# second-state/qwen3_asr_rs

Hardware: AMD Instinct MI355X
Metric: audio-seconds/sec (RTFx) Qwen3-ASR-0.6B greedy, 30s clips (higher is better)
Workload: dtype bf16; 1 GPU; Qwen3-ASR-0.6b bf16, batch=1 x 30s synthetic 16kHz clip per GPU, 100 new tokens (fixed, EOS ignored); clips_per_gpu=1, parallelism=dp1 (independent utterances per GPU, no data-path collective)

## Files before the change

### include/q3asr.h

```cpp
#ifndef Q3ASR_H
#define Q3ASR_H

#include <stdint.h>

#ifdef __cplusplus
extern "C" {
#endif

typedef struct q3a_engine q3a_engine;

typedef struct q3a_opts {
  int32_t precise;
  int32_t max_new_tokens;
  int32_t use_graph;
  int32_t debug_taps;
  int32_t valu_attention;
  int32_t token_logprobs;
  int32_t reserved[10];
} q3a_opts;

void q3a_opts_default(q3a_opts* o);

typedef struct q3a_dims {
  int32_t enc_d_model, enc_layers, enc_heads, enc_ffn, num_mel_bins, n_window, n_window_infer,
// ... 129 lines not shown


int32_t q3a_aligner_info(const q3a_engine* e, int32_t* classify_num, int32_t* timestamp_token_id, float* segment_ms);
int32_t q3a_build_align_prompt(int32_t num_audio_tokens, const int32_t* text_ids, int32_t n_text, int32_t* ids, int32_t* len);
int32_t q3a_align(q3a_engine* e, const int32_t* ids, const int32_t* lens, int32_t B, int32_t* out_classes, int32_t stride,
                  int32_t* out_counts, float* logits_out);
int32_t q3a_align_batch_ptrs(q3a_engine* e, const float* const* pcm16k, const int64_t* n_samples, int32_t B, const int32_t* text_ids,
                             const int32_t* text_lens, int32_t* out_classes, int32_t stride, int32_t* out_counts);
int32_t q3a_split_words_for_alignment(const char* utf8, const char* language, char* out, int32_t cap, int32_t* n_words,
                                      int32_t* len);
int32_t q3a_align_text_ids(const q3a_tokenizer* t, const char* const* words, int32_t n_words, int32_t timestamp_token_id,
                           int32_t* ids, int32_t cap, int32_t* n);
int32_t q3a_fix_timestamps(const float* ms, int32_t n, float* out);


int32_t q3a_score(q3a_engine* e, const int32_t* prompt_ids, const int32_t* prompt_lens, const int32_t* target_ids,
                  const int32_t* target_lens, int32_t B, float* out_lp, int32_t* out_top_ids, float* out_top_lp, int32_t stride,
                  float* logits_out);
int32_t q3a_score_batch_ptrs(q3a_engine* e, const float* const* pcm16k, const int64_t* n_samples, int32_t B,
                             const int32_t* lang_prefix_ids, int32_t n_prefix, const int32_t* target_ids, const int32_t* target_lens,
                             float* out_lp, int32_t* out_top_ids, float* out_top_lp, int32_t stride);


int32_t q3a_prefill_draft(q3a_engine* e, const int32_t* prompt_ids, const int32_t* prompt_lens, const int32_t* draft_ids,
                          const int32_t* draft_lens, int32_t B, int32_t* accepted_out, int32_t* next_ids_out, float* logits_out);
int32_t q3a_transcribe_draft_batch_ptrs(q3a_engine* e, const float* const* pcm16k, const int64_t* n_samples, int32_t B,
                                        const int32_t* lang_prefix_ids, int32_t n_prefix, const int32_t* draft_ids, const int32_t* draft_lens,
                                        int32_t max_new, int32_t max_rounds, int32_t min_tail, int32_t* out_ids, int32_t stride,
                                        int32_t* out_lens, int32_t* accepted_out);
int32_t q3a_draft_next_round(const int32_t* draft, int32_t n, int32_t k, int32_t tok, int32_t* out, int32_t cap, int32_t* n_out);
int32_t q3a_selftest_draft_accept(int32_t device, int32_t S, const int32_t* draft_ids, const int32_t* draft_off, const int32_t* prompt_lens,
                                  const int32_t* top_ids, const float* top_lp, int32_t out_stride, const uint16_t* embed, int32_t V, int32_t H,
                                  const float* norm_w, int32_t group_size, const float* cos_t, const float* sin_t, int32_t max_pos,
                                  int32_t* accepted, int32_t* out_ids, float* out_lp, int32_t* state, float* x_next, float* rope_cur,
                                  uint16_t* nn_x, float* nn_ss);


int32_t q3a_beam_search_batch_ptrs(q3a_engine* e, const float* const* pcm16k, const int64_t* n_samples, int32_t U,
                                   const int32_t* lang_prefix_ids, int32_t n_prefix, int32_t width, int32_t max_new, int32_t* out_ids,
                                   int32_t stride, int32_t* out_lens, float* out_scores, uint8_t* out_finished, float* out_lp);
int32_t q3a_beam_begin(q3a_engine* e, int32_t width);
int32_t q3a_beam_step(q3a_engine* e, uint8_t* all_finished, float* logits_out);
int32_t q3a_beam_fetch(q3a_engine* e, int32_t* out_ids, int32_t stride, int32_t* out_lens, float* out_scores, uint8_t* out_finished,
                       float* out_lp);
int32_t q3a_selftest_beam_topk(int32_t device, const float* logits, int32_t S, int32_t V, int32_t W, int32_t* out_ids, float* out_lp);
int32_t q3a_selftest_beam_advance(int32_t device, int32_t U, int32_t W, const int32_t* topk_ids, const float* topk_lp, const float* score_in,
                                  const uint8_t* finished_in, int32_t* parent_out, int32_t* token_out, float* score_out, uint8_t* finished_out);
int32_t q3a_selftest_kv_reorder(int32_t device, void* cache, int32_t elem_bytes, int32_t layers, int32_t S, int32_t n_kv, int32_t max_ctx,
                                const int32_t* lo, const int32_t* hi, const int32_t* parent);


int32_t q3a_set_logit_bias(q3a_engine* e, const int32_t* ids, const float* bias, int32_t n, float default_bias);
int32_t q3a_parse_logit_bias(const char* text, const char* suppress_list, int32_t* ids, float* bias, int32_t cap, int32_t* n);

int32_t q3a_set_sampling(q3a_engine* e, float temperature, float min_p, uint64_t seed);
uint32_t q3a_sample_word(uint64_t seed, uint32_t s, uint32_t t, uint32_t j);
int32_t q3a_selftest_sample(int32_t device, const float* logits, int32_t S, int32_t V, float temperature, float min_p,
                            uint64_t seed, int32_t step, int32_t* out_ids, float* out_lp, float* out_z);

int32_t q3a_set_repetition(q3a_engine* e, float repetition_penalty, int32_t no_repeat_ngram_size);
int32_t q3a_selftest_repeat(int32_t device, const float* logits, int32_t S, int32_t V, const int32_t* hist, int32_t stride,
                            const int32_t* lens, float p, int32_t n, float* out_logits, int32_t* out_ids, float* out_lp);

int32_t q3a_debug_set(const char* key, int32_t value);

int32_t q3a_selftest_gemm(int32_t device, int32_t M, int32_t N, int32_t K, int32_t split, float* max_abs_err,
                          float* ref_abs_max);
int32_t q3a_selftest_gemm16(int32_t device, int32_t M, int32_t N, int32_t K, int32_t reps, float* max_abs_err,
                            float* ref_abs_max, float* avg_us_bf16, float* avg_us_f32);

int32_t q3a_selftest_gemm_launch(int32_t device, int32_t launcher, int32_t flags, const void* x, const uint16_t* w, int32_t M, int32_t N, int32_t K,
                                 int32_t lda, int32_t ldo, int32_t imgs, int32_t H, int32_t Wd, int32_t C, const float* bias, const float* addend,
                                 int32_t addend_period, const float* resid, const int32_t* rowmap, int32_t act, void* out, int32_t out_rows);
int32_t q3a_selftest_qkrope_launch(int32_t device, int32_t fused, int32_t kv_f32, const uint16_t* x, int32_t lda, const uint16_t* w, int32_t M, int32_t K,
                                   const float* bias, float* qkv, const int32_t* row_seq, const int32_t* row_pos, const float* q_norm,
                                   const float* k_norm, float eps, const float* cos_t, const float* sin_t, int32_t max_pos, int32_t n_q, int32_t n_kv,
                                   int32_t n_seq, int32_t max_ctx, uint16_t* q16, void* kcache, void* vcache);
int32_t q3a_selftest_gemv_launch(int32_t device, int32_t pruned, const uint16_t* w, int32_t N, int32_t K, const float* x, const float* rms_w, float eps,
                                 const float* bias, int32_t mode, const float* resid, const float* attn_pm, const float* attn_pl, const float* attn_po,
                                 int32_t attn_nsplit, int32_t attn_heads, float* out, int32_t* out_state);
int32_t q3a_selftest_decode_attn_launch(int32_t device, int32_t kv_f32, const float* qkv, int32_t pos, const float* q_norm, const float* k_norm, float eps,
                                        const float* rope_cur, void* kcache, void* vcache, int32_t n_q, int32_t n_kv, int32_t max_ctx, int32_t nsplit,
                                        float scale_div, float* pm, float* pl, float* po);
int32_t q3a_gemm256_split_rows(int32_t M, int32_t N);

#ifdef __cplusplus
}
#endif
#endif
```

### qwen3_asr_rs_amd/_lib.py

```python
from __future__ import annotations

import ctypes as C
import os

HERE = os.path.dirname(os.path.abspath(__file__))
LIB_PATH = os.environ.get("Q3A_LIB") or os.path.join(HERE, "lib", "libq3asr_hip.so")

SYMBOLS = [
    "q3a_opts_default", "q3a_device_count", "q3a_engine_create", "q3a_arena_bytes", "q3a_arena_pack", "q3a_engine_create_from_arena",
    "q3a_engine_destroy", "q3a_last_error", "q3a_get_dims", "q3a_weights_rounded", "q3a_num_frames", "q3a_num_audio_tokens",
    "q3a_build_prompt", "q3a_mel", "q3a_encode", "q3a_prefill", "q3a_decode_step", "q3a_set_next_tokens",
    "q3a_upload_pcm", "q3a_run_resident", "q3a_fetch_ids", "q3a_fetch_logprobs", "q3a_transcribe_batch", "q3a_transcribe_batch_ptrs", "q3a_io_timings_last", "q3a_stage_timings",
    "q3a_profile_decode_step", "q3a_profile_weight_stream", "q3a_measure_peaks", "q3a_debug_read", "q3a_debug_set", "q3a_selftest_gemm", "q3a_selftest_gemm16",
    "q3a_load_audio", "q3a_resample", "q3a_resample_rubato", "q3a_free", "q3a_tokenizer_create", "q3a_tokenizer_destroy",
    "q3a_tokenizer_decode", "q3a_tokenizer_encode", "q3a_normalize_nfc", "q3a_parse_asr_output", "q3a_capitalize_first",
    "q3a_group_create", "q3a_group_destroy", "q3a_group_size", "q3a_group_used_rccl", "q3a_group_last_error",
    "q3a_group_engine", "q3a_group_partition", "q3a_group_transcribe", "q3a_group_transcribe_ptrs", "q3a_group_startup_seconds",
    "q3a_aligner_info", "q3a_build_align_prompt", "q3a_align", "q3a_align_batch_ptrs", "q3a_split_words_for_alignment",
    "q3a_align_text_ids", "q3a_fix_timestamps", "q3a_score", "q3a_score_batch_ptrs",
    "q3a_beam_search_batch_ptrs", "q3a_beam_begin", "q3a_beam_step", "q3a_beam_fetch", "q3a_selftest_beam_topk", "q3a_selftest_beam_advance",
    "q3a_selftest_kv_reorder", "q3a_set_logit_bias", "q3a_parse_logit_bias",
    "q3a_set_sampling", "q3a_sample_word", "q3a_selftest_sample",
    "q3a_set_repetition", "q3a_selftest_repeat",
    "q3a_selftest_gemm_launch", "q3a_selftest_qkrope_launch", "q3a_gemm256_split_rows",
    "q3a_selftest_gemv_launch", "q3a_selftest_decode_attn_launch",
    "q3a_prefill_draft", "q3a_transcribe_draft_batch_ptrs", "q3a_draft_next_round", "q3a_selftest_draft_accept",
]


class Peaks(C.Structure):
    _fields_ = [("hbm_read_gbps", C.c_double), ("hbm_copy_gbps", C.c_double), ("hbm_triad_gbps", C.c_double), ("hbm_read_bytes", C.c_double),
                ("mfma_bf16_tflops", C.c_double), ("gemm_m", C.c_int32), ("gemm_n", C.c_int32), ("gemm_k", C.c_int32), ("n_cu", C.c_int32),
                ("reps", C.c_int32), ("reserved", C.c_int32), ("mfma_bf16_tflops_random", C.c_double)]


class Opts(C.Structure):
    _fields_ = [("precise", C.c_int32), ("max_new_tokens", C.c_int32), ("use_graph", C.c_int32),
                ("debug_taps", C.c_int32), ("valu_attention", C.c_int32), ("token_logprobs", C.c_int32), ("reserved", C.c_int32 * 10)]


class DimsC(C.Structure):
    _fields_ = [(n, C.c_int32) for n in (
        "enc_d_model", "enc_layers", "enc_heads", "enc_ffn", "num_mel_bins", "n_window", "n_window_infer",
        "conv_channels", "enc_output_dim", "max_source_positions", "vocab_size", "hidden_size",
        "intermediate_size", "dec_layers", "num_q_heads", "num_kv_heads", "head_dim", "tie_word_embeddings",
        "mrope_interleaved")] + [("mrope_section", C.c_int32 * 4), ("rms_norm_eps", C.c_float), ("rope_theta", C.c_double)]


class Timings(C.Structure):
    _fields_ = [("mel_ms", C.c_float), ("encoder_ms", C.c_float), ("prefill_ms", C.c_float), ("decode_ms", C.c_float),
                ("total_ms", C.c_float), ("decode_steps", C.c_int32), ("batch", C.c_int32),
                ("total_audio_tokens", C.c_int32), ("total_prompt_tokens", C.c_int32)]


class IoTimings(C.Structure):
    _fields_ = [("stage_ms", C.c_float), ("h2d_ms", C.c_float), ("wall_ms", C.c_float), ("pieces", C.c_int32), ("threads", C.c_int32),
                ("mode", C.c_int32)]


KC_NAMES = ["gemv_qkv_gateup", "decode_attn", "argmax", "gemm", "norm", "other", "gemv_o_proj", "gemv_down", "gemv_lm_head"]


class KernelProfile(C.Structure):
    _fields_ = [("total_us", C.c_float * 9), ("launches", C.c_int32 * 9), ("weight_bytes", C.c_double * 9)]


_lib = None


def load() -> C.CDLL:
    global _lib
    if _lib is not None:
        return _lib
    if not os.path.exists(LIB_PATH):
        raise RuntimeError(f"{LIB_PATH} not found: build it with `python -m qwen3_asr_rs_amd.build` "
                           "(there is no CPU fallback for the HIP engine)")
    lib = C.CDLL(LIB_PATH)
    P, i32, i64, u64, f32p = C.c_void_p, C.c_int32, C.c_int64, C.c_uint64, C.POINTER(C.c_float)
    i32p, i64p, u8p = C.POINTER(C.c_int32), C.POINTER(C.c_int64), C.POINTER(C.c_uint8)
    sig = {
        "q3a_opts_default": (None, [C.POINTER(Opts)]),
        "q3a_device_count": (i32, []),
        "q3a_engine_create": (i32, [C.c_char_p, i32, C.POINTER(Opts), C.POINTER(P)]),
        "q3a_arena_bytes": (i32, [C.c_char_p, C.POINTER(u64)]),
        "q3a_arena_pack": (i32, [C.c_char_p, P, u64]),
        "q3a_engine_create_from_arena": (i32, [C.c_char_p, i32, P, u64, C.POINTER(Opts), C.POINTER(P)]),
        "q3a_engine_destroy": (None, [P]),
        "q3a_last_error": (C.c_char_p, [P]),
        "q3a_get_dims": (i32, [P, C.POINTER(DimsC)]),
        "q3a_weights_rounded": (i32, [P]),
        "q3a_num_frames": (i64, [i64]),
        "q3a_num_audio_tokens": (i32, [P, i64]),
        "q3a_build_prompt": (i32, [i32, i32p, i32, i32p, i32p]),
        "q3a_mel": (i32, [P, f32p, i64p, i32, f32p, i32p]),
        "q3a_encode": (i32, [P, f32p, i32p]),
        "q3a_prefill": (i32, [P, i32p, i32p, i32, f32p, i32p]),
        "q3a_decode_step": (i32, [P, i32p, u8p, f32p]),
        "q3a_set_next_tokens": (i32, [P, i32p, i32]),
        "q3a_upload_pcm": (i32, [P, f32p, i64p, i32]),
        "q3a_run_resident": (i32, [P, i32p, i32, i32, i32]),
        "q3a_fetch_ids": (i32, [P, i32p, i32, i32p]),
        "q3a_fetch_logprobs": (i32, [P, f32p, i32, i32p]),
        "q3a_transcribe_batch": (i32, [P, f32p, i64p, i32, i32p, i32, i32, i32, i32p, i32, i32p]),
        "q3a_transcribe_batch_ptrs": (i32, [P, C.POINTER(P), i64p, i32, i32p, i32, i32, i32, i32p, i32, i32p]),
        "q3a_io_timings_last": (i32, [P, C.POINTER(IoTimings)]),
        "q3a_stage_timings": (i32, [P, C.POINTER(Timings)]),
        "q3a_profile_decode_step": (i32, [P, C.POINTER(KernelProfile)]),
        "q3a_profile_weight_stream": (i32, [P, i32, f32p, C.POINTER(C.c_double), i32p]),
        "q3a_measure_peaks": (i32, [i32, i32, C.POINTER(Peaks)]),
        "q3a_debug_read": (i32, [P, C.c_char_p, P, u64, C.POINTER(u64)]),
        "q3a_debug_set": (i32, [C.c_char_p, i32]),
        "q3a_selftest_gemm": (i32, [i32, i32, i32, i32, i32, f32p, f32p]),
        "q3a_selftest_gemm16": (i32, [i32, i32, i32, i32, i32, f32p, f32p, f32p, f32p]),
        "q3a_load_audio": (i32, [C.c_char_p, i32, C.POINTER(f32p), i64p]),
        "q3a_resample": (i32, [f32p, i64, i32, i32, C.POINTER(f32p), i64p]),
        "q3a_resample_rubato": (i32, [f32p, i64, i32, i32, C.POINTER(f32p), i64p]),
        "q3a_free": (None, [P]),
        "q3a_tokenizer_create": (i32, [C.c_char_p, C.POINTER(P)]),
        "q3a_tokenizer_destroy": (None, [P]),
        "q3a_tokenizer_decode": (i32, [P, i32p, i32, i32, C.c_char_p, i32, i32p]),
        "q3a_tokenizer_encode": (i32, [P, C.c_char_p, i32p, i32, i32p]),
        "q3a_parse_asr_output": (i32, [C.c_char_p, i32, C.c_char_p, i32, C.c_char_p, i32]),
        "q3a_capitalize_first": (i32, [C.c_char_p, C.c_char_p, i32]),
        "q3a_normalize_nfc": (i32, [C.c_char_p, C.c_char_p, i32, i32p]),
        "q3a_group_create": (i32, [C.c_char_p, i32, i32p, C.POINTER(Opts), C.POINTER(P)]),
        "q3a_group_destroy": (None, [P]),
        "q3a_group_size": (i32, [P]),
        "q3a_group_used_rccl": (i32, [P]),
        "q3a_group_startup_seconds": (i32, [P, C.POINTER(C.c_double)]),
        "q3a_group_last_error": (C.c_char_p, [P]),
        "q3a_group_engine": (P, [P, i32]),
        "q3a_group_partition": (None, [i32, i32, i32, i32p, i32p]),
        "q3a_group_transcribe": (i32, [P, f32p, i64p, i32, i32p, i32, i32, i32, i32p, i32, i32p]),
        "q3a_group_transcribe_ptrs": (i32, [P, C.POINTER(P), i64p, i32, i32p, i32, i32, i32, i32p, i32, i32p]),
        "q3a_aligner_info": (i32, [P, i32p, i32p, f32p]),
        "q3a_build_align_prompt": (i32, [i32, i32p, i32, i32p, i32p]),
        "q3a_align": (i32, [P, i32p, i32p, i32, i32p, i32, i32p, f32p]),
        "q3a_align_batch_ptrs": (i32, [P, C.POINTER(P), i64p, i32, i32p, i32p, i32p, i32, i32p]),
        "q3a_split_words_for_alignment": (i32, [C.c_char_p, C.c_char_p, C.c_char_p, i32, i32p, i32p]),
        "q3a_align_text_ids": (i32, [P, C.POINTER(C.c_char_p), i32, i32, i32p, i32, i32p]),
        "q3a_fix_timestamps": (i32, [f32p, i32, f32p]),
        "q3a_score": (i32, [P, i32p, i32p, i32p, i32p, i32, f32p, i32p, f32p, i32, f32p]),
        "q3a_score_batch_ptrs": (i32, [P, C.POINTER(P), i64p, i32, i32p, i32, i32p, i32p, f32p, i32p, f32p, i32]),
        "q3a_beam_search_batch_ptrs": (i32, [P, C.POINTER(P), i64p, i32, i32p, i32, i32, i32, i32p, i32, i32p, f32p, u8p, f32p]),
        "q3a_beam_begin": (i32, [P, i32]),
        "q3a_beam_step": (i32, [P, u8p, f32p]),
        "q3a_beam_fetch": (i32, [P, i32p, i32, i32p, f32p, u8p, f32p]),
        "q3a_selftest_beam_topk": (i32, [i32, f32p, i32, i32, i32, i32p, f32p]),
        "q3a_selftest_beam_advance": (i32, [i32, i32, i32, i32p, f32p, f32p, u8p, i32p, i32p, f32p, u8p]),
        "q3a_selftest_kv_reorder": (i32, [i32, P, i32, i32, i32, i32, i32, i32p, i32p, i32p]),
        "q3a_set_logit_bias": (i32, [P, i32p, f32p, i32, C.c_float]),
        "q3a_parse_logit_bias": (i32, [C.c_char_p, C.c_char_p, i32p, f32p, i32, i32p]),
        "q3a_set_sampling": (i32, [P, C.c_float, C.c_float, u64]),
        "q3a_sample_word": (C.c_uint32, [u64, C.c_uint32, C.c_uint32, C.c_uint32]),
        "q3a_selftest_sample": (i32, [i32, f32p, i32, i32, C.c_float, C.c_float, u64, i32, i32p, f32p, f32p]),
        "q3a_set_repetition": (i32, [P, C.c_float, i32]),
        "q3a_selftest_repeat": (i32, [i32, f32p, i32, i32, i32p, i32, i32p, C.c_float, i32, f32p, i32p, f32p]),
        "q3a_selftest_gemm_launch": (i32, [i32, i32, i32, P, P, i32, i32, i32, i32, i32, i32, i32, i32, i32, P, P, i32, P, P, i32, P, i32]),
        "q3a_selftest_qkrope_launch": (i32, [i32, i32, i32, P, i32, P, i32, i32, P, P, P, P, P, P, C.c_float, P, P, i32, i32, i32, i32, i32, P, P, P]),
        "q3a_selftest_gemv_launch": (i32, [i32, i32, P, i32, i32, P, P, C.c_float, P, i32, P, P, P, P, i32, i32, P, P]),
        "q3a_selftest_decode_attn_launch": (i32, [i32, i32, P, i32, P, P, C.c_float, P, P, P, i32, i32, i32, i32, C.c_float, P, P, P]),
        "q3a_gemm256_split_rows": (i32, [i32, i32]),
        "q3a_prefill_draft": (i32, [P, i32p, i32p, i32p, i32p, i32, i32p, i32p, f32p]),
        "q3a_transcribe_draft_batch_ptrs": (i32, [P, C.POINTER(P), i64p, i32, i32p, i32, i32p, i32p, i32, i32, i32, i32p, i32, i32p, i32p]),
        "q3a_draft_next_round": (i32, [i32p, i32, i32, i32, i32p, i32, i32p]),
        "q3a_selftest_draft_accept": (i32, [i32, i32, i32p, i32p, i32p, i32p, f32p, i32, P, i32, i32, f32p, i32, f32p, f32p, i32,
                                            i32p, i32p, f32p, i32p, f32p, f32p, P, f32p]),
    }
    for name, (res, args) in sig.items():
        fn = getattr(lib, name)
        fn.restype = res
        fn.argtypes = args
    _lib = lib
    return lib
```

### qwen3_asr_rs_amd/csrc/engine.cpp

```cpp
#include <hip/hip_runtime.h>

#include <sched.h>

#include <chrono>
#include <cmath>
#include <cstdio>
#include <cstring>
#include <map>
#include <memory>
#include <mutex>
#include <thread>

#include "engine_internal.h"

using namespace q3a;

namespace {

thread_local std::string g_last_error;

constexpr int kGemvMaxSeq = 2;

template <typename T>
void upload(DevBuf& b, const std::vector<T>& v, hipStream_t s) {
  b.ensure(std::max<size_t>(v.size() * sizeof(T), 16));
  if (!v.empty()) HIPCHK(hipMemcpyAsync(b.p, v.data(), v.size() * sizeof(T), hipMemcpyHostToDevice, s));
}

struct ProfEvent {
  int kclass;
  double bytes;
  hipEvent_t a, b;
};

template <class Build>
std::pair<std::vector<int32_t>, std::vector<int32_t>> concat_prompts(int B, Build&& build) {
  std::vector<int32_t> ids, lens(B);
  for (int s = 0; s < B; ++s) {
    lens[s] = build(s, nullptr);
    const size_t o = ids.size();
    ids.resize(o + lens[s]);
    build(s, ids.data() + o);
  }
  return {std::move(ids), std::move(lens)};
}

void require_utterance_ptrs(const char* what, const float* const* ptrs, int B) {
  for (int u = 0; u < B; ++u)
    if (!ptrs[u]) fail(std::string(what) + ": null utterance pointer");
}

}

namespace q3a {
struct KnobEntry { const char* key; const char* env; std::atomic<int> Knobs::*field; };
static const KnobEntry kKnobTable[] = {
    {"gemm256_min_tiles", "Q3A_GEMM256_MIN_TILES", &Knobs::gemm256_min_tiles},
    {"gemm256_persist", "Q3A_GEMM256_PERSIST", &Knobs::gemm256_persist},
    {"gemm256_group_m", "Q3A_GEMM256_GROUP_M", &Knobs::gemm256_group_m},
    {"dattn_batched_min_wgs", "Q3A_DATTN_BATCHED_MIN_WGS", &Knobs::dattn_batched_min_wgs},
    {"decode_group_size", "Q3A_DECODE_GROUP", &Knobs::decode_group_size},
    {"decode_parallel_groups", "Q3A_DECODE_PARALLEL", &Knobs::decode_parallel_groups},
    {"fuse_qkrope", "Q3A_FUSE_QKROPE", &Knobs::fuse_qkrope},
    {"skinny_q", "Q3A_SKINNY_Q", &Knobs::skinny_q},
    {"eos_run_ahead", "Q3A_EOS_RUN_AHEAD", &Knobs::eos_run_ahead},
    {"skinny_glu_hp3", "Q3A_SKINNY_GLU_HP3", &Knobs::skinny_glu_hp3},
    {"lm_head_prune", "Q3A_LM_HEAD_PRUNE", &Knobs::lm_head_prune},
    {"layer_taps", "Q3A_DEBUG_LAYER_TAPS", &Knobs::layer_taps},
    {"poison_attn_partials", nullptr, &Knobs::poison_attn_partials},
};
Knobs& knobs() {
  static Knobs k;
  static std::once_flag once;
  std::call_once(once, [] {
    for (const KnobEntry& t : kKnobTable)
      if (const char* e = t.env ? getenv(t.env) : nullptr) (k.*t.field).store(atoi(e));
  });
  return k;
}
}

namespace {

struct Taps {
  std::map<std::string, DevBuf> bufs;  std::map<std::string, size_t> bytes;
  DevBuf& reserve(const char* name, size_t n) { DevBuf& t = bufs[name]; t.ensure(n); bytes[name] = n; return t; }
  static bool light(const char* name) { return strcmp(name, "dec_last_hidden") == 0 || strcmp(name, "head_in") == 0; }
  void copy(int level, hipStream_t s, const char* name, const void* ptr, size_t n) {
    if (!level || n == 0 || (level == 2 && !light(name))) return;
    HIPCHK(hipMemcpyAsync(reserve(name, n).p, ptr, n, hipMemcpyDeviceToDevice, s));
  }
};

struct StepView {
  const Dims& d; const ArenaLayout& L; const q3a_opts& opts;
  uint8_t* const& arena; const uint32_t& arena_flags; const hipStream_t& stream;
  const std::vector<hipStream_t>& chain_streams;
  const std::vector<hipEvent_t>& join_ev; const hipEvent_t& fork_ev; const int& n_cu; int* const& host_prog_dev;
  std::vector<ProfEvent>* const& prof; Taps& taps;
  const int8_t* const& lm_q; const float* const& lm_qs; const int& lm_q_cols;
  const int &B, &max_ctx, &max_new, &gsize, &live_nsplit_, &attn_nsplit, &min_P_, &part_stride, &beam_w_;
  const size_t& kv_layer_elems; const bool& head_logits_;
  const int &k_parallel_groups, &k_skinny_q, &k_dattn_batched_min_wgs, &k_skinny_glu_hp3, &k_lm_head_prune;
  const bool& logit_bias_on_;
  const bool& sampling_on_;
  const bool& repetition_on_;

  bool precise() const { return opts.precise != 0; }
  bool token_lp() const { return opts.token_logprobs != 0; }
  bool kv_f32() const { return opts.precise != 0; }
  size_t kv_elem() const { return kv_f32() ? 4 : 2; }
  int fast_math() const { return precise() ? 0 : 1; }
  template <typename T> const T* w(uint64_t off) const { return reinterpret_cast<const T*>(arena + off); }
  const float* wf(uint64_t off) const { return w<float>(off); }
  const uint16_t* wh(uint64_t off) const { return w<uint16_t>(off); }
};

struct DecodeStep : StepView {
  DevBuf kcache, vcache, x_dec, d_pos, next_tok, out_ids, step_count, done, s_ln, s_qkv, s_ctx, s_act, logits, part_val, part_idx;
  DevBuf part_sum, out_lp;
  DevBuf blk_lo, blk_hi;
  DevBuf prune_stats;
  DevBuf attn_pm, attn_pl, attn_po, nn_x, nn_ss;
  DevBuf rope_cur, rope_cos, rope_sin;
  DevBuf n_done, forced_tok;
  DevBuf beam_cand_val, beam_cand_idx, beam_part_max, beam_part_sum, beam_topk_ids, beam_topk_lp, beam_score, beam_finished, beam_parent, beam_token;
  DevBuf beam_feed, beam_hist_parent, beam_hist_token, beam_hist_lp, beam_state, beam_lo;
  DevBuf logit_bias;
  DevBuf samp_params, samp_max, samp_sum;
  DevBuf rep_params;
  DevBuf draft_accepted;
  template <class Self, class F> static void each_buf(Self& s, F&& f) {
    for (auto* b : {&s.kcache, &s.vcache, &s.x_dec, &s.d_pos, &s.next_tok, &s.out_ids, &s.step_count, &s.done, &s.s_ln, &s.s_qkv, &s.s_ctx, &s.s_act, &s.logits,
                    &s.part_val, &s.part_idx, &s.part_sum, &s.out_lp, &s.blk_lo, &s.blk_hi, &s.prune_stats, &s.attn_pm, &s.attn_pl, &s.attn_po, &s.nn_x, &s.nn_ss,
                    &s.rope_cur, &s.rope_cos, &s.rope_sin, &s.n_done, &s.forced_tok,
                    &s.beam_cand_val, &s.beam_cand_idx, &s.beam_part_max, &s.beam_part_sum, &s.beam_topk_ids, &s.beam_topk_lp, &s.beam_score, &s.beam_finished,
                    &s.beam_parent, &s.beam_token, &s.beam_feed, &s.beam_hist_parent, &s.beam_hist_token, &s.beam_hist_lp, &s.beam_state, &s.beam_lo,
                    &s.logit_bias, &s.samp_params, &s.samp_max, &s.samp_sum, &s.rep_params, &s.draft_accepted})
      f(*b);
  }

  void tap(const char* name, const void* ptr, size_t bytes) { taps.copy(opts.debug_taps, stream, name, ptr, bytes); }
  template <class F> void timed(int kclass, double bytes, F&& fn) {
    if (!prof) return fn();
    ProfEvent pe{kclass, bytes, nullptr, nullptr};
    HIPCHK(hipEventCreate(&pe.a));
    HIPCHK(hipEventCreate(&pe.b));
    HIPCHK(hipEventRecord(pe.a, stream));
    fn();
    HIPCHK(hipEventRecord(pe.b, stream));
    prof->push_back(pe);
  }

  void* kc_layer(int l) { return (uint8_t*)kcache.p + (size_t)l * kv_layer_elems * kv_elem(); }
  void* vc_layer(int l) { return (uint8_t*)vcache.p + (size_t)l * kv_layer_elems * kv_elem(); }

  LmHeadPruneArgs prune_args(const GemvArgs& g) {
    LmHeadPruneArgs pa{};
    pa.g = g; pa.Wq = lm_q; pa.qcols = lm_q_cols; pa.qs = lm_qs;
    pa.blk_lo = blk_lo.as<float>(); pa.blk_hi = blk_hi.as<float>(); pa.stats = prune_stats.as<int>();
    pa.logit_bias = g.bias != nullptr;
    return pa;
  }

  const float* head_bias() const { return logit_bias_on_ ? logit_bias.as<float>() : nullptr; }

  void run_head(int advance) {
    const int S = B, H = d.hidden, V = d.vocab;
    const float* const hb = head_bias();
    const bool sample = sampling_on_, repeat = repetition_on_, store = head_logits_ || sample || repeat;
    tap("head_in", x_dec.p, (size_t)S * H * 4);
    const double wbytes = 2.0 * V * H;
    int n_part = 0;
    const ArgmaxPartials part{part_val.as<float>(), part_idx.as<int>(), token_lp() ? part_sum.as<float>() : nullptr, part_stride};
    if (S <= kGemvMaxSeq) {
      GemvArgs g{};
      g.fast_math = fast_math();
      g.x = x_dec.as<float>(); g.ldx = H; g.rms_w = wf(L.final_norm); g.eps = d.rms_eps;
      g.W = wh(L.lm_head); g.N = V; g.K = H; g.mode = 3; g.out = logits.as<float>(); g.ldo = V;
      g.part = part; g.bias = hb;
      LmHeadPruneArgs pa{};
      const bool prunable = S == 1 && !precise() && lm_q_cols > 0 && (pa = prune_args(g), !lm_head_prune_check(pa));
      if (prunable && opts.debug_taps == 1) {
        DevBuf& t = taps.reserve("lm_head_bound", (size_t)V * 8);
        LmHeadPruneArgs pd = pa;
        pd.dbg = t.as<float>(); pd.stats = nullptr;
        KCHK(launch_lm_head_approx(pd, stream));
      }
      if (prunable && k_lm_head_prune && !store) {
        g.out = nullptr; pa.g.out = nullptr;
        n_part = lm_head_rescore_groups(g, n_cu);
        timed(Q3A_KC_GEMV_LM_HEAD, (double)V * lm_q_cols, [&] { KCHK(launch_lm_head_approx(pa, stream)); });
        timed(Q3A_KC_ARGMAX, 0, [&] { KCHK(launch_lm_head_rescore(pa, n_part, stream)); });
      } else {
        n_part = gemv_blocks(g);
        timed(Q3A_KC_GEMV_LM_HEAD, wbytes, [&] { KCHK(launch_gemv(g, S, stream)); });
      }
    } else if (!precise()) {
      timed(Q3A_KC_NORM, 0, [&] { KCHK(launch_rmsnorm(x_dec.as<float>(), wf(L.final_norm), s_ln.as<float>(), S, H, d.rms_eps, stream, s_ln.as<uint16_t>())); });
      GemmEpilogue ep; ep.out = logits.as<float>(); ep.ldo = V; ep.bias = hb;
      if (S <= 32 && V % 4 == 0 && H % 64 == 0 && part_stride >= (V + 63) / 64) {
        ep.part = part;
        if (!store) ep.out = nullptr;
        n_part = (V + 63) / 64;
        timed(Q3A_KC_GEMM, wbytes, [&] { KCHK(launch_gemm16(s_ln.as<uint16_t>(), H, wh(L.lm_head), S, V, H, ep, false, stream)); });
      } else {
        timed(Q3A_KC_GEMM, wbytes, [&] { KCHK(launch_gemm16(s_ln.as<uint16_t>(), H, wh(L.lm_head), S, V, H, ep, false, stream)); });
        n_part = 128;
        if (!repeat) timed(Q3A_KC_ARGMAX, 0, [&] { KCHK(launch_argmax_partials(logits.as<float>(), V, S, part, n_part, stream)); });
      }
    } else {
      timed(Q3A_KC_NORM, 0, [&] { KCHK(launch_rmsnorm(x_dec.as<float>(), wf(L.final_norm), s_ln.as<float>(), S, H, d.rms_eps, stream)); });
      timed(Q3A_KC_GEMM, wbytes, [&] { batched_proj(s_ln.as<float>(), H, wh(L.lm_head), V, H, hb, 0, logits.as<float>(), V, nullptr); });
      n_part = 128;
      if (!repeat) timed(Q3A_KC_ARGMAX, 0, [&] { KCHK(launch_argmax_partials(logits.as<float>(), V, S, part, n_part, stream)); });
    }
    if (repeat) n_part = enqueue_repetition(part, !sample);
// ... 42 lines not shown
  void enqueue_sample_logprob() {
    SampleLogprobArgs sl{};
    sl.logits = logits.as<float>(); sl.S = B; sl.V = d.vocab; sl.chunk_max = samp_max.as<float>(); sl.chunk_sum = samp_sum.as<float>();
    sl.next_tok = next_tok.as<int>(); sl.step_count = step_count.as<int>(); sl.out_lp = out_lp.as<float>(); sl.out_stride = max_new;
    timed(Q3A_KC_ARGMAX, 0, [&] { KCHK(launch_sample_logprob(sl, stream)); });
  }

  bool prenorm_path() const { return B > kGemvMaxSeq && !precise(); }
  bool skinny_q() const {
    auto whole = [](int K) { const int st = K / 32, per = (st + 7) / 8, unr = per <= 2 ? 2 : per <= 4 ? 4 : per <= 8 ? 8 : 12; return K % 256 == 0 && per % unr == 0; };
    return k_skinny_q != 0 && !precise() && d.hidden % 64 == 0 && whole(d.q_dim()) && whole(d.inter);
  }
  int nn_parts() const { return d.hidden / (skinny_q() ? 8 : 16); }
  int n_groups(int b) const { return b <= kGemvMaxSeq ? 1 : (b + gsize - 1) / gsize; }
  size_t nn_x_stride() const { return (size_t)32 * d.hidden; }
  size_t nn_ss_stride() const { return (size_t)nn_parts() * 32; }
  uint16_t* nn_x_g(int g) const { return nn_x.as<uint16_t>() + (size_t)g * nn_x_stride(); }
  float* nn_ss_g(int g) const { return nn_ss.as<float>() + (size_t)g * nn_ss_stride(); }
  float* s_ctx_g(int g) const { return s_ctx.as<float>() + (size_t)g * 32 * d.q_dim(); }
  float* s_act_g(int g) const { return s_act.as<float>() + (size_t)g * 32 * d.inter; }
  NextNormOut first_layer_norm_out() const {
    NextNormOut nn{};
    if (prenorm_path()) {
      nn.next_w = wf(L.dec[0].in_ln); nn.next_xw16f = nn_x.as<uint16_t>(); nn.next_ss = nn_ss.as<float>(); nn.nparts = nn_parts();
      nn.group_stride_x = (long)nn_x_stride(); nn.group_stride_ss = (long)nn_ss_stride(); nn.group_size = gsize;
    }
    return nn;
  }

  void batched_proj(const float* x, int ldx, const uint16_t* W, int N, int K, const float* bias, int mode, float* out,
                    int ldo, const float* resid) {
    const int S = B;
    if (S <= 32) {
      SkinnyArgs sk{};
      sk.fast_math = fast_math();
      sk.x = x; sk.ldx = ldx; sk.S = S; sk.W = W; sk.N = N; sk.K = K; sk.bias = bias; sk.mode = mode; sk.out = out; sk.ldo = ldo; sk.resid = resid;
      KCHK(launch_skinny(sk, precise(), stream));
    } else {
      GemmEpilogue ep; ep.out = out; ep.ldo = ldo; ep.bias = bias; ep.resid = (mode == 1) ? resid : nullptr;
      KCHK(launch_gemm(x, ldx, W, S, N, K, ep, mode == 2, precise(), stream));
    }
  }

  struct Proj {
    const uint16_t* W;
    int N, K;
    const float* bias;
    int mode;
    int kclass;
    double bytes;
  };
  struct LayerProjs { Proj qkv, o, gu, down; };
  LayerProjs layer_projs(int li) const {
    const DecLayerOff& l = L.dec[li];
    const int H = d.hidden, I = d.inter, QD = d.q_dim(), QKV = d.qkv_dim();
    auto proj = [&](uint64_t w_off, int N, int K, uint32_t bias_flag, uint64_t b_off, int mode, int kclass) {
      return Proj{wh(w_off), N, K, (arena_flags & bias_flag) ? wf(b_off) : nullptr, mode, kclass, 2.0 * N * K};
    };
    return {proj(l.qkv_w, QKV, H, kFlagDecQkvBias, l.qkv_b, 0, Q3A_KC_GEMV), proj(l.o_w, H, QD, kFlagDecOBias, l.o_b, 1, Q3A_KC_GEMV_O),
            proj(l.gu_w, 2 * I, H, kFlagDecMlpBias, l.gu_b, 2, Q3A_KC_GEMV), proj(l.down_w, H, I, kFlagDecMlpBias, l.down_b, 1, Q3A_KC_GEMV_DOWN)};
  }
  template <class Args> Args proj_args(const Proj& p) const {
    Args a{};
    a.fast_math = fast_math(); a.eps = d.rms_eps;
    a.W = p.W; a.N = p.N; a.K = p.K; a.ldx = p.K; a.bias = p.bias; a.mode = p.mode; a.ldo = p.mode == 2 ? p.N / 2 : p.N;
    return a;
  }
  GemvArgs gemv_args(const Proj& p) const { return proj_args<GemvArgs>(p); }
  SkinnyArgs skinny_args(const Proj& p, int S) const { SkinnyArgs k = proj_args<SkinnyArgs>(p); k.S = S; return k; }

  void decode_layer(int li, int grp, int s0, int S, hipStream_t ks) {
    const int H = d.hidden, QKV = d.qkv_dim();
    const bool gemv = B <= kGemvMaxSeq;
    const DecLayerOff& l = L.dec[li];
    const LayerProjs pj = layer_projs(li);
    float* const x = x_dec.as<float>() + (size_t)s0 * H;
    float* const qkv = s_qkv.as<float>() + (size_t)s0 * QKV;
    const size_t kv_seq = (size_t)d.n_kv * max_ctx * 128 * kv_elem();
    DecodeAttnArgs da{};
    da.qkv = qkv; da.pos = d_pos.as<int>() + s0; da.eps = d.rms_eps;
    da.rope_cur = rope_cur.as<float>() + (size_t)s0 * 128;
    da.pm = attn_pm.as<float>() + (size_t)s0 * d.n_q * attn_nsplit; da.pl = attn_pl.as<float>() + (size_t)s0 * d.n_q * attn_nsplit;
    da.po = attn_po.as<float>() + (size_t)s0 * d.n_q * attn_nsplit * 128; da.nsplit = live_nsplit_;
    da.n_q = d.n_q; da.n_kv = d.n_kv; da.max_ctx = max_ctx; da.scale_div = sqrtf((float)d.head_dim);
    da.q_norm = wf(l.q_norm); da.k_norm = wf(l.k_norm);
    da.kcache = (uint8_t*)kc_layer(li) + (size_t)s0 * kv_seq; da.vcache = (uint8_t*)vc_layer(li) + (size_t)s0 * kv_seq;
    if (gemv) {
      auto run = [&](const Proj& p, const GemvArgs& a) { timed(p.kclass, p.bytes, [&] { KCHK(launch_gemv(a, S, ks)); }); };
      GemvArgs g = gemv_args(pj.qkv);
      g.x = x; g.rms_w = wf(l.in_ln); g.out = qkv;
      run(pj.qkv, g);
      timed(Q3A_KC_DECODE_ATTN, 0, [&] { KCHK(launch_decode_attn(da, S, kv_f32(), ks)); });
      GemvArgs o = gemv_args(pj.o);
      if (std::min(S, 4) * d.n_q * live_nsplit_ <= GEMV_ATTN_MAX_TABLE) {
        o.attn_pm = da.pm; o.attn_pl = da.pl; o.attn_po = da.po;
        o.attn_nsplit = live_nsplit_; o.attn_heads = d.n_q; o.attn_fast_exp = fast_math();
      } else {
        timed(Q3A_KC_DECODE_ATTN, 0, [&] { KCHK(launch_attn_combine(da.pm, da.pl, da.po, live_nsplit_, S, d.n_q, s_ctx_g(grp), ks)); });
        o.x = s_ctx_g(grp);
      }
      o.out = x; o.resid = x;
      run(pj.o, o);
      GemvArgs u = gemv_args(pj.gu);
      u.x = x; u.rms_w = wf(l.post_ln); u.out = s_act_g(grp);
      run(pj.gu, u);
      GemvArgs dn = gemv_args(pj.down);
      dn.x = s_act_g(grp); dn.out = x; dn.resid = x;
      run(pj.down, dn);
      return;
    }
    const bool b16 = !precise(), pre = prenorm_path();
    uint16_t* const s_ctx16 = b16 ? reinterpret_cast<uint16_t*>(s_ctx_g(grp)) : nullptr;
    uint16_t* const s_act16 = b16 ? reinterpret_cast<uint16_t*>(s_act_g(grp)) : nullptr;
    auto run = [&](const Proj& p, const SkinnyArgs& a) { timed(Q3A_KC_GEMM, p.bytes, [&] { KCHK(launch_skinny(a, precise(), ks)); }); };
    auto from_residual = [&](SkinnyArgs& a, const float* norm_w) {
      a.x = x;
      if (pre) { a.xw16f = nn_x_g(grp); a.ss_parts = nn_ss_g(grp); a.ss_nparts = nn_parts(); }
      else a.rms_w = norm_w;
    };
    auto to_residual = [&](SkinnyArgs& a, const float* next_w) {
      a.out = x; a.resid = x;
      a.qsplit = b16 && skinny_q();
      if (pre && next_w) { a.next_w = next_w; a.next_xw16f = nn_x_g(grp); a.next_ss = nn_ss_g(grp); }
    };
    SkinnyArgs q = skinny_args(pj.qkv, S);
    from_residual(q, wf(l.in_ln));
    q.out = qkv;
    run(pj.qkv, q);
    if (S * d.n_kv >= k_dattn_batched_min_wgs) {
      if (b16) { da.out16 = s_ctx16; da.out_frag = 1; } else da.out = s_ctx_g(grp);
      da.trim_prologue = min_P_ < 2 * 128;
      timed(Q3A_KC_DECODE_ATTN, 0, [&] { KCHK(launch_decode_attn_batched(da, S, kv_f32(), ks)); });
    } else {
      timed(Q3A_KC_DECODE_ATTN, 0, [&] { KCHK(launch_decode_attn(da, S, kv_f32(), ks)); });
      timed(Q3A_KC_DECODE_ATTN, 0, [&] { KCHK(launch_attn_combine(da.pm, da.pl, da.po, live_nsplit_, S, d.n_q, s_ctx_g(grp), ks, s_ctx16, b16)); });
    }
    SkinnyArgs o = skinny_args(pj.o, S);
    o.x = s_ctx_g(grp); o.x16 = s_ctx16; o.x16_frag = b16;
    to_residual(o, wf(l.post_ln));
    run(pj.o, o);
    SkinnyArgs u = skinny_args(pj.gu, S);
    from_residual(u, wf(l.post_ln));
    u.out = s_act_g(grp); u.out16 = s_act16; u.out16_frag = b16;
    u.n_cu = n_cu;
    u.glu_hp3 = k_skinny_glu_hp3;
    run(pj.gu, u);
    SkinnyArgs dn = skinny_args(pj.down, S);
    dn.x = s_act_g(grp); dn.x16 = s_act16; dn.x16_frag = b16;
    to_residual(dn, li + 1 < d.dec_layers ? wf(L.dec[li + 1].in_ln) : nullptr);
    run(pj.down, dn);
  }

  bool forks() const { return n_groups(B) > 1 && !prof && k_parallel_groups != 0; }
  void enqueue_decode_step() {
    const int ng = n_groups(B);
    const bool chains = forks();
    if (chains) HIPCHK(hipEventRecord(fork_ev, stream));
    for (int g = 0; g < ng; ++g) {
      const int s0 = ng == 1 ? 0 : g * gsize;
      const int S = ng == 1 ? B : std::min(gsize, B - s0);
      hipStream_t ks = (chains && g > 0) ? chain_streams[g - 1] : stream;
      if (chains && g > 0) HIPCHK(hipStreamWaitEvent(ks, fork_ev, 0));
      for (int li = 0; li < d.dec_layers; ++li) decode_layer(li, g, s0, S, ks);
      if (chains && g > 0) {
        HIPCHK(hipEventRecord(join_ev[g - 1], ks));
        HIPCHK(hipStreamWaitEvent(stream, join_ev[g - 1], 0));
      }
    }
    run_head(1);
  }

  bool uses_key_splits() const {
    if (B <= kGemvMaxSeq) return true;
    const int ng = n_groups(B);
    const int smallest = ng == 1 ? B : std::min(gsize, B - (ng - 1) * gsize);
    return smallest * d.n_kv < k_dattn_batched_min_wgs;
  }

  void enqueue_step() {
    enqueue_decode_step();
    if (beam_w_ > 0) enqueue_beam_round();
  }
  void enqueue_beam_round() {
    const int W = beam_w_, S = B, U = B / W;
    BeamTopkArgs t{};
    t.logits = logits.as<float>(); t.S = S; t.V = d.vocab; t.W = W;
    t.cand_val = beam_cand_val.as<float>(); t.cand_idx = beam_cand_idx.as<int>();
    t.part_max = beam_part_max.as<float>(); t.part_sum = beam_part_sum.as<float>();
    t.out_ids = beam_topk_ids.as<int>(); t.out_lp = beam_topk_lp.as<float>();
    timed(Q3A_KC_ARGMAX, 0, [&] { KCHK(launch_beam_topk(t, stream)); });
    BeamAdvanceArgs a{};
    a.U = U; a.W = W; a.topk_ids = t.out_ids; a.topk_lp = t.out_lp;
    a.score = beam_score.as<float>(); a.finished = beam_finished.as<uint8_t>();
    a.parent = beam_parent.as<int>(); a.token = beam_token.as<int>(); a.feed = beam_feed.as<int>();
    a.hist_parent = beam_hist_parent.as<int>(); a.hist_token = beam_hist_token.as<int>(); a.hist_lp = beam_hist_lp.as<float>();
    a.hist_cap = max_new; a.state = beam_state.as<int>();
    a.pos = d_pos.as<int>(); a.lo = beam_lo.as<int>(); a.hi_bias = -1;
    a.host_progress = host_prog_dev + 2; a.eos0 = kEos0; a.eos1 = kEos1;
    timed(Q3A_KC_ARGMAX, 0, [&] { KCHK(launch_beam_advance(a, stream)); });
    KvReorderArgs r{};
    r.kcache = kcache.p; r.vcache = vcache.p; r.elem_bytes = (int)kv_elem(); r.layers = d.dec_layers; r.S = S; r.n_kv = d.n_kv; r.max_ctx = max_ctx;
    r.parent = a.parent; r.lo = a.lo; r.hi = a.pos; r.hi_bias = -1; r.all_done = a.state + BEAM_ST_ALL_DONE;
    timed(Q3A_KC_OTHER, 0, [&] { KCHK(launch_kv_reorder(r, stream)); });
    timed(Q3A_KC_OTHER, 0, [&] { enqueue_set_tokens(a.feed); });
  }
};

enum class Stage { None, Batch, Mel, Encoded, Decoding };

class CallState {
  Stage stage_ = Stage::None;
  int beam_w_ = 0;
  bool fixed_mode_ = false;
  bool head_logits_ = true;
 public:
  bool at(Stage s) const { return stage_ >= s; }
  const int& beam_w() const { return beam_w_; }
  bool fixed_mode() const { return fixed_mode_; }
  const bool& head_logits() const { return head_logits_; }
  void advance(Stage s) { if (stage_ < s) stage_ = s; }
  void rewind(Stage s) {
    if (stage_ > s) stage_ = s;
    if (stage_ < Stage::Decoding) end_search();
  }
  void drop_decode_state() { rewind(Stage::Encoded); }
  void require(Stage s, const char* text) const { if (stage_ < s) fail(text); }
  void require(Stage s, const std::string& text) const { require(s, text.c_str()); }
  void begin_search(int W) { beam_w_ = W; }
  void end_search() { beam_w_ = 0; }
  void begin_call(bool fixed, bool keep_logits) { fixed_mode_ = fixed; head_logits_ = keep_logits; }
  void begin_step_call() { head_logits_ = true; }
};

}

struct q3a_engine : CallState {
  Dims d;
  ArenaLayout L;
  q3a_opts opts{};
  int device = 0;
  hipStream_t stream = nullptr;
  uint8_t* arena = nullptr;
  bool own_arena = false;
  uint32_t arena_flags = 0;
  std::string err;

  DevBuf dft, filt_t, pos_emb;
  int rope_positions = 0;

  int B = 0;
  std::vector<int64_t> n_samples, pcm_off, mel_off;
  std::vector<int> n_frames, n_chunks, T, tok_off;
  int total_chunks = 0, total_T = 0, max_frames = 0;
  std::vector<int> P, seq_off;
  int total_P = 0, max_ctx = 0, max_new = 0;
  std::vector<AttnSeg> enc_segs_h;
  int enc_max_seg = 0;

  DevBuf pcm, d_pcm_off, d_n_samples, d_mel_off, d_n_frames, mel, gmax, d_chunk_utt, d_chunk_frame0;
  DevBuf conv1, conv2, conv3, conv3_rowmap, convout_rowmap;
  DevBuf enc_x, enc_ln, enc_qkv, enc_ctx, enc_ffn, enc_segs, audio_embeds;
  DevBuf ids, audio_rowmap, row_seq, row_pos, dec_segs, last_rows;
  DevBuf dec_x, dec_ln, dec_qkv, dec_ctx, dec_act;
  DevBuf lm_q_buf, lm_qs_buf;
  const int8_t* lm_q = nullptr; const float* lm_qs = nullptr;
  int lm_q_cols = 0;
  DevBuf enc_ctx16, dec_ctx16;
  DevBuf dec_q16;
  int n_cu = 256;
  int* host_prog = nullptr;
  int* host_prog_dev = nullptr;
  DevBuf zero_page;
  int part_stride = 0, attn_nsplit = 0;
  size_t kv_layer_elems = 0;

  int gsize = 32;
  int k_parallel_groups = 1, k_skinny_q = 1, k_dattn_batched_min_wgs = 128, k_skinny_glu_hp3 = 1, k_lm_head_prune = 1;
  std::vector<hipStream_t> chain_streams;
  std::vector<hipEvent_t> join_ev;
  hipEvent_t fork_ev = nullptr;

  static constexpr size_t kGraphCacheMax = 16;
  std::vector<std::pair<std::string, hipGraphExec_t>> graph_cache;
  int pos_hi_ = 0, live_nsplit_ = 0;
  int min_P_ = 0;

  hipStream_t up_stream = nullptr;
  void* pin_p = nullptr;
  size_t pin_cap = 0;
  std::vector<hipEvent_t> up_ev;
  hipEvent_t up_t0 = nullptr, up_t1 = nullptr;
  q3a_io_timings io{};
  bool geom_valid = false;

  q3a_timings timings{};
  hipEvent_t ev[5] = {nullptr, nullptr, nullptr, nullptr, nullptr};
  std::vector<ProfEvent>* prof = nullptr;
  Taps taps;

  bool logit_bias_on_ = false;
  int logit_bias_finite_ = 0;
  bool sampling_on_ = false;
  uint32_t samp_words_[4] = {0, 0, 0, 0};
  bool logit_bias_eos_open_ = true;
  bool repetition_on_ = false;
  float rep_penalty_ = 1.f;
  int rep_ngram_ = 0;

  DecodeStep step{StepView{d, L, opts, arena, arena_flags, stream, chain_streams, join_ev, fork_ev, n_cu, host_prog_dev, prof, taps, lm_q, lm_qs, lm_q_cols,
                           B, max_ctx, max_new, gsize, live_nsplit_, attn_nsplit, min_P_, part_stride, beam_w(), kv_layer_elems, head_logits(),
                           k_parallel_groups, k_skinny_q, k_dattn_batched_min_wgs, k_skinny_glu_hp3, k_lm_head_prune, logit_bias_on_, sampling_on_, repetition_on_}};

  bool precise() const { return step.precise(); }
  bool token_lp() const { return step.token_lp(); }
  bool kv_f32() const { return step.kv_f32(); }
  size_t kv_elem() const { return step.kv_elem(); }
  size_t act_elem() const { return precise() ? 4 : 2; }
  bool valu_attn() const { return precise() || opts.valu_attention; }
  const float* wf(uint64_t off) const { return step.wf(off); }
  const uint16_t* wh(uint64_t off) const { return step.wh(off); }

  void tap(const char* name, const void* ptr, size_t bytes) { step.tap(name, ptr, bytes); }
  void tap_act(const char* name, const void* ptr, size_t elems) {
    if (!opts.debug_taps || elems == 0 || opts.debug_taps == 2) return;
    if (precise()) return tap(name, ptr, elems * 4);
    KCHK(launch_from_bf16((const uint16_t*)ptr, taps.reserve(name, elems * 4).as<float>(), elems, stream));
  }

  void act_gemm(const DevBuf& x, int lda, const uint16_t* W, int M, int N, int K, const GemmEpilogue& ep, bool glu) {
    if (precise()) KCHK(launch_gemm(x.as<float>(), lda, W, M, N, K, ep, glu, true, stream));
    else KCHK(launch_gemm16(x.as<uint16_t>(), lda, W, M, N, K, ep, glu, stream));
  }
  void act_conv(const DevBuf& x, int imgs, int H, int Wd, int C, const uint16_t* W, int Cout, const GemmEpilogue& ep) {
    if (precise()) KCHK(launch_conv3x3s2_gemm(x.as<float>(), imgs, H, Wd, C, W, Cout, ep, true, stream));
    else KCHK(launch_conv3x3s2_gemm16(x.as<uint16_t>(), zero_page.as<uint16_t>(), imgs, H, Wd, C, W, Cout, ep, stream));
  }
  void act_out(GemmEpilogue& ep, const DevBuf& buf) const {
    if (precise()) ep.out = buf.as<float>(); else ep.out16 = buf.as<uint16_t>();
  }
  uint16_t* act16(const DevBuf& buf) const { return precise() ? nullptr : buf.as<uint16_t>(); }

  float stage_ms(int i, int j) { float ms = 0.f; HIPCHK(hipEventElapsedTime(&ms, ev[i], ev[j])); return ms; }

  void init_common(const std::string& model_dir, int dev, const q3a_opts* o) {
    if (o) opts = *o; else q3a_opts_default(&opts);
    if (opts.max_new_tokens <= 0) opts.max_new_tokens = 4096;
    d = parse_config_file(model_dir + "/config.json");
    validate_dims(d);
    L = plan_arena(d);
    device = dev;
    int n_dev = 0;
    hipError_t e = hipGetDeviceCount(&n_dev);
    if (e != hipSuccess || n_dev == 0)
      fail("no HIP device available: libq3asr_hip has no CPU fallback (hipGetDeviceCount: " + std::string(hipGetErrorString(e)) + ")");
    if (dev < 0 || dev >= n_dev) fail("device index out of range");
    HIPCHK(hipSetDevice(dev));
    KCHK(skinny_init());
    (void)hipDeviceGetAttribute(&n_cu, hipDeviceAttributeMultiprocessorCount, dev);
    HIPCHK(hipStreamCreateWithFlags(&stream, hipStreamNonBlocking));
    for (auto& x : ev) HIPCHK(hipEventCreate(&x));
    HIPCHK(hipHostMalloc((void**)&host_prog, 64, hipHostMallocMapped));
    memset(host_prog, 0, 64);
    HIPCHK(hipHostGetDevicePointer((void**)&host_prog_dev, host_prog, 0));
    step.n_done.ensure(64);
    step.prune_stats.ensure(8);
    HIPCHK(hipMemsetAsync(step.prune_stats.p, 0, 8, stream));
    if (!d.aligner()) {
      step.logit_bias.ensure((size_t)d.vocab * 4);
      HIPCHK(hipMemsetAsync(step.logit_bias.p, 0, (size_t)d.vocab * 4, stream));
      logit_bias_finite_ = d.vocab;
      step.samp_params.ensure(16);
      step.rep_params.ensure(16);
    }
  }

  void init_tables() {
    auto dftm = make_dft_matrix(400, 416);
    auto filt = make_mel_filterbank_T(d.n_mels, 400, 16000, 202);
    auto pe = make_sinusoid_rows(d.tokens_per_chunk(), d.enc_d);
    upload(dft, dftm, stream);
    upload(filt_t, filt, stream);
    upload(pos_emb, pe, stream);
    zero_page.ensure(256);
    HIPCHK(hipMemsetAsync(zero_page.p, 0, 256, stream));
    ensure_rope(8192);
    HIPCHK(hipStreamSynchronize(stream));
  }

  void ensure_rope(int n_pos) {
    if (n_pos <= rope_positions) return;
    int n = std::max(n_pos, 8192);
    std::vector<float> c, s;
    make_rope_tables(n, d.head_dim, d.rope_theta, c, s);
    HIPCHK(hipStreamSynchronize(stream));
// ... 304 lines not shown
        tap(name, enc_x.p, Tt * D * 4);
      }
    }
    tap("enc_last", enc_x.p, Tt * D * 4);
    KCHK(launch_layernorm(enc_x.as<float>(), wf(L.ln_post_w), wf(L.ln_post_b), enc_ln.as<float>(), total_T, D, 1e-5f, stream, act16(enc_ln)));
    {
      GemmEpilogue ep; act_out(ep, enc_ffn); ep.ldo = D; ep.bias = wf(L.proj1_b); ep.act = 1;
      act_gemm(enc_ln, D, wh(L.proj1_w), total_T, D, D, ep, false);
    }
    {
      GemmEpilogue ep; ep.out = audio_embeds.as<float>(); ep.ldo = d.enc_out; ep.bias = wf(L.proj2_b);
      act_gemm(enc_ffn, D, wh(L.proj2_w), total_T, d.enc_out, D, ep, false);
    }
    tap("audio_embeds", audio_embeds.p, Tt * d.enc_out * 4);
    HIPCHK(hipGetLastError());
    advance(Stage::Encoded);
  }

  void setup_prompts(const int32_t* ids_h, const int32_t* lens, int b, int max_new_req, bool before_encoder = false) {
    if (!before_encoder) require_encoded("q3a_prefill", b);
    P.assign(lens, lens + b);
    end_search();
    seq_off.resize(b);
    std::vector<int> rowseq, rowpos, amap((size_t)total_T, -1), last(b);
    int off = 0, maxP = 0;
    for (int s = 0; s < b; ++s) {
      seq_off[s] = off;
      int na = 0;
      for (int i = 0; i < P[s]; ++i) {
        rowseq.push_back(s);
        rowpos.push_back(i);
        int id = ids_h[off + i];
        if (id < 0 || id >= d.vocab) fail("q3a_prefill: token id out of range");
        if (id == kAudioPad) {
          if (na >= T[s]) fail("q3a_prefill: more <|audio_pad|> tokens than encoder tokens");
          amap[(size_t)tok_off[s] + na] = off + i;
          ++na;
        }
      }
      if (na != T[s]) fail("q3a_prefill: number of <|audio_pad|> tokens does not match the encoder output length");
      if (P[s] <= 0) fail("q3a_prefill: empty prompt");
      last[s] = off + P[s] - 1;
      off += P[s];
      maxP = std::max(maxP, P[s]);
    }
    total_P = off;
    max_new = std::min(std::max(max_new_req, 1), opts.max_new_tokens);
    max_ctx = ((maxP + max_new + 1 + 127) / 128) * 128;
    pos_hi_ = maxP;
    min_P_ = *std::min_element(P.begin(), P.end());
    {
      static const int pad = [] { const char* e = getenv("Q3A_CTX_PAD"); return e ? atoi(e) : 0; }();
      if (pad > 0) max_ctx += (pad + 127) / 128 * 128;
    }
    ensure_rope(max_ctx + 1);
    std::vector<int> ids_v(ids_h, ids_h + total_P);
    std::vector<AttnSeg> segs(b);
    for (int s = 0; s < b; ++s)
      segs[s] = AttnSeg{seq_off[s], P[s], (int64_t)s * d.n_kv * max_ctx * 128};
    upload(ids, ids_v, stream);
    upload(row_seq, rowseq, stream);
    upload(row_pos, rowpos, stream);
    upload(audio_rowmap, amap, stream);
    upload(last_rows, last, stream);
    upload(dec_segs, segs, stream);
    upload(step.d_pos, P, stream);
    const size_t Pt = (size_t)total_P, H = d.hidden;
    dec_x.ensure(Pt * H * 4); dec_ln.ensure(Pt * H * act_elem()); dec_qkv.ensure(Pt * d.qkv_dim() * 4);
    dec_ctx.ensure(Pt * d.q_dim() * (valu_attn() ? 4 : act_elem())); dec_act.ensure(Pt * d.inter * act_elem());
    if (!valu_attn()) dec_q16.ensure(Pt * d.q_dim() * 2);
    if (valu_attn() && !precise()) dec_ctx16.ensure(Pt * d.q_dim() * 2);
    kv_layer_elems = (size_t)b * d.n_kv * max_ctx * 128;
    step.kcache.ensure(kv_layer_elems * d.dec_layers * kv_elem());
    step.vcache.ensure(kv_layer_elems * d.dec_layers * kv_elem());
    step.rope_cur.ensure((size_t)b * 128 * 4);
    {
      Knobs& kn = knobs();
      const int gs = kn.decode_group_size.load();
      gsize = (gs >= 1 && gs <= 32) ? gs : 32;
      k_parallel_groups = kn.decode_parallel_groups.load(); k_skinny_q = kn.skinny_q.load();
      k_dattn_batched_min_wgs = kn.dattn_batched_min_wgs.load();
      k_skinny_glu_hp3 = kn.skinny_glu_hp3.load();
      k_lm_head_prune = kn.lm_head_prune.load();
    }
    const size_t ng = (size_t)step.n_groups(b);
    step.nn_x.ensure(ng * 32 * H * 2); step.nn_ss.ensure((size_t)ng * (H / 8) * 32 * 4);
    step.x_dec.ensure((size_t)b * H * 4); step.next_tok.ensure((size_t)b * 4); step.forced_tok.ensure((size_t)b * 4); step.draft_accepted.ensure((size_t)b * 8);
    step.out_ids.ensure((size_t)b * max_new * 4); step.step_count.ensure((size_t)b * 4); step.done.ensure((size_t)b);
    step.s_ln.ensure((size_t)b * H * 4); step.s_qkv.ensure((size_t)b * d.qkv_dim() * 4); step.s_ctx.ensure(ng * 32 * d.q_dim() * 4);
    step.s_act.ensure(ng * 32 * d.inter * 4); step.logits.ensure((size_t)b * d.vocab * 4);
    part_stride = std::max(128, (d.vocab + 3) / 4);
    step.part_val.ensure((size_t)b * part_stride * 4); step.part_idx.ensure((size_t)b * part_stride * 4);
    if (token_lp()) { step.part_sum.ensure((size_t)b * part_stride * 4); step.out_lp.ensure((size_t)b * max_new * 4); }
    if (sampling_on_) { step.samp_max.ensure((size_t)b * sample_chunks(d.vocab) * 4); step.samp_sum.ensure((size_t)b * sample_chunks(d.vocab) * 4); }
    {
      const size_t nblk4 = ((size_t)(d.vocab + 15) / 16 + 3) & ~size_t(3);
      step.blk_lo.ensure(nblk4 * 4); step.blk_hi.ensure(nblk4 * 4);
    }
    attn_nsplit = (max_ctx + dattn_keys_per_split(kv_f32()) - 1) / dattn_keys_per_split(kv_f32());
    {
      const size_t n_stat = (size_t)b * d.n_q * attn_nsplit;
      step.attn_pm.ensure((n_stat + 8) * 4); step.attn_pl.ensure((n_stat + 8) * 4);
      step.attn_po.ensure(n_stat * 128 * 4);
      if (knobs().poison_attn_partials.load() != 0) {
        HIPCHK(hipMemsetAsync(step.attn_pm.p, 0xFF, step.attn_pm.cap, stream));
        HIPCHK(hipMemsetAsync(step.attn_pl.p, 0xFF, step.attn_pl.cap, stream));
        HIPCHK(hipMemsetAsync(step.attn_po.p, 0xFF, step.attn_po.cap, stream));
      }
    }
    HIPCHK(hipMemsetAsync(step.step_count.p, 0, (size_t)b * 4, stream));
    HIPCHK(hipMemsetAsync(step.done.p, 0, (size_t)b, stream));
    HIPCHK(hipMemsetAsync(step.n_done.p, 0, 64, stream));
    HIPCHK(hipMemsetAsync(step.out_ids.p, 0, (size_t)b * max_new * 4, stream));
    if (token_lp()) HIPCHK(hipMemsetAsync(step.out_lp.p, 0, (size_t)b * max_new * 4, stream));
    HIPCHK(hipStreamSynchronize(stream));
    for (auto cs : chain_streams) HIPCHK(hipStreamSynchronize(cs));
    __atomic_store_n(&host_prog[0], 0, __ATOMIC_RELAXED);
    __atomic_store_n(&host_prog[1], 0, __ATOMIC_RELAXED);
    drain_retired_graphs();
    {
      bool any = false;
      DecodeStep::each_buf(step, [&](DevBuf& sb) { any = any || sb.grew; sb.grew = false; });
      if (any) drop_graphs();
    }
  }

  void run_prefill() {
    run_prefill_layers();
    const int H = d.hidden;
    KCHK(launch_gather_rows(dec_x.as<float>(), last_rows.as<int>(), B, H, step.x_dec.as<float>(), stream));
    tap("dec_last_hidden", step.x_dec.p, (size_t)B * H * 4);
    step.run_head(0);
    tap("logits", step.logits.p, (size_t)B * d.vocab * 4);
    HIPCHK(hipGetLastError());
    advance(Stage::Decoding);
  }

  void run_prefill_layers() {
    drop_decode_state();
    const int H = d.hidden, I = d.inter, QD = d.q_dim(), QKV = d.qkv_dim();
    const bool sp = precise();
    KCHK(launch_embed(ids.as<int>(), total_P, wh(L.embed), H, kAudioPad, dec_x.as<float>(), stream));
    KCHK(launch_scatter_rows(audio_embeds.as<float>(), audio_rowmap.as<int>(), total_T, d.hidden, dec_x.as<float>(), stream));
    tap("dec_embed", dec_x.p, (size_t)total_P * H * 4);
    AttnArgs at{};
    at.q = dec_qkv.as<float>(); at.q_rs = QKV; at.kv_hs = (int64_t)max_ctx * 128; at.kv_rs = 128;
    at.o = dec_ctx.as<float>(); at.o_rs = QD; at.segs = dec_segs.as<AttnSeg>(); at.n_segs = B;
    at.max_len = *std::max_element(P.begin(), P.end()); at.n_kv_heads = d.n_kv;
    at.scale_div = sqrtf((float)d.head_dim);
    at.o16 = valu_attn() ? nullptr : dec_ctx.as<uint16_t>();
    if (!valu_attn()) { at.q16 = dec_q16.as<uint16_t>(); at.q_rs = QD; }
    const DevBuf& ctx_in = (valu_attn() && !sp) ? dec_ctx16 : dec_ctx;
    auto proj_gemm = [&](const DevBuf& x, const DecodeStep::Proj& p, GemmEpilogue ep) {
      ep.bias = p.bias;
      act_gemm(x, p.K, p.W, total_P, p.N, p.K, ep, p.mode == 2);
    };
    const bool fuse_rope = knobs().fuse_qkrope.load() != 0 && !valu_attn() && !precise() && d.head_dim == 128 && gemm256_eligible(total_P, QKV, H) && H % 64 == 0;
    const bool layer_taps = opts.debug_taps && knobs().layer_taps.load() != 0;
    for (int li = 0; li < d.dec_layers; ++li) {
      const DecLayerOff& l = L.dec[li];
      const DecodeStep::LayerProjs pj = step.layer_projs(li);
      auto ltap = [&](const char* what, const void* ptr, size_t bytes) {
        if (!layer_taps) return;
        char name[32];
        snprintf(name, sizeof(name), "L%02d_%s", li, what);
        tap(name, ptr, bytes);
      };
      KCHK(launch_rmsnorm(dec_x.as<float>(), wf(l.in_ln), dec_ln.as<float>(), total_P, H, d.rms_eps, stream, act16(dec_ln)));
      ltap("ln1", dec_ln.p, (size_t)total_P * H * act_elem());
      RopeKvArgs rk{};
      rk.qkv = dec_qkv.as<float>(); rk.row_seq = row_seq.as<int>(); rk.row_pos = row_pos.as<int>();
      rk.q_norm = wf(l.q_norm); rk.k_norm = wf(l.k_norm); rk.eps = d.rms_eps;
      rk.cos_t = step.rope_cos.as<float>(); rk.sin_t = step.rope_sin.as<float>();
      rk.kcache = step.kc_layer(li); rk.vcache = step.vc_layer(li); rk.n_q = d.n_q; rk.n_kv = d.n_kv; rk.max_ctx = max_ctx;
      rk.q16 = valu_attn() ? nullptr : dec_q16.as<uint16_t>();
      if (fuse_rope) {
        KCHK(launch_gemm256_qkrope(dec_ln.as<uint16_t>(), pj.qkv.K, pj.qkv.W, total_P, pj.qkv.K, pj.qkv.bias, rk, stream));
      } else {
        GemmEpilogue ep; ep.out = dec_qkv.as<float>(); ep.ldo = QKV;
        proj_gemm(dec_ln, pj.qkv, ep);
        KCHK(launch_qknorm_rope_kv(rk, total_P, kv_f32(), stream));
      }
// ... 171 lines not shown
      gp.lens[s] = p + fed;
      po += p; to += n;
    }
    return gp;
  }
  void run_score(const GivenPlan& sp, int stride, float* out_lp, int32_t* out_top_ids, float* out_top_lp, float* logits_out) {
    const int M = (int)sp.rows.size(), V = d.vocab;
    run_prefill_then_head(sp.rows, &score_head_ms, [&] { KCHK(launch_score_head(score_head_args(M, sp.targets, logits_out != nullptr), stream)); });
    if (M == 0) return;
    std::vector<float> res((size_t)M * 4);
    HIPCHK(hipMemcpy(res.data(), score_out.p, res.size() * 4, hipMemcpyDeviceToHost));
    if (logits_out) HIPCHK(hipMemcpy(logits_out, align_logits.p, (size_t)M * V * 4, hipMemcpyDeviceToHost));
    scatter_rows(res.data() + M, sp.n.data(), stride, out_lp);
    scatter_rows(reinterpret_cast<const int32_t*>(res.data()) + 2 * (size_t)M, sp.n.data(), stride, out_top_ids);
    scatter_rows(res.data() + 3 * (size_t)M, sp.n.data(), stride, out_top_lp);
  }
  DevBuf score_tgt, score_psum, score_out;
  float score_head_ms = 0.f;

  void draft_check(const char* what) const {
    require_asr(what);
    if (sampling_on_) fail(std::string(what) + ": sampling is on (q3a_set_sampling with temperature > 0): a sampled id is not the argmax of its row -- turn it off first");
    if (repetition_on_) fail(std::string(what) + ": repetition control is on (q3a_set_repetition): its choice depends on the history, not on the row alone -- turn it off first");
    if (beam_w() > 0) fail(std::string(what) + ": a beam search owns the decode state (a new q3a_prefill returns to the greedy step)");
  }
  void run_prefill_draft(const GivenPlan& dp, std::vector<int>& acc, float* logits_out) {
    const int M = (int)dp.rows.size(), V = d.vocab;
    std::vector<int> words((size_t)2 * B + 1, 0);
    for (int s = 0, off = 0; s < B; off += dp.lens[s++]) {
      words[s + 1] = words[s] + dp.n[s];
      words[(size_t)B + 1 + s] = dp.lens[s] - dp.n[s];
      words.insert(words.end(), dp.ids.begin() + off + dp.lens[s] - dp.n[s], dp.ids.begin() + off + dp.lens[s]);
    }
    const int* const plen = words.data() + B + 1;
    run_prefill_then_head(dp.rows, nullptr, [&] {
      upload(draft_in, words, stream);
      ScoreHeadArgs a = score_head_args(M, dp.targets, logits_out != nullptr);
      a.bias = step.head_bias();
      KCHK(launch_score_head(a, stream));
      DraftAcceptArgs da{};
      da.draft_off = draft_in.as<int>(); da.prompt_len = da.draft_off + B + 1; da.draft = da.prompt_len + B;
      da.top_id = a.top_id; da.top_lp = a.top_lp;
      step.enqueue_draft_accept(da);
    });
    acc.resize((size_t)2 * B);
    HIPCHK(hipMemcpy(acc.data(), step.draft_accepted.p, acc.size() * 4, hipMemcpyDeviceToHost));
    if (logits_out) HIPCHK(hipMemcpy(logits_out, align_logits.p, (size_t)M * V * 4, hipMemcpyDeviceToHost));
    pos_hi_ = 0; min_P_ = 0x7fffffff;
    for (int s = 0; s < B; ++s) {
      if (acc[s] < 0 || acc[s] > dp.n[s]) fail("draft accept: the device returned a first mismatch outside the draft");
      pos_hi_ = std::max(pos_hi_, plen[s] + acc[s]);
      min_P_ = std::min(min_P_, plen[s] + acc[s]);
    }
    draft_stats_[0] += 1;
    draft_stats_.push_back(total_P);
    advance(Stage::Decoding);
  }
  DevBuf draft_in;
  std::vector<int32_t> draft_stats_{0};

  void enqueue_step() {
    if (step.forks()) ensure_chain_streams(step.n_groups(B) - 1);
    step.enqueue_step();
  }
  void ensure_chain_streams(int n) {
    while ((int)chain_streams.size() < n) {
      hipStream_t s2;
      hipEvent_t e2;
      HIPCHK(hipStreamCreateWithFlags(&s2, hipStreamNonBlocking));
      HIPCHK(hipEventCreateWithFlags(&e2, hipEventDisableTiming));
      chain_streams.push_back(s2);
      join_ev.push_back(e2);
    }
    if (!fork_ev) HIPCHK(hipEventCreateWithFlags(&fork_ev, hipEventDisableTiming));
  }

  std::string make_graph_sig() const {
    uint64_t h = 1469598103934665603ull;
    DecodeStep::each_buf(step, [&](const DevBuf& sb) {
      uint64_t v = (uint64_t)(uintptr_t)sb.p;
      for (int i = 0; i < 8; ++i) { h ^= (v >> (8 * i)) & 0xff; h *= 1099511628211ull; }
    });
    char buf[256];
    snprintf(buf, sizeof(buf), "%d.%d.%d.%d.%d.%d.%d.%d.%d.%d.b%d.lb%d.sm%d.rp%d/%d/%d/%d/%p/%016llx", B, gsize, k_parallel_groups, k_skinny_q,
             k_dattn_batched_min_wgs, k_skinny_glu_hp3, k_lm_head_prune, (int)(min_P_ < 256), (int)head_logits(), (int)token_lp(), beam_w(), (int)logit_bias_on_, (int)sampling_on_, (int)repetition_on_, live_nsplit_,
             max_ctx, max_new, (const void*)arena, (unsigned long long)h);
    return buf;
  }

  template <class F> hipGraphExec_t capture_graph(F&& fn) {
    hipGraph_t g = nullptr;
    hipGraphExec_t exec = nullptr;
    HIPCHK(hipStreamBeginCapture(stream, hipStreamCaptureModeThreadLocal));
    try {
      fn();
    } catch (...) {
      hipGraph_t tmp = nullptr;
      (void)hipStreamEndCapture(stream, &tmp);
      if (tmp) (void)hipGraphDestroy(tmp);
      throw;
    }
    HIPCHK(hipStreamEndCapture(stream, &g));
    const hipError_t ie = hipGraphInstantiate(&exec, g, nullptr, nullptr, 0);
    (void)hipGraphDestroy(g);
    HIPCHK(ie);
    return exec;
  }
  hipGraphExec_t graph_for_step() {
    const std::string sig = make_graph_sig();
    for (size_t i = 0; i < graph_cache.size(); ++i)
      if (graph_cache[i].first == sig) {
        if (i + 1 != graph_cache.size()) std::rotate(graph_cache.begin() + i, graph_cache.begin() + i + 1, graph_cache.end());
        return graph_cache.back().second;
      }
    const hipGraphExec_t exec = capture_graph([&] { enqueue_step(); });
    ++graph_captures_;
    if (graph_cache.size() >= kGraphCacheMax) {
      retired_graphs.push_back(graph_cache.front().second);
      graph_cache.erase(graph_cache.begin());
    }
    graph_cache.emplace_back(sig, exec);
    return exec;
  }
  std::vector<hipGraphExec_t> retired_graphs;
  int32_t graph_captures_ = 0;
  void drain_retired_graphs() {
    for (auto ge : retired_graphs) (void)hipGraphExecDestroy(ge);
    retired_graphs.clear();
  }
  void drop_graphs() {
    drain_retired_graphs();
    for (auto& ge : graph_cache) (void)hipGraphExecDestroy(ge.second);
    graph_cache.clear();
  }

  void decode_steps(int n) {
    require(Stage::Decoding, "decode: no prefill state");
    if (n <= 0) return;
    const bool eager = !opts.use_graph || prof;
    const int kps = dattn_keys_per_split(kv_f32());
    for (int i = 0; i < n; ++i) {
      live_nsplit_ = step.uses_key_splits() ? std::min(attn_nsplit, pos_hi_ / kps + 1) : attn_nsplit;
      if (eager) enqueue_step();
      else HIPCHK(hipGraphLaunch(graph_for_step(), stream));
      ++pos_hi_;
    }
    if (eager) HIPCHK(hipGetLastError());
  }

  int max_new_request(int max_new_req, int fixed_new) const { return fixed_new > 0 ? fixed_new : max_new_req > 0 ? max_new_req : opts.max_new_tokens; }
  std::pair<std::vector<int32_t>, std::vector<int32_t>> asr_prompts(const int32_t* lang_ids, int n_prefix) const {
    return concat_prompts(B, [&](int s, int32_t* dst) {
      int32_t len = 0;
      q3a_build_prompt(T[s], lang_ids, n_prefix, dst, &len);
      return len;
    });
  }

  template <class Prompts>
  void whole_path_front(const char* what, const float* const* pcm16k, const int64_t* ns_in, int n, int width, int max_new_req, Prompts&& prompts) {
    if (!pcm16k || !ns_in || n < 1) fail(std::string(what) + ": bad argument");
    require_utterance_ptrs(what, pcm16k, n);
    HIPCHK(hipSetDevice(device));
    const int b = n * width;
    std::vector<const float*> ptrs((size_t)b);
    std::vector<int64_t> ns((size_t)b);
    for (int s = 0; s < b; ++s) { ptrs[s] = pcm16k[s / width]; ns[s] = ns_in[s / width]; }
    set_batch(ns.data(), b);
    auto&& [ids_v, lens_v] = prompts();
    setup_prompts(ids_v.data(), lens_v.data(), b, max_new_req, true);
    timings = q3a_timings{};
    upload_ptrs_and_mel(ptrs.data(), ns.data(), b);
    run_encoder();
  }

  void run_resident(int fixed_new, bool front_done = false) {
    if (!front_done) {
      HIPCHK(hipEventRecord(ev[0], stream));
      run_mel();
      HIPCHK(hipEventRecord(ev[1], stream));
      run_encoder();
    }
    HIPCHK(hipEventRecord(ev[2], stream));
    run_prefill();
    HIPCHK(hipEventRecord(ev[3], stream));
    int steps = 0;
    static const bool host_timing = [] { const char* e = getenv("Q3A_DEBUG_HOST_TIMING"); return e && atoi(e) != 0; }();
    const auto h0 = std::chrono::steady_clock::now();
    if (fixed_new > 0) {
      steps = fixed_new - 1;
      decode_steps(steps);
      if (host_timing) fprintf(stderr, "[q3a host timing] %d graph launches enqueued in %.1f us\n", steps,
                               std::chrono::duration<double, std::micro>(std::chrono::steady_clock::now() - h0).count());
    } else {
      steps = run_ahead(host_prog, max_new - 1, "greedy");
    }
    HIPCHK(hipEventRecord(ev[4], stream));
    HIPCHK(hipStreamSynchronize(stream));
    HIPCHK(hipGetLastError());
    decode_timings(steps);
  }

  void fetch_ids(int32_t* out, int stride, int32_t* out_lens) {
    if (!at(Stage::Decoding) || beam_w() > 0) fail("q3a_fetch_ids: nothing generated");
    fetch_generated<int32_t>(nullptr, out, stride, out_lens);
  }
  void fetch_logprobs(float* out, int stride, int32_t* out_lens) {
    if (!token_lp()) fail("q3a_fetch_logprobs: the engine was created without opts.token_logprobs = 1");
    require(Stage::Decoding, "q3a_fetch_logprobs: nothing generated");
    fetch_generated<float>(&step.out_lp, out, stride, out_lens);
  }
  template <class T> void fetch_generated(const DevBuf* vals, T* out, int stride, int32_t* out_lens) {
    std::vector<int> ids((size_t)B * max_new);
    std::vector<T> v(vals ? ids.size() : 0);
    HIPCHK(hipMemcpy(ids.data(), step.out_ids.p, ids.size() * 4, hipMemcpyDeviceToHost));
    if (vals) HIPCHK(hipMemcpy(v.data(), vals->p, v.size() * sizeof(T), hipMemcpyDeviceToHost));
    generated_lens(ids, out_lens);
    for (int s = 0; s < B; ++s)
      for (int i = 0; i < std::min(out_lens[s], stride); ++i) out[(size_t)s * stride + i] = vals ? v[(size_t)s * max_new + i] : (T)ids[(size_t)s * max_new + i];
  }
  void generated_lens(const std::vector<int>& all, int32_t* out_lens) {
    std::vector<int> sc(B);
    HIPCHK(hipMemcpy(sc.data(), step.step_count.p, (size_t)B * 4, hipMemcpyDeviceToHost));
    for (int s = 0; s < B; ++s) {
      int n = std::min(sc[s], max_new), len = 0;
// ... 924 lines not shown
```

### qwen3_asr_rs_amd/csrc/k_dattn.hip

```cpp
#include <stdlib.h>

#include <type_traits>

#include "dev.h"
#include "kernels.h"

namespace q3a {
namespace {

template <typename KVT> struct Frag16;
template <> struct Frag16<uint16_t> {
  static constexpr int DPL = 8;
  static __device__ __forceinline__ void unpack(const uint4& r, float (&f)[8]) {
    f[0] = bf16lo(r.x); f[1] = bf16hi(r.x); f[2] = bf16lo(r.y); f[3] = bf16hi(r.y);
    f[4] = bf16lo(r.z); f[5] = bf16hi(r.z); f[6] = bf16lo(r.w); f[7] = bf16hi(r.w);
  }
};
template <> struct Frag16<float> {
  static constexpr int DPL = 4;
  static __device__ __forceinline__ void unpack(const uint4& r, float (&f)[4]) {
    f[0] = __uint_as_float(r.x); f[1] = __uint_as_float(r.y); f[2] = __uint_as_float(r.z); f[3] = __uint_as_float(r.w);
  }
};

#ifndef Q3A_DATTN_NT
#define Q3A_DATTN_NT 1
#endif
#ifndef Q3A_DA_WAVES
#define Q3A_DA_WAVES 8
#endif
constexpr int DA_WAVES = Q3A_DA_WAVES;

template <int GROUP, typename KVT>
__device__ __forceinline__ void decode_attn_body(const DecodeAttnArgs& a, const int kvh, const int s, const int sp) {
  constexpr int DPL = Frag16<KVT>::DPL;
  constexpr int LPK = 128 / DPL;
  constexpr int KPI = 64 / LPK;
  constexpr int SPLIT_KEYS = sizeof(KVT) == 2 ? DATTN_KEYS_PER_SPLIT_BF16 : DATTN_KEYS_PER_SPLIT_F32;
  constexpr int NI = (SPLIT_KEYS / DA_WAVES) / KPI;
  constexpr int KEYS_PER_WAVE = KPI * NI;
  constexpr int KEYS_PER_SPLIT = KEYS_PER_WAVE * DA_WAVES;
  static_assert(KEYS_PER_SPLIT == (sizeof(KVT) == 2 ? DATTN_KEYS_PER_SPLIT_BF16 : DATTN_KEYS_PER_SPLIT_F32), "split size");
  __shared__ float q_s[GROUP][128];
  __shared__ __attribute__((aligned(16))) KVT k_s[128];
  __shared__ __attribute__((aligned(16))) KVT v_s[128];
  __shared__ float cm[DA_WAVES][GROUP], cl[DA_WAVES][GROUP];
  __shared__ float co[DA_WAVES][GROUP][128];
  const int pos = a.pos[s];
  Q3A_ARG(a.q_norm); Q3A_ARG(a.k_norm); Q3A_ARG(a.eps); Q3A_ARG(a.pm); Q3A_ARG(a.pl); Q3A_ARG(a.po); Q3A_ARG(a.scale_div); Q3A_ARG(pos);
  const int tid = threadIdx.x, lane = tid & 63, wave = tid >> 6;
  const int stamp_wg = (blockIdx.z * gridDim.y + blockIdx.y) * gridDim.x + blockIdx.x;
  Q3A_STAMP_ENTRY(t_entry);
  const int sub = lane % LPK, kq = lane / LPK;
  const int key_lo = sp * KEYS_PER_SPLIT;
  const size_t pbase = ((size_t)s * a.n_q + (size_t)kvh * GROUP) * a.nsplit + sp;
  const int qkv_dim = (a.n_q + 2 * a.n_kv) * 128;
  const float* row = a.qkv + (size_t)s * qkv_dim;
  KVT* kc = reinterpret_cast<KVT*>(a.kcache) + ((size_t)s * a.n_kv + kvh) * (size_t)a.max_ctx * 128;
  KVT* vc = reinterpret_cast<KVT*>(a.vcache) + ((size_t)s * a.n_kv + kvh) * (size_t)a.max_ctx * 128;

  float x1 = 0.f, x2 = 0.f, nw1 = 0.f, nw2 = 0.f, c = 0.f, sn = 0.f;
  auto load_rows = [&]() {
    if (wave < GROUP + 2) {
      const int r = wave < GROUP ? kvh * GROUP + wave : (wave == GROUP ? a.n_q + kvh : a.n_q + a.n_kv + kvh);
      x1 = row[r * 128 + lane];
      x2 = row[r * 128 + lane + 64];
    }
  };
  if (wave <= GROUP) {
    const float* nw = wave < GROUP ? a.q_norm : a.k_norm;
    nw1 = nw[lane];
    nw2 = nw[lane + 64];
    c = a.rope_cur[(size_t)s * 128 + lane];
    sn = a.rope_cur[(size_t)s * 128 + 64 + lane];
  }
  load_rows();
  const int key_base = key_lo + wave * KEYS_PER_WAVE + kq;
  uint4 kraw[NI], vraw[NI];
#pragma unroll
  for (int i = 0; i < NI; ++i) {
    const int key = min(key_base + i * KPI, a.max_ctx - 1);
#if Q3A_DATTN_NT
    kraw[i] = ld_stream16(kc + (size_t)key * 128 + sub * DPL);
    vraw[i] = ld_stream16(vc + (size_t)key * 128 + sub * DPL);
#else
    kraw[i] = *reinterpret_cast<const uint4*>(kc + (size_t)key * 128 + sub * DPL);
    vraw[i] = *reinterpret_cast<const uint4*>(vc + (size_t)key * 128 + sub * DPL);
#endif
  }
  __builtin_amdgcn_sched_barrier(0);
  Q3A_STAMP_AT(a.stamp, stamp_wg, 1);
  Q3A_STAMP_PUT(a.stamp, stamp_wg, 0, t_entry);
  if (key_lo > pos) {
    if (tid < GROUP) { a.pm[pbase + (size_t)tid * a.nsplit] = -INFINITY; a.pl[pbase + (size_t)tid * a.nsplit] = 0.f; }
    if (tid < GROUP * 128) a.po[(pbase + (size_t)(tid >> 7) * a.nsplit) * 128 + (tid & 127)] = 0.f;
    return;
  }
  const bool owner = (pos - key_lo) < KEYS_PER_SPLIT;

  if (wave <= GROUP) {
    const float ss = wave_sum_fast(x1 * x1 + x2 * x2);
    const float rstd = rstd_of(ss / 128.0f + a.eps, sizeof(KVT) == 2);
    const float n1 = (x1 * rstd) * nw1, n2 = (x2 * rstd) * nw2;
    rope_rotate(n1, n2, c, sn, x1, x2);
  }
  if (wave < GROUP) {
    q_s[wave][lane] = x1;
    q_s[wave][lane + 64] = x2;
  } else if (owner && wave == GROUP) {
    KvIo<KVT>::store(kc + (size_t)pos * 128 + lane, x1);
    KvIo<KVT>::store(kc + (size_t)pos * 128 + lane + 64, x2);
    KvIo<KVT>::store(&k_s[lane], x1);
    KvIo<KVT>::store(&k_s[lane + 64], x2);
  } else if (owner && wave == GROUP + 1) {
    KvIo<KVT>::store(vc + (size_t)pos * 128 + lane, x1);
    KvIo<KVT>::store(vc + (size_t)pos * 128 + lane + 64, x2);
    KvIo<KVT>::store(&v_s[lane], x1);
    KvIo<KVT>::store(&v_s[lane + 64], x2);
  }
  __syncthreads();
  Q3A_STAMP_AT(a.stamp, stamp_wg, 2);

  const float inv_scale = 1.0f / a.scale_div;
  auto expw = [](float x) { return sizeof(KVT) == 4 ? expf(x) : __expf(x); };
  f32x2_t qf[GROUP][DPL / 2];
#pragma unroll
  for (int g = 0; g < GROUP; ++g)
#pragma unroll
    for (int e = 0; e < DPL / 2; ++e) qf[g][e] = f32x2_t{q_s[g][sub * DPL + 2 * e], q_s[g][sub * DPL + 2 * e + 1]};
  const uint4 k_new = *reinterpret_cast<const uint4*>(&k_s[sub * DPL]), v_new = *reinterpret_cast<const uint4*>(&v_s[sub * DPL]);
  float sc[NI][GROUP];
#pragma unroll
  for (int i = 0; i < NI; ++i) {
    const int key = key_base + i * KPI;
    if (key == pos) { kraw[i] = k_new; vraw[i] = v_new; }
    if (key > pos) vraw[i] = make_uint4(0u, 0u, 0u, 0u);
    float kf[DPL];
    Frag16<KVT>::unpack(kraw[i], kf);
#pragma unroll
    for (int g = 0; g < GROUP; ++g) {
      f32x2_t p2 = qf[g][0] * f32x2_t{kf[0], kf[1]};
#pragma unroll
      for (int e = 1; e < DPL / 2; ++e) p2 += qf[g][e] * f32x2_t{kf[2 * e], kf[2 * e + 1]};
      float p = p2.x + p2.y;
      p = row16_sum(p);
      if (LPK == 32) p = xor16_sum(p);
      sc[i][g] = (key <= pos) ? p * inv_scale : -INFINITY;
    }
  }
  f32x2_t acc[GROUP][DPL / 2];
  float mw[GROUP], lw[GROUP];
#pragma unroll
  for (int g = 0; g < GROUP; ++g) {
    float mx = sc[0][g];
#pragma unroll
    for (int i = 1; i < NI; ++i) mx = fmaxf(mx, sc[i][g]);
    if (LPK == 16) mx = xor16_max(mx);
    mx = xor32_max(mx);
    mw[g] = mx;
    lw[g] = 0.f;
#pragma unroll
    for (int e = 0; e < DPL / 2; ++e) acc[g][e] = f32x2_t{0.f, 0.f};
  }
#pragma unroll
  for (int i = 0; i < NI; ++i) {
    const int key = key_base + i * KPI;
    float vf[DPL];
    Frag16<KVT>::unpack(vraw[i], vf);
#pragma unroll
    for (int g = 0; g < GROUP; ++g) {
      const float p = (key <= pos) ? expw(sc[i][g] - mw[g]) : 0.f;
      lw[g] += p;
#pragma unroll
      for (int e = 0; e < DPL / 2; ++e) acc[g][e] += f32x2_t{p, p} * f32x2_t{vf[2 * e], vf[2 * e + 1]};
    }
  }
  Q3A_STAMP_AT(a.stamp, stamp_wg, 3);
#pragma unroll
  for (int g = 0; g < GROUP; ++g) {
    if (LPK == 16) lw[g] = xor16_sum(lw[g]);
    lw[g] = xor32_sum(lw[g]);
    float af[DPL];
#pragma unroll
    for (int e = 0; e < DPL; ++e) {
      af[e] = (e & 1) ? acc[g][e >> 1].y : acc[g][e >> 1].x;
      if (LPK == 16) af[e] = xor16_sum(af[e]);
      af[e] = xor32_sum(af[e]);
    }
    if (lane == 0) { cm[wave][g] = mw[g]; cl[wave][g] = lw[g]; }
    if (kq == 0) {
#pragma unroll
      for (int e = 0; e < DPL; ++e) co[wave][g][sub * DPL + e] = af[e];
    }
  }
  __syncthreads();
  Q3A_STAMP_AT(a.stamp, stamp_wg, 4);
  if (wave < GROUP) {
    const int g = wave;
    float M = -INFINITY;
#pragma unroll
    for (int w = 0; w < DA_WAVES; ++w) M = fmaxf(M, cm[w][g]);
    float L = 0.f, o0 = 0.f, o1 = 0.f;
#pragma unroll
    for (int w = 0; w < DA_WAVES; ++w) {
      const float f = (cm[w][g] == -INFINITY) ? 0.f : expw(cm[w][g] - M);
      L += cl[w][g] * f;
      o0 += co[w][g][lane] * f;
      o1 += co[w][g][lane + 64] * f;
    }
    const size_t pi = pbase + (size_t)g * a.nsplit;
    if (lane == 0) { a.pm[pi] = M; a.pl[pi] = L; }
    a.po[pi * 128 + lane] = o0;
    a.po[pi * 128 + lane + 64] = o1;
  }
  Q3A_STAMP_AT(a.stamp, stamp_wg, 5);
}

struct DecodeAttnTail {
  const float* q_norm; const float* k_norm; float eps;
  float* pm; float* pl; float* po;
  float scale_div;
  Q3A_STAMP_FIELD
};
template <int GROUP, typename KVT>
__global__ __launch_bounds__(DA_WAVES * 64) void decode_attn_kernel(void* kcache, void* vcache, const int* pos, const float* qkv,
                                                                    const float* rope_cur, int nsplit, int n_q, int n_kv, int max_ctx,
                                                                    DecodeAttnTail t) {
  DecodeAttnArgs a{};
  a.kcache = kcache; a.vcache = vcache; a.pos = pos; a.qkv = qkv; a.rope_cur = rope_cur; a.nsplit = nsplit; a.n_q = n_q; a.n_kv = n_kv;
  a.max_ctx = max_ctx;
  a.q_norm = t.q_norm; a.k_norm = t.k_norm; a.eps = t.eps; a.pm = t.pm; a.pl = t.pl; a.po = t.po; a.scale_div = t.scale_div;
#ifdef Q3A_STAMP
  a.stamp = t.stamp;
#endif
  decode_attn_body<GROUP, KVT>(a, blockIdx.x, blockIdx.y, blockIdx.z);
}


template <bool B> struct BoolC { static constexpr bool value = B; };
#ifndef Q3A_DATTN_RING
#define Q3A_DATTN_RING 2
#endif
template <int GROUP, typename KVT, int TILE = 128, int RING_T = Q3A_DATTN_RING>
__global__ __launch_bounds__(DA_WAVES * 64) void decode_attn_batched_kernel(DecodeAttnArgs a) {
  constexpr int DPL = Frag16<KVT>::DPL;
  constexpr int LPK = 128 / DPL;
  constexpr int KPI = 64 / LPK;
  constexpr int NI = (TILE / DA_WAVES) / KPI;
  constexpr int KEYS_PER_WAVE = KPI * NI;
  constexpr bool DOT2 = sizeof(KVT) == 2;
  __shared__ float q_s[GROUP][128];
  __shared__ __attribute__((aligned(16))) KVT k_s[128];
  __shared__ __attribute__((aligned(16))) KVT v_s[128];
  __shared__ float cm[DA_WAVES][GROUP], cl[DA_WAVES][GROUP];
  __shared__ float co[DA_WAVES][GROUP][128];
  const int pos = a.pos[blockIdx.y];
  Q3A_ARG(a.qkv); Q3A_ARG(a.pos); Q3A_ARG(a.q_norm); Q3A_ARG(a.k_norm); Q3A_ARG(a.eps); Q3A_ARG(a.rope_cur); Q3A_ARG(a.kcache); Q3A_ARG(a.vcache);
  Q3A_ARG(a.n_q); Q3A_ARG(a.n_kv); Q3A_ARG(a.max_ctx); Q3A_ARG(a.scale_div); Q3A_ARG(a.out); Q3A_ARG(a.out16); Q3A_ARG(a.out_frag); Q3A_ARG(a.trim_prologue);
  const int kvh = blockIdx.x, s = blockIdx.y;
  const int tid = threadIdx.x, lane = tid & 63, wave = tid >> 6;
  const int stamp_wg = blockIdx.y * gridDim.x + blockIdx.x;
  Q3A_STAMP_AT(a.stamp, stamp_wg, 0);
  const int sub = lane % LPK, kq = lane / LPK;
  const int qkv_dim = (a.n_q + 2 * a.n_kv) * 128;
  const float* row = a.qkv + (size_t)s * qkv_dim;
  KVT* kc = reinterpret_cast<KVT*>(a.kcache) + ((size_t)s * a.n_kv + kvh) * (size_t)a.max_ctx * 128;
  KVT* vc = reinterpret_cast<KVT*>(a.vcache) + ((size_t)s * a.n_kv + kvh) * (size_t)a.max_ctx * 128;

  const int key_w = wave * KEYS_PER_WAVE + kq;
  constexpr int RING = DOT2 ? RING_T : 1;
  static_assert(RING >= 1 && RING <= 4 && NI >= 1, "ring depth / tile size");
  uint4 kr0[NI], vr0[NI], kr1[RING > 1 ? NI : 1], vr1[RING > 1 ? NI : 1], kr2[RING > 2 ? NI : 1], vr2[RING > 2 ? NI : 1], kr3[RING > 3 ? NI : 1], vr3[RING > 3 ? NI : 1];
  const int last_tile = a.max_ctx / TILE - 1;
  const size_t lane_off = (size_t)key_w * 128 + sub * DPL;
  auto load_tile = [&](int j, uint4 (&kr)[NI], uint4 (&vr)[NI], const bool trim = false, const int pos_row = 0) {
    const int t = j;
    if (!trim) {
      const size_t base = (size_t)min(t, last_tile) * (TILE * 128) + lane_off;
#pragma unroll
      for (int i = 0; i < NI; ++i) {
        kr[i] = ld_stream16(kc + base + (size_t)i * (KPI * 128));
        vr[i] = ld_stream16(vc + base + (size_t)i * (KPI * 128));
      }
    } else {
#pragma unroll
      for (int i = 0; i < NI; ++i) {
        const int key = min(t * TILE + key_w + i * KPI, pos_row);
        const size_t off = (size_t)key * 128 + sub * DPL;
        kr[i] = ld_stream16(kc + off);
        vr[i] = ld_stream16(vc + off);
      }
    }
  };
#ifndef Q3A_DATTN_TRIM
#define Q3A_DATTN_TRIM 2
#endif
  constexpr bool TRIM = Q3A_DATTN_TRIM != 0;
  const bool TRIM_PRO = Q3A_DATTN_TRIM >= 2 && a.trim_prologue != 0;
  load_tile(0, kr0, vr0);
  float x1 = 0.f, x2 = 0.f, nw1 = 0.f, nw2 = 0.f, c = 0.f, sn = 0.f;
  if (wave < GROUP + 2) {
    const int r = wave < GROUP ? kvh * GROUP + wave : (wave == GROUP ? a.n_q + kvh : a.n_q + a.n_kv + kvh);
    x1 = row[r * 128 + lane];
    x2 = row[r * 128 + lane + 64];
    if (wave <= GROUP) {
      const float* nw = wave < GROUP ? a.q_norm : a.k_norm;
      nw1 = nw[lane];
      nw2 = nw[lane + 64];
      c = a.rope_cur[(size_t)s * 128 + lane];
      sn = a.rope_cur[(size_t)s * 128 + 64 + lane];
    }
  }
  __builtin_amdgcn_sched_barrier(0);
  if constexpr (RING > 1) load_tile(1, kr1, vr1, TRIM_PRO, pos);
  if constexpr (RING > 2) load_tile(2, kr2, vr2, TRIM_PRO, pos);
  if constexpr (RING > 3) load_tile(3, kr3, vr3, TRIM_PRO, pos);
  __builtin_amdgcn_sched_barrier(0);
  Q3A_STAMP_AT(a.stamp, stamp_wg, 1);
// ... 148 lines not shown
  Q3A_STAMP_AT(a.stamp, stamp_wg, 3);
#pragma unroll
  for (int g = 0; g < GROUP; ++g) {
    float lw = lrun[g];
    if (LPK == 16) lw = xor16_sum(lw);
    lw = xor32_sum(lw);
    float af[DPL];
#pragma unroll
    for (int e = 0; e < DPL; ++e) {
      af[e] = (e & 1) ? acc[g][e >> 1].y : acc[g][e >> 1].x;
      if (LPK == 16) af[e] = xor16_sum(af[e]);
      af[e] = xor32_sum(af[e]);
    }
    if (lane == 0) { cm[wave][g] = mrun[g]; cl[wave][g] = lw; }
    if (kq == 0) {
#pragma unroll
      for (int e = 0; e < DPL; ++e) co[wave][g][sub * DPL + e] = af[e];
    }
  }
  __syncthreads();
  Q3A_STAMP_AT(a.stamp, stamp_wg, 4);
  float M = -INFINITY, L = 0.f, o0 = 0.f, o1 = 0.f;
  if (wave < GROUP) {
    const int g = wave;
#pragma unroll
    for (int w = 0; w < DA_WAVES; ++w) M = fmaxf(M, cm[w][g]);
#pragma unroll
    for (int w = 0; w < DA_WAVES; ++w) {
      const float f = (cm[w][g] == -INFINITY) ? 0.f : expw(cm[w][g] - M);
      L += cl[w][g] * f;
      o0 += co[w][g][lane] * f;
      o1 += co[w][g][lane + 64] * f;
    }
  }
  if (wave < GROUP) {
    const int g = wave;
    o0 /= L;
    o1 /= L;
    const int head = kvh * GROUP + g;
    if (a.out16) {
      const int k0 = head * 128 + lane;
      if (a.out_frag) {
        a.out16[skinny_frag_index(s, k0)] = (uint16_t)f32_to_bf16_bits(o0);
        a.out16[skinny_frag_index(s, k0 + 64)] = (uint16_t)f32_to_bf16_bits(o1);
      } else {
        a.out16[(size_t)s * a.n_q * 128 + k0] = (uint16_t)f32_to_bf16_bits(o0);
        a.out16[(size_t)s * a.n_q * 128 + k0 + 64] = (uint16_t)f32_to_bf16_bits(o1);
      }
    } else {
      a.out[(size_t)s * a.n_q * 128 + head * 128 + lane] = o0;
      a.out[(size_t)s * a.n_q * 128 + head * 128 + lane + 64] = o1;
    }
  }
  Q3A_STAMP_AT(a.stamp, stamp_wg, 5);
}

__global__ __launch_bounds__(128) void attn_combine_kernel(const float* __restrict__ pm, const float* __restrict__ pl,
                                                           const float* __restrict__ po, int nsplit, float* __restrict__ out,
                                                           uint16_t* __restrict__ out16, int n_q, int frag) {
  const size_t sh = blockIdx.x;
  const int d = threadIdx.x;
  float M = -INFINITY;
  for (int sp = 0; sp < nsplit; ++sp) M = fmaxf(M, pm[sh * nsplit + sp]);
  float L = 0.f, o = 0.f;
  for (int sp = 0; sp < nsplit; ++sp) {
    const float m = pm[sh * nsplit + sp];
    if (m == -INFINITY) continue;
    const float f = expf(m - M);
    L += pl[sh * nsplit + sp] * f;
    o += po[(sh * nsplit + sp) * 128 + d] * f;
  }
  if (out16) {
    const int s = (int)(sh / n_q), k = (int)(sh % n_q) * 128 + d;
    out16[frag ? skinny_frag_index(s, k) : sh * 128 + d] = (uint16_t)f32_to_bf16_bits(o / L);
  } else {
    out[sh * 128 + d] = o / L;
  }
}

}

const char* launch_decode_attn(const DecodeAttnArgs& a, int S, bool kv_f32, hipStream_t s) {
  if (S <= 0) return nullptr;
  if (a.nsplit <= 0 || (a.nsplit - 1) * dattn_keys_per_split(kv_f32) >= a.max_ctx) return "decode_attn: 1 .. ceil(max_ctx / keys per split) key splits";
  const int group = a.n_q / a.n_kv;
  dim3 grid(a.n_kv, S, a.nsplit), block(DA_WAVES * 64);
  DecodeAttnTail t{};
  t.q_norm = a.q_norm; t.k_norm = a.k_norm; t.eps = a.eps; t.pm = a.pm; t.pl = a.pl; t.po = a.po; t.scale_div = a.scale_div;
#ifdef Q3A_STAMP
  t.stamp = a.stamp;
#endif
#define Q3A_DA_ARGS a.kcache, a.vcache, a.pos, a.qkv, a.rope_cur, a.nsplit, a.n_q, a.n_kv, a.max_ctx, t
#define Q3A_DA(G)                                                                                   \
  do {                                                                                              \
    if (kv_f32) hipLaunchKernelGGL((decode_attn_kernel<G, float>), grid, block, 0, s, Q3A_DA_ARGS); \
    else hipLaunchKernelGGL((decode_attn_kernel<G, uint16_t>), grid, block, 0, s, Q3A_DA_ARGS);     \
  } while (0)
  if (group == 1) Q3A_DA(1);
  else if (group == 2) Q3A_DA(2);
  else if (group == 4) Q3A_DA(4);
  else return "decode_attn: GQA group must be 1, 2 or 4";
#undef Q3A_DA
#undef Q3A_DA_ARGS
  return nullptr;
}


const char* launch_decode_attn_batched(const DecodeAttnArgs& a, int S, bool kv_f32, hipStream_t s) {
  if (S <= 0) return nullptr;
  if (!a.out && !a.out16) return "decode_attn_batched: no output buffer";
  if (a.out16 && a.out_frag && S > 32) return "decode_attn_batched: fragment order holds at most 32 sequences";
  if (a.max_ctx % 128 != 0) return "decode_attn_batched: max_ctx must be a multiple of 128 (whole key tiles)";
  const int group = a.n_q / a.n_kv;
  dim3 grid(a.n_kv, S), block(DA_WAVES * 64);
#define Q3A_DAB(G)                                                                                          \
  do {                                                                                                      \
    if (kv_f32) hipLaunchKernelGGL((decode_attn_batched_kernel<G, float>), grid, block, 0, s, a);          \
    else hipLaunchKernelGGL((decode_attn_batched_kernel<G, uint16_t>), grid, block, 0, s, a);              \
  } while (0)
  if (group == 1) Q3A_DAB(1);
  else if (group == 2) Q3A_DAB(2);
  else if (group == 4) Q3A_DAB(4);
  else return "decode_attn_batched: GQA group must be 1, 2 or 4";
#undef Q3A_DAB
  return nullptr;
}

const char* launch_attn_combine(const float* pm, const float* pl, const float* po, int nsplit, int S, int n_q, float* out,
                                hipStream_t s, uint16_t* out16, bool frag) {
  if (S <= 0) return nullptr;
  if (frag && S > 32) return "attn_combine: fragment order holds at most 32 sequences";
  hipLaunchKernelGGL(attn_combine_kernel, dim3(S * n_q), dim3(128), 0, s, pm, pl, po, nsplit, out, out16, n_q, frag ? 1 : 0);
  return nullptr;
}

}
```

### qwen3_asr_rs_amd/csrc/k_gemv.hip

```cpp
#include <algorithm>
#include <type_traits>

#include "argmax.h"


namespace q3a {

int gemv_rows_per_wave(const GemvArgs& a) {
  const int logical = (a.mode == 2) ? a.N / 2 : a.N;
  if (logical >= 32768 && a.K <= 2048) return 4;
  if (logical >= 4096 || a.mode == 2) return 2;
  return 1;
}
int gemv_blocks(const GemvArgs& a) {
  const int pr = gemv_rows_per_wave(a);
  const int rows_per_wave = (a.mode == 2) ? pr / 2 : pr;
  const int logical = (a.mode == 2) ? a.N / 2 : a.N;
  return (logical + 4 * rows_per_wave - 1) / (4 * rows_per_wave);
}

namespace {

constexpr int ATTN_F_MAX = 1024;
struct AttnTables {
// ... 160 lines not shown
#pragma unroll
    for (int e = 0; e < 8; ++e) { ss += x[it][e] * x[it][e]; x[it][e] *= wv[e]; }
    if constexpr (YY) {
#pragma unroll
      for (int e = 0; e < 8; ++e) *yy += x[it][e] * x[it][e];
    }
  }
}
template <bool LP, int NB>
__device__ __forceinline__ ArgmaxAcc<LP> merge_wave_partials(float (*am_v)[NB], int (*am_i)[NB], float (*am_s)[NB], int b) {
  ArgmaxAcc<LP> r{am_v[0][b], am_i[0][b], LP ? am_s[0][b] : 0.f};
  for (int w = 1; w < 4; ++w) r.merge(am_v[w][b], am_i[w][b], LP ? am_s[w][b] : 0.f);
  return r;
}

template <int NB, int PR, bool LP>
__device__ __forceinline__ void gemv_epilogue(const GemvArgs& a, int g, const int (&prow)[PR], float (&acc)[PR][NB],
                                              float (*am_v)[NB], int (*am_i)[NB], float (*am_s)[NB]) {
  const int tid = threadIdx.x, lane = tid & 63, wave = tid >> 6;
  if (a.mode == 3) {
    ArgmaxAcc<LP> m[NB];
    float lv[LP ? PR : 1][NB];
#pragma unroll
    for (int i = 0; i < PR; ++i) {
      if constexpr (LP) {
#pragma unroll
        for (int b = 0; b < NB; ++b) lv[i][b] = -INFINITY;
      }
      if (prow[i] < 0) continue;
#pragma unroll
      for (int b = 0; b < NB; ++b) {
        float v = acc[i][b];
        if (a.bias) v += a.bias[prow[i]];
        if (lane == 0 && a.out) a.out[(size_t)b * a.ldo + prow[i]] = v;
        if (v > m[b].v) { m[b].v = v; m[b].i = prow[i]; }
        if constexpr (LP) lv[i][b] = v;
      }
    }
    if (lane == 0) {
#pragma unroll
      for (int b = 0; b < NB; ++b) {
        am_v[wave][b] = m[b].v; am_i[wave][b] = m[b].i;
        if constexpr (LP) {
          float ws = 0.f;
#pragma unroll
          for (int i = 0; i < PR; ++i) ws += lse_term(1.f, lv[i][b], m[b].v);
          am_s[wave][b] = ws;
        }
      }
    }
    __syncthreads();
    if (tid < NB) merge_wave_partials<LP, NB>(am_v, am_i, am_s, tid).store(a.part, tid, g >> 2);
    return;
  }
  if (lane != 0) return;
  if (a.mode != 2) {
#pragma unroll
    for (int i = 0; i < PR; ++i) {
      if (prow[i] < 0) continue;
      const int n = prow[i];
#pragma unroll
      for (int b = 0; b < NB; ++b) {
        float v = acc[i][b];
        if (a.bias) v += a.bias[n];
        if (a.mode == 1) v += a.resid[(size_t)b * a.ldo + n];
        a.out[(size_t)b * a.ldo + n] = v;
      }
    }
  } else {
#pragma unroll
    for (int i = 0; i + 1 < PR; i += 2) {
      if (prow[i] < 0) continue;
      const int j = g * (PR / 2) + (i >> 1);
#pragma unroll
      for (int b = 0; b < NB; ++b) {
        float gv = acc[i][b], uv = acc[i + 1][b];
        if (a.bias) { gv += a.bias[prow[i]]; uv += a.bias[prow[i + 1]]; }
        a.out[(size_t)b * a.ldo + j] = silu_sel(gv, a.fast_math != 0) * uv;
      }
    }
  }
}

template <int PR, int KI, bool RMS, bool ATTN, int MF, bool XL>
__device__ __forceinline__ void gemv1_body(const GemvArgs& a) {
  static_assert(!XL || !ATTN, "the merged attention vector already goes through LDS");
  constexpr bool XH = !RMS && !ATTN && KI > 4;
  constexpr bool XLDS = XL || XH;
  static_assert(!XH || KI % 2 == 0, "the hand-over stores unguarded: its rounds of 1024 columns must end at KI * 512");
  __shared__ __attribute__((aligned(16))) float x_lds[(ATTN || XLDS) ? KI * 512 : 4], xl_w[(XL && RMS) ? KI * 512 : 4];
  const int tid = threadIdx.x, lane = tid & 63, wave = tid >> 6;
  Q3A_STAMP_ENTRY(t_entry);
  const int K = a.K;
  const int g = blockIdx.x * 4 + wave;
  int prow[PR];
  gemv_rows<PR>(a, g, prow);
  bool kin[KI];
  int kk[KI];
#pragma unroll
  for (int it = 0; it < KI; ++it) {
    const int k = lane * 8 + it * 512;
    kin[it] = k < K;
    kk[it] = kin[it] ? k : 0;
  }
  float4 xr[KI][2], nr[RMS ? KI : 1][2];
  uint4 wq[KI][PR];
  constexpr int XLN = (KI + 1) / 2;
  float4 xl_rx[XLDS ? XLN : 1], xl_rw[(XL && RMS) ? XLN : 1];
  auto request_x = [&]() {
    if (ATTN) return;
    if constexpr (XLDS) {
#pragma unroll
      for (int j = 0; j < XLN; ++j) {
        const int k = (tid + j * 256) * 4, kc = k < K ? k : 0;
        xl_rx[j] = *reinterpret_cast<const float4*>(a.x + kc);
        if (RMS) xl_rw[j] = *reinterpret_cast<const float4*>(a.rms_w + kc);
      }
      return;
    }
#pragma unroll
    for (int it = 0; it < KI; ++it) {
      xr[it][0] = *reinterpret_cast<const float4*>(a.x + kk[it]);
      xr[it][1] = *reinterpret_cast<const float4*>(a.x + kk[it] + 4);
      if (RMS) {
        nr[it][0] = *reinterpret_cast<const float4*>(a.rms_w + kk[it]);
        nr[it][1] = *reinterpret_cast<const float4*>(a.rms_w + kk[it] + 4);
      }
    }
  };
  auto request_w = [&]() {
#pragma unroll
    for (int it = 0; it < KI; ++it)
#pragma unroll
      for (int i = 0; i < PR; ++i) {
        const int row = prow[i] >= 0 ? prow[i] : a.N - 1;
        wq[it][i] = ld_stream16(a.W + (size_t)row * K + kk[it]);
      }
  };
  constexpr int MCH = MF > 0 ? MF : 1;
  float mg_m[MCH], mg_l[MCH];
  float4 mg_o0[MCH], mg_o1[MCH];
  const int mg_k = lane * 8 + wave * 512;
  const bool mg_on = wave < KI && mg_k < K;
  if constexpr (ATTN && MF > 0) {
    const int kc = mg_k < K ? mg_k : 0;
    const int h = kc >> 7, d = kc & 127, ns = a.attn_nsplit, base = h * ns;
    typedef float __attribute__((ext_vector_type(4), aligned(4))) f4u_t;
#pragma unroll
    for (int j = 0; j < MCH; j += 4) {
      const f4u_t m4 = *reinterpret_cast<const f4u_t*>(a.attn_pm + base + j), l4 = *reinterpret_cast<const f4u_t*>(a.attn_pl + base + j);
#pragma unroll
      for (int e = 0; e < 4; ++e) {
        mg_m[j + e] = j + e < ns ? m4[e] : -INFINITY;
        mg_l[j + e] = j + e < ns ? l4[e] : 0.f;
      }
    }
#pragma unroll
    for (int j = 0; j < MCH; ++j) attn_partial_row8(a, base, j, d, mg_o0[j], mg_o1[j]);
    __builtin_amdgcn_sched_barrier(0);
  }
  if (RMS || XLDS) { request_x(); request_w(); } else { request_w(); request_x(); }
  if constexpr (ATTN && MF > 0) __builtin_amdgcn_sched_barrier(0);
  float bv[PR], rv[PR];
#pragma unroll
  for (int i = 0; i < PR; ++i) {
    const int n = prow[i] >= 0 ? prow[i] : 0;
    bv[i] = a.bias ? a.bias[n] : 0.f;
    rv[i] = a.mode == 1 ? a.resid[n] : 0.f;
  }
  __builtin_amdgcn_sched_barrier(0);
  Q3A_STAMP_AT(a.stamp, blockIdx.x, 1);
  Q3A_STAMP_PUT(a.stamp, blockIdx.x, 0, t_entry);
  Q3A_ARG(a.out); Q3A_ARG(a.fast_math);
  if (ATTN) Q3A_ARG(a.attn_fast_exp);
  if constexpr (ATTN && MF > 0) {
    if (mg_on) {
      const bool fast = a.attn_fast_exp != 0;
      float Mn = -INFINITY;
#pragma unroll
      for (int j = 0; j < MCH; ++j) Mn = fmaxf(Mn, mg_m[j]);
      float L = 0.f, v[8];
#pragma unroll
      for (int e = 0; e < 8; ++e) v[e] = 0.f;
#pragma unroll
      for (int j = 0; j < MCH; ++j) {
        const float f = fast ? __expf(mg_m[j] - Mn) : expf(mg_m[j] - Mn);
        L += mg_l[j] * f;
        v[0] += mg_o0[j].x * f; v[1] += mg_o0[j].y * f; v[2] += mg_o0[j].z * f; v[3] += mg_o0[j].w * f;
        v[4] += mg_o1[j].x * f; v[5] += mg_o1[j].y * f; v[6] += mg_o1[j].z * f; v[7] += mg_o1[j].w * f;
      }
      const float inv = 1.0f / L;
#pragma unroll
      for (int e = 0; e < 8; ++e) v[e] *= inv;
      *reinterpret_cast<float4*>(x_lds + mg_k) = make_float4(v[0], v[1], v[2], v[3]);
      *reinterpret_cast<float4*>(x_lds + mg_k + 4) = make_float4(v[4], v[5], v[6], v[7]);
    }
    __syncthreads();
  } else if constexpr (ATTN) {
    auto merge_pieces = [&](auto fast_c, auto ch_c) {
#pragma unroll
      for (int it = 0; it < KI; ++it) {
        if ((it & 3) == wave && kin[it]) {
          float v[8];
          attn_merge8_ch<decltype(fast_c)::value, decltype(ch_c)::value>(a, 0, kk[it], v);
          *reinterpret_cast<float4*>(x_lds + kk[it]) = make_float4(v[0], v[1], v[2], v[3]);
          *reinterpret_cast<float4*>(x_lds + kk[it] + 4) = make_float4(v[4], v[5], v[6], v[7]);
        }
      }
    };
    typedef std::integral_constant<int, 4> Ch4;
    typedef std::integral_constant<int, 8> Ch8;
    if (a.attn_fast_exp) {
      if (a.attn_nsplit <= 4) merge_pieces(std::true_type{}, Ch4{}); else merge_pieces(std::true_type{}, Ch8{});
    } else {
      if (a.attn_nsplit <= 4) merge_pieces(std::false_type{}, Ch4{}); else merge_pieces(std::false_type{}, Ch8{});
    }
    __syncthreads();
  }
  if constexpr (XLDS) {
#pragma unroll
    for (int j = 0; j < XLN; ++j) {
      const int k = (tid + j * 256) * 4;
      if (XH || k < KI * 512) {
        const float4 v = xl_rx[j];
        *reinterpret_cast<float4*>(x_lds + k) = make_float4(v.x, v.y, v.z, v.w);
        if (RMS) *reinterpret_cast<float4*>(xl_w + k) = xl_rw[j];
      }
    }
    __syncthreads();
  }
  if constexpr (ATTN || XLDS) {
#pragma unroll
    for (int it = 0; it < KI; ++it) {
      xr[it][0] = *reinterpret_cast<const float4*>(x_lds + kk[it]);
      xr[it][1] = *reinterpret_cast<const float4*>(x_lds + kk[it] + 4);
      if (XL && RMS) {
        nr[it][0] = *reinterpret_cast<const float4*>(xl_w + kk[it]);
        nr[it][1] = *reinterpret_cast<const float4*>(xl_w + kk[it] + 4);
      }
    }
  }
  Q3A_STAMP_AT(a.stamp, blockIdx.x, 2);
  float x[KI][8], acc[PR];
  float ss = 0.f;
#pragma unroll
  for (int it = 0; it < KI; ++it) {
    const float4 v0 = xr[it][0], v1 = xr[it][1];
    const float xv[8] = {v0.x, v0.y, v0.z, v0.w, v1.x, v1.y, v1.z, v1.w};
#pragma unroll
    for (int e = 0; e < 8; ++e) x[it][e] = (K == KI * 512 || kin[it]) ? xv[e] : 0.f;
    if (RMS) {
      const float4 w0 = nr[it][0], w1 = nr[it][1];
      const float wv[8] = {w0.x, w0.y, w0.z, w0.w, w1.x, w1.y, w1.z, w1.w};
#pragma unroll
      for (int e = 0; e < 8; ++e) { ss += x[it][e] * x[it][e]; x[it][e] *= wv[e]; }
    }
  }
#pragma unroll
  for (int i = 0; i < PR; ++i) acc[i] = 0.f;
#pragma unroll
  for (int it = 0; it < KI; ++it)
#pragma unroll
    for (int i = 0; i < PR; ++i) acc[i] = dot8(wq[it][i], x[it], acc[i]);
  if (wave == 0) asm volatile("" ::"v"(acc[0]));
  Q3A_STAMP_AT(a.stamp, blockIdx.x, 3);
  float rstd = 1.0f;
  if (RMS) rstd = rstd_of(wave_sum_fast(ss) / (float)K + a.eps, a.fast_math != 0);
#pragma unroll
  for (int i = 0; i < PR; ++i) acc[i] = wave_sum_fast(acc[i]) * rstd + bv[i];
  if (lane != 0) return;
  if (a.mode != 2) {
#pragma unroll
    for (int i = 0; i < PR; ++i)
      if (prow[i] >= 0) a.out[prow[i]] = acc[i] + rv[i];
  } else {
#pragma unroll
    for (int i = 0; i + 1 < PR; i += 2)
      if (prow[i] >= 0) a.out[g * (PR / 2) + (i >> 1)] = silu_sel(acc[i], a.fast_math != 0) * acc[i + 1];
  }
  Q3A_STAMP_AT(a.stamp, blockIdx.x, 4);
}

struct GemvTail {
  float* out; int fast_math;
  Q3A_STAMP_FIELD
};
struct GemvAttnTail {
  float* out; const float* bias; int attn_heads; int attn_fast_exp; int fast_math;
  Q3A_STAMP_FIELD
};
#ifdef Q3A_STAMP
#define Q3A_STAMP_COPY(dst, src) (dst).stamp = (src).stamp
#else
#define Q3A_STAMP_COPY(dst, src) do { } while (0)
#endif
template <int PR, int KI, bool RMS, bool ATTN, int MF = 0, bool XL = false>
__global__ __launch_bounds__(256) void gemv1_kernel(const uint16_t* W, const float* x, const float* rms_w, const float* bias,
                                                    const float* resid, int N, int K, int mode, float eps, GemvTail t) {
  static_assert(!ATTN, "the ATTN forms take the partials in their head");
  GemvArgs a{};
  a.W = W; a.x = x; a.rms_w = rms_w; a.bias = bias; a.resid = resid; a.N = N; a.K = K; a.mode = mode; a.eps = eps;
  a.out = t.out; a.fast_math = t.fast_math;
  Q3A_STAMP_COPY(a, t);
  gemv1_body<PR, KI, RMS, ATTN, MF, XL>(a);
}
template <int PR, int KI, bool RMS, bool ATTN, int MF = 0, bool XL = false>
__global__ __launch_bounds__(256) void gemv1_kernel(const float* attn_pm, const float* attn_pl, const float* attn_po, const uint16_t* W,
                                                    const float* resid, int N, int K, int attn_nsplit, int mode, GemvAttnTail t) {
  static_assert(ATTN && !RMS, "the plain forms take x and the norm weight in their head");
  GemvArgs a{};
  a.attn_pm = attn_pm; a.attn_pl = attn_pl; a.attn_po = attn_po; a.W = W; a.resid = resid; a.N = N; a.K = K; a.attn_nsplit = attn_nsplit;
  a.mode = mode;
  a.out = t.out; a.bias = t.bias; a.attn_heads = t.attn_heads; a.attn_fast_exp = t.attn_fast_exp; a.fast_math = t.fast_math;
  Q3A_STAMP_COPY(a, t);
  gemv1_body<PR, KI, RMS, ATTN, MF, XL>(a);
}

template <int PR, int KI, bool LP = false>
__device__ __forceinline__ void gemv1_head_block(const GemvArgs& a, int blk, float (&am_v)[4][1], int (&am_i)[4][1], float (*am_s)[1],
                                                 ArgmaxAcc<LP>& out) {
  const int tid = threadIdx.x, lane = tid & 63, wave = tid >> 6;
  const int g = blk * 4 + wave;
  int prow[PR];
  gemv_rows<PR>(a, g, prow);
  bool kin[KI];
  int kk[KI];
  lane_cols<KI>(lane, a.K, kin, kk);
  float4 xr[KI][2], nr[KI][2];
  uint4 wq[KI][PR];
  fetch_cols<KI>(a, kk, xr, nr);
  request_rows<KI, PR>(a, prow, kk, wq);
  float bv[PR];
#pragma unroll
  for (int i = 0; i < PR; ++i) bv[i] = a.bias ? a.bias[prow[i] >= 0 ? prow[i] : 0] : 0.f;
  __builtin_amdgcn_sched_barrier(0);
  float x[KI][8], acc[PR];
  float ss = 0.f;
  unpack_cols<KI>(a.K, kin, xr, nr, x, ss);
#pragma unroll
  for (int i = 0; i < PR; ++i) acc[i] = 0.f;
#pragma unroll
  for (int it = 0; it < KI; ++it)
#pragma unroll
    for (int i = 0; i < PR; ++i) acc[i] = dot8(wq[it][i], x[it], acc[i]);
  const float rstd = rstd_of(wave_sum_fast(ss) / (float)a.K + a.eps, a.fast_math != 0);
#pragma unroll
  for (int i = 0; i < PR; ++i) acc[i] = wave_sum_fast(acc[i]) * rstd + bv[i];
  ArgmaxAcc<LP> m;
#pragma unroll
  for (int i = 0; i < PR; ++i) {
    if (prow[i] < 0) continue;
    if (lane == 0 && a.out) a.out[prow[i]] = acc[i];
    if (acc[i] > m.v) { m.v = acc[i]; m.i = prow[i]; }
  }
  if (lane == 0) { am_v[wave][0] = m.v; am_i[wave][0] = m.i; }
  if constexpr (LP) {
    float ws = 0.f;
#pragma unroll
    for (int i = 0; i < PR; ++i) ws += prow[i] < 0 ? 0.f : lse_term(1.f, acc[i], m.v);
    if (lane == 0) am_s[wave][0] = ws;
  }
  __syncthreads();
  if (tid == 0) out = merge_wave_partials<LP, 1>(am_v, am_i, am_s, 0);
}

template <int PR, int KI, bool LP = false>
__global__ __launch_bounds__(256) void gemv1_head_kernel(const uint16_t* W, const float* x, const float* rms_w, const float* bias, float* out,
                                                         int N, int K, float eps, int fast_math, ArgmaxPartials part) {
  __shared__ float am_v[4][1];
  __shared__ int am_i[4][1];
  __shared__ float am_s[LP ? 4 : 1][1];
  GemvArgs a{};
  a.W = W; a.x = x; a.rms_w = rms_w; a.bias = bias; a.out = out; a.N = N; a.K = K; a.eps = eps; a.fast_math = fast_math; a.mode = 3;
  ArgmaxAcc<LP> r;
  gemv1_head_block<PR, KI, LP>(a, blockIdx.x, am_v, am_i, am_s, r);
  if (threadIdx.x == 0) r.store(part, 0, blockIdx.x);
}

struct LmHeadArgsDev {
  GemvArgs g;
  const int8_t* Wq; const float* qs; int qcols;
  float gamma;
  float* blk_lo; float* blk_hi; int n_blk;
  float* dbg;
};

__device__ __forceinline__ float dotq8(uint32_t lo, uint32_t hi, const float (&x)[8], float s) {
  f32x2_t a = f32x2_t{(float)(int8_t)lo, (float)(int8_t)(lo >> 8)} * f32x2_t{x[0], x[1]};
  a += f32x2_t{(float)(int8_t)(lo >> 16), (float)((int32_t)lo >> 24)} * f32x2_t{x[2], x[3]};
  a += f32x2_t{(float)(int8_t)hi, (float)(int8_t)(hi >> 8)} * f32x2_t{x[4], x[5]};
  a += f32x2_t{(float)(int8_t)(hi >> 16), (float)((int32_t)hi >> 24)} * f32x2_t{x[6], x[7]};
  return s + (a.x + a.y);
}

__global__ __launch_bounds__(256) void lm_head_quantize_kernel(const uint16_t* W, int N, int K, int cols, int8_t* Q, float* qs) {
  const int lane = threadIdx.x & 63, r = blockIdx.x * 4 + (threadIdx.x >> 6);
  if (r >= N) return;
  const uint16_t* w = W + (size_t)r * K;
  float m = 0.f;
  for (int k = lane; k < K; k += 64) m = fmaxf(m, fabsf(__uint_as_float((uint32_t)w[k] << 16)));
// ... 216 lines not shown
        x[0] = v0.x; x[1] = v0.y; x[2] = v0.z; x[3] = v0.w; x[4] = v1.x; x[5] = v1.y; x[6] = v1.z; x[7] = v1.w;
      }
      if (a.rms_w) {
        const float4 w0 = *reinterpret_cast<const float4*>(a.rms_w + k);
        const float4 w1 = *reinterpret_cast<const float4*>(a.rms_w + k + 4);
        const float wv[8] = {w0.x, w0.y, w0.z, w0.w, w1.x, w1.y, w1.z, w1.w};
#pragma unroll
        for (int e = 0; e < 8; ++e) { ss += x[e] * x[e]; x[e] *= wv[e]; }
      }
      *reinterpret_cast<float4*>(xs + (size_t)b * K + k) = make_float4(x[0], x[1], x[2], x[3]);
      *reinterpret_cast<float4*>(xs + (size_t)b * K + k + 4) = make_float4(x[4], x[5], x[6], x[7]);
    }
    if (a.rms_w) {
      ss = wave_sum_fast(ss);
      if (lane == 0) red[b][wave] = ss;
    }
  }
  __syncthreads();
  float acc[PR][NB];
#pragma unroll
  for (int i = 0; i < PR; ++i)
#pragma unroll
    for (int b = 0; b < NB; ++b) acc[i][b] = 0.f;
  auto fma_all = [&](const uint4 (&w)[PR], int k) {
#pragma unroll
    for (int b = 0; b < NB; ++b) {
      const float4 xa = *reinterpret_cast<const float4*>(xs + (size_t)b * K + k);
      const float4 xb = *reinterpret_cast<const float4*>(xs + (size_t)b * K + k + 4);
      const float x[8] = {xa.x, xa.y, xa.z, xa.w, xb.x, xb.y, xb.z, xb.w};
#pragma unroll
      for (int i = 0; i < PR; ++i) acc[i][b] = dot8(w[i], x, acc[i][b]);
    }
  };
#pragma unroll
  for (int it = 0; it < PF; ++it)
    if (kin[it]) fma_all(wq[it], kk[it]);
  for (int k = lane * 8 + PF * 512; k < K; k += 512) {
    uint4 w[PR];
#pragma unroll
    for (int i = 0; i < PR; ++i) w[i] = ld_w16(a, prow[i], k);
    fma_all(w, k);
  }
#pragma unroll
  for (int b = 0; b < NB; ++b) {
    float rstd = 1.0f;
    if (a.rms_w) rstd = rstd_of((red[b][0] + red[b][1] + red[b][2] + red[b][3]) / (float)K + a.eps, a.fast_math != 0);
#pragma unroll
    for (int i = 0; i < PR; ++i) acc[i][b] = wave_sum_fast(acc[i][b]) * rstd;
  }
  gemv_epilogue<NB, PR, LP>(a, g, prow, acc, am_v, am_i, am_s);
}

#define GEMV_PLAIN_ARGS(a) (a).W, (a).x, (a).rms_w, (a).bias, (a).resid, (a).N, (a).K, (a).mode, (a).eps, gemv_tail(a)
#define GEMV_ATTN_ARGS(a) (a).attn_pm, (a).attn_pl, (a).attn_po, (a).W, (a).resid, (a).N, (a).K, (a).attn_nsplit, (a).mode, gemv_attn_tail(a)
#define GEMV_HEAD_ARGS(a) (a).W, (a).x, (a).rms_w, (a).bias, (a).out, (a).N, (a).K, (a).eps, (a).fast_math, (a).part
GemvTail gemv_tail(const GemvArgs& a) {
  GemvTail t{};
  t.out = a.out; t.fast_math = a.fast_math;
  Q3A_STAMP_COPY(t, a);
  return t;
}
GemvAttnTail gemv_attn_tail(const GemvArgs& a) {
  GemvAttnTail t{};
  t.out = a.out; t.bias = a.bias; t.attn_heads = a.attn_heads; t.attn_fast_exp = a.attn_fast_exp; t.fast_math = a.fast_math;
  Q3A_STAMP_COPY(t, a);
  return t;
}

template <int PR, int KI>
void launch1k(const GemvArgs& a, hipStream_t s) {
  const dim3 grid(gemv_blocks(a)), block(256);
  if (a.attn_po) {
    if constexpr (KI <= 4) {
      if (a.attn_nsplit <= 4) { hipLaunchKernelGGL((gemv1_kernel<PR, KI, false, true, 4>), grid, block, 0, s, GEMV_ATTN_ARGS(a)); return; }
      if (a.attn_nsplit <= 8) { hipLaunchKernelGGL((gemv1_kernel<PR, KI, false, true, 8>), grid, block, 0, s, GEMV_ATTN_ARGS(a)); return; }
    }
    hipLaunchKernelGGL((gemv1_kernel<PR, KI, false, true>), grid, block, 0, s, GEMV_ATTN_ARGS(a));
  } else if (a.rms_w) {
    if (a.mode == 3) {
      if (a.part.sum) hipLaunchKernelGGL((gemv1_head_kernel<PR, KI, true>), grid, block, 0, s, GEMV_HEAD_ARGS(a));
      else hipLaunchKernelGGL((gemv1_head_kernel<PR, KI>), grid, block, 0, s, GEMV_HEAD_ARGS(a));
      return;
    }
    if constexpr (KI == 2) { hipLaunchKernelGGL((gemv1_kernel<PR, KI, true, false, 0, true>), grid, block, 0, s, GEMV_PLAIN_ARGS(a)); return; }
    hipLaunchKernelGGL((gemv1_kernel<PR, KI, true, false>), grid, block, 0, s, GEMV_PLAIN_ARGS(a));
  } else {
    hipLaunchKernelGGL((gemv1_kernel<PR, KI, false, false>), grid, block, 0, s, GEMV_PLAIN_ARGS(a));
  }
}
template <int PR>
void launch1(const GemvArgs& a, hipStream_t s) {
  if (a.K <= 1024) launch1k<PR, 2>(a, s);
  else if (a.K <= 2048) launch1k<PR, 4>(a, s);
  else if constexpr (PR < 4) {
    if (a.K <= 3072) launch1k<PR, 6>(a, s); else launch1k<PR, 12>(a, s);
  }
}
template <int NB, int PR, int PF>
void launchn(const GemvArgs& a, hipStream_t s) {
  if (a.part.sum) hipLaunchKernelGGL((gemvn_kernel<NB, PR, PF, true>), dim3(gemv_blocks(a)), dim3(256), (size_t)NB * a.K * sizeof(float), s, a);
  else hipLaunchKernelGGL((gemvn_kernel<NB, PR, PF>), dim3(gemv_blocks(a)), dim3(256), (size_t)NB * a.K * sizeof(float), s, a);
}

}

int lm_head_prune_blocks(const GemvArgs& g) { return (g.N + 15) / 16; }
const char* launch_lm_head_quantize(const uint16_t* W, int N, int K, int8_t* Q, float* qs, hipStream_t s) {
  const int cols = lm_head_q_cols(K);
  if (cols == 0 || K % 8 != 0) return "lm_head_quantize: hidden size beyond the one-sequence GEMV";
  if (hipMemsetAsync(Q, 0, (size_t)N * cols, s) != hipSuccess) return "lm_head_quantize: memset failed";
  hipLaunchKernelGGL(lm_head_quantize_kernel, dim3((N + 3) / 4), dim3(256), 0, s, W, N, K, cols, Q, qs);
  return nullptr;
}
const char* lm_head_prune_check(const LmHeadPruneArgs& a) {
  const GemvArgs& g = a.g;
  if (g.mode != 3 || !g.rms_w || !g.x || g.attn_po) return "lm_head_prune: needs the plain mode-3 GEMV with a fused norm";
  if (g.bias && !a.logit_bias) return "lm_head_prune: the only bias the bound covers is the logit bias (finite or -inf entries)";
  if (g.part.sum) return "lm_head_prune: token log-probabilities need every logit (the full GEMV)";
  if (gemv_rows_per_wave(g) != 4 || gemv_blocks(g) != lm_head_prune_blocks(g)) return "lm_head_prune: the GEMV does not run 16-row blocks here";
  if (g.K % 8 != 0 || a.qcols != lm_head_q_cols(g.K)) return "lm_head_prune: int8 row width does not match the hidden size";
  if (!a.Wq || !a.qs || !a.blk_lo || !a.blk_hi || !g.part.val) return "lm_head_prune: missing buffer";
  if (const char* e = argmax_partials_check(g.part, 1)) return e;
  return nullptr;
}
const char* launch_lm_head_approx(const LmHeadPruneArgs& a, hipStream_t s) {
  if (const char* e = lm_head_prune_check(a)) return e;
  const GemvArgs& g = a.g;
  const int n_blk = lm_head_prune_blocks(g);
  const dim3 grid((n_blk + 3) / 4), block(256);
  const double nu = (double)a.qcols * 0x1p-24;
  const LmHeadApproxTail t{g.eps, g.fast_math, (float)(nu / (1.0 - nu)) * (1.0f + 0x1p-20f), a.blk_lo, a.blk_hi, a.dbg};
#define LM_HEAD_APPROX_ARGS a.Wq, g.x, g.rms_w, a.qs, g.bias, g.N, g.K, a.qcols, n_blk, t
  if (a.g.bias) {
    if (a.qcols == 1024) hipLaunchKernelGGL(lm_head_approx_bias_kernel<2>, grid, block, 0, s, LM_HEAD_APPROX_ARGS);
    else hipLaunchKernelGGL(lm_head_approx_bias_kernel<4>, grid, block, 0, s, LM_HEAD_APPROX_ARGS);
  } else {
    if (a.qcols == 1024) hipLaunchKernelGGL(lm_head_approx_kernel<2>, grid, block, 0, s, LM_HEAD_APPROX_ARGS);
    else hipLaunchKernelGGL(lm_head_approx_kernel<4>, grid, block, 0, s, LM_HEAD_APPROX_ARGS);
  }
#undef LM_HEAD_APPROX_ARGS
  return nullptr;
}
int lm_head_rescore_groups(const GemvArgs& g, int n_cu) {
  const int nb = lm_head_prune_blocks(g);
  return std::min(nb, std::max(n_cu > 0 ? n_cu : 256, (nb + 255) / 256));
}
const char* launch_lm_head_rescore(const LmHeadPruneArgs& a, int groups, hipStream_t s) {
  if (const char* e = lm_head_prune_check(a)) return e;
  const GemvArgs& g = a.g;
  const int n_blk = lm_head_prune_blocks(g);
  if (groups < 1 || groups > g.part.stride || (n_blk + groups - 1) / groups > 256) return "lm_head_prune: bad rescore grid";
  const LmHeadRescoreTail t{g.bias, g.out, g.fast_math, g.part, a.stats};
#define LM_HEAD_RESCORE_ARGS a.blk_lo, a.blk_hi, g.W, g.x, g.rms_w, n_blk, g.N, g.K, g.eps, t
  if (a.qcols == 1024) hipLaunchKernelGGL((lm_head_rescore_kernel<4, 2>), dim3(groups), dim3(256), 0, s, LM_HEAD_RESCORE_ARGS);
  else hipLaunchKernelGGL((lm_head_rescore_kernel<4, 4>), dim3(groups), dim3(256), 0, s, LM_HEAD_RESCORE_ARGS);
#undef LM_HEAD_RESCORE_ARGS
  return nullptr;
}

const char* launch_gemv(const GemvArgs& a0, int NB, hipStream_t s) {
  if (a0.K % 8 != 0) return "gemv: K must be a multiple of 8";
  if (a0.K > 6144) return "gemv: K > 6144 unsupported";
  if (a0.mode == 2 && a0.N % 32 != 0) return "gemv: GLU needs N % 32 == 0";
  if (a0.mode == 3 && !a0.rms_w) return "gemv: mode 3 (the lm_head) needs the fused final norm";
  if (a0.mode == 3 && !a0.part.val) return "gemv: argmax partial buffer missing";
  if (const char* e = argmax_partials_check(a0.part, a0.mode == 3 ? gemv_blocks(a0) : 0)) return e;
  if (a0.part.sum && a0.mode != 3) return "gemv: log-sum partials need mode 3";
  if (a0.attn_po && (a0.K % 128 != 0 || a0.K != a0.attn_heads * 128)) return "gemv: attention-partial input needs K = heads*128";
  if (a0.attn_po && a0.rms_w) return "gemv: attention-partial input cannot be combined with a fused RMSNorm";
  if (a0.attn_po && (NB < 4 ? NB : 4) * a0.attn_heads * a0.attn_nsplit > ATTN_F_MAX) return "gemv: too many attention splits for the LDS scale table";
  const int pr = gemv_rows_per_wave(a0);
  const int nb_cap = (int)((64 * 1024) / ((size_t)a0.K * 4));
  int done = 0;
  while (done < NB) {
    GemvArgs a = a0;
    if (a0.x) a.x = a0.x + (size_t)done * a0.ldx;
    if (a0.out) a.out = a0.out + (size_t)done * a0.ldo;
    if (a0.resid) a.resid = a0.resid + (size_t)done * a0.ldo;
    a.part = a0.part.at(done);
    if (a0.attn_po) {
      const size_t adv = (size_t)done * a0.attn_heads * a0.attn_nsplit;
      a.attn_pm = a0.attn_pm + adv; a.attn_pl = a0.attn_pl + adv; a.attn_po = a0.attn_po + adv * 128;
    }
    int nb = NB - done;
    if (nb >= 4 && nb_cap >= 4) nb = 4;
    else if (nb >= 2 && nb_cap >= 2) nb = 2;
    else nb = 1;
    if (nb == 1) {
      if (pr == 4) launch1<4>(a, s); else if (pr == 2) launch1<2>(a, s); else launch1<1>(a, s);
    } else if (nb == 2) {
      if (pr == 4) launchn<2, 4, 2>(a, s); else if (pr == 2) launchn<2, 2, 4>(a, s); else launchn<2, 1, 6>(a, s);
    } else {
      if (pr == 4) launchn<4, 4, 2>(a, s); else if (pr == 2) launchn<4, 2, 4>(a, s); else launchn<4, 1, 6>(a, s);
    }
    done += nb;
  }
  return nullptr;
}

}
```

### qwen3_asr_rs_amd/csrc/kernels.h

```cpp
#pragma once
#include <hip/hip_runtime.h>
#include <stdint.h>

#include <atomic>

#ifndef Q3A_STAMP_FIELD
#ifdef Q3A_STAMP
#define Q3A_STAMP_FIELD unsigned long long* stamp = nullptr;
#else
#define Q3A_STAMP_FIELD
#endif
#endif

namespace q3a {

struct ArgmaxPartials {
  float* val = nullptr;
  int* idx = nullptr;
  float* sum = nullptr;
  int stride = 0;
  ArgmaxPartials at(size_t rows) const {
    const size_t o = rows * stride;
    return {val ? val + o : nullptr, idx ? idx + o : nullptr, sum ? sum + o : nullptr, stride};
  }
};
inline const char* argmax_partials_check(const ArgmaxPartials& p, int n_part) {
  if (!p.val != !p.idx) return "argmax partials: val and idx go together";
  if (p.sum && !p.val) return "argmax partials: the log-sum channel needs val and idx";
  if (p.val && p.stride < n_part) return "argmax partials: buffer too small";
  return nullptr;
}

struct RowHeadArgs {
  const float* x; int ldx;
  const int* rows; int M;
  const float* norm_w; float eps;
  const uint16_t* W; int N; int K;
  int planes;
  uint16_t* xn;
  ArgmaxPartials part;
  float* logits; size_t ldl;
};
int align_rows_padded(int M);
const char* launch_head_rows_norm(const RowHeadArgs& a, hipStream_t s);
struct AlignHeadArgs : RowHeadArgs {
  int* classes;
};
int align_head_parts(int N);
const char* launch_align_head(const AlignHeadArgs& a, hipStream_t s);
struct ScoreHeadArgs : RowHeadArgs {
  const int* targets;
  float* tgt_logit;
  float* lp;
  int* top_id; float* top_lp;
  const float* bias;
};
const char* launch_score_head(const ScoreHeadArgs& a, hipStream_t s);

struct GemmEpilogue {
  float* out = nullptr;
  uint16_t* out16 = nullptr;
  int ldo = 0;
  const float* bias = nullptr;
  int act = 0;
  const float* resid = nullptr;
  const int* rowmap = nullptr;
  const float* addend = nullptr;
  int addend_period = 1;
  ArgmaxPartials part;
  Q3A_STAMP_FIELD
};
const char* launch_gemm(const float* X, int lda, const uint16_t* W, int M, int N, int K, const GemmEpilogue& ep,
                        bool glu, bool split, hipStream_t s);
const char* launch_conv3x3s2_gemm(const float* X, int imgs, int H, int Wd, int C, const uint16_t* Wt, int Cout,
                                  const GemmEpilogue& ep, bool split, hipStream_t s);
void launch_gemm_ref(const float* X, const uint16_t* W, float* Y, int M, int N, int K, hipStream_t s);
const char* launch_gemm16(const uint16_t* X, int lda, const uint16_t* W, int M, int N, int K, const GemmEpilogue& ep,
                          bool glu, hipStream_t s);
const char* launch_conv3x3s2_gemm16(const uint16_t* X, const uint16_t* zero_page, int imgs, int H, int Wd, int C,
                                    const uint16_t* Wt, int Cout, const GemmEpilogue& ep, hipStream_t s);
bool gemm256_eligible(int M, int N, int K);
const char* launch_gemm16_small(const uint16_t* X, int lda, const uint16_t* W, int M, int N, int K, const GemmEpilogue& ep,
                                bool glu, hipStream_t s);
struct Knobs {
  std::atomic<int> gemm256_min_tiles{128};
  std::atomic<int> gemm256_persist{1};
  std::atomic<int> gemm256_group_m{0};
  std::atomic<int> dattn_batched_min_wgs{128};
  std::atomic<int> decode_group_size{0};
  std::atomic<int> decode_parallel_groups{1};
  std::atomic<int> fuse_qkrope{1};
  std::atomic<int> skinny_q{1};
  std::atomic<int> eos_run_ahead{1};
  std::atomic<int> skinny_glu_hp3{1};
  std::atomic<int> lm_head_prune{1};
  std::atomic<int> layer_taps{0};
  std::atomic<int> poison_attn_partials{0};
};
Knobs& knobs();
const char* launch_gemm256(const uint16_t* X, int lda, const uint16_t* W, int M, int N, int K, const GemmEpilogue& ep,
                           bool glu, hipStream_t s);
const char* launch_conv3x3s2_gemm256(const uint16_t* X, const uint16_t* zero_page, int imgs, int H, int Wd, int C,
                                     const uint16_t* Wt, int Cout, const GemmEpilogue& ep, hipStream_t s);
const char* launch_to_bf16(const float* x, uint16_t* y, size_t n, hipStream_t s);
const char* launch_from_bf16(const uint16_t* x, float* y, size_t n, hipStream_t s);

struct MelBatch {
  const float* pcm;
  const int64_t* pcm_off;
  const int64_t* n_samples;
  const int64_t* mel_off;
  const int* n_frames;
  float* mel;
  unsigned* gmax_key;
};
const char* launch_mel(const MelBatch& mb, int B, int max_frames, const float* dft ,
                       const float* filt_t , hipStream_t s);

struct ChunkTable {
  const int* chunk_utt;
  const int* chunk_frame0;
};
const char* launch_conv1(const float* mel, const int64_t* mel_off, const int* n_frames, const ChunkTable& ct,
                         int n_chunks, int n_mels, int chunk_frames, const float* w ,
                         const float* b, int Cout, float* out, hipStream_t s, uint16_t* out16 = nullptr);

const char* launch_layernorm(const float* x, const float* w, const float* b, float* y, int rows, int D, float eps,
                             hipStream_t s, uint16_t* y16 = nullptr);
const char* launch_rmsnorm(const float* x, const float* w, float* y, int rows, int D, float eps, hipStream_t s,
                           uint16_t* y16 = nullptr);

struct AttnSeg {
  int q_row0;
  int len;
  int64_t kv_off;
};
struct AttnArgs {
  const float* q; int q_rs;
  const uint16_t* q16;
  const void* k; const void* v; int64_t kv_hs; int kv_rs;
  float* o; int o_rs;
  uint16_t* o16;
  const AttnSeg* segs; int n_segs; int max_len;
  int n_kv_heads;
  float scale_div;
};
const char* launch_attn_enc(const AttnArgs& a, hipStream_t s);
const char* launch_attn_prefill(const AttnArgs& a, int group, bool kv_f32, hipStream_t s);
const char* launch_fattn_enc(const AttnArgs& a, hipStream_t s);
const char* launch_fattn_prefill(const AttnArgs& a, int group, hipStream_t s);

const char* launch_embed(const int* ids, int rows, const uint16_t* embed, int H, int skip_id, float* out, hipStream_t s);
struct RopeKvArgs {
  float* qkv;
  const int* row_seq;
  const int* row_pos;
  const float* q_norm; const float* k_norm; float eps;
  const float* cos_t; const float* sin_t;
  void* kcache; void* vcache;
  int n_q, n_kv, max_ctx;
  uint16_t* q16;
};
const char* launch_qknorm_rope_kv(const RopeKvArgs& a, int rows, bool kv_f32, hipStream_t s);
int gemm256_split_rows(int M, int N);
const char* launch_gemm256_qkrope(const uint16_t* X, int lda, const uint16_t* W, int M, int K, const float* bias,
                                  const RopeKvArgs& a, hipStream_t s);
const char* launch_gather_rows(const float* src, const int* row_idx, int n, int D, float* dst, hipStream_t s);
const char* launch_scatter_rows(const float* src, const int* dst_row, int n, int D, float* dst, hipStream_t s);

struct GemvArgs {
  const float* x; int ldx;
  const float* rms_w;
  float eps;
  const uint16_t* W; int N; int K;
  const float* bias;
  int mode;
  float* out; int ldo;
  const float* resid;
  ArgmaxPartials part;
  const float* attn_pm; const float* attn_pl; const float* attn_po; int attn_nsplit; int attn_heads;
  int attn_fast_exp;
  int fast_math;
  Q3A_STAMP_FIELD
};
const char* launch_gemv(const GemvArgs& a, int NB, hipStream_t s);
constexpr int GEMV_ATTN_MAX_TABLE = 1024;
int gemv_blocks(const GemvArgs& a);
int gemv_rows_per_wave(const GemvArgs& a);

struct LmHeadPruneArgs {
  GemvArgs g;
  const int8_t* Wq; int qcols;
  const float* qs;
  float* blk_lo; float* blk_hi;
  float* dbg;
  int* stats;
  int logit_bias;
};
inline int lm_head_q_cols(int hidden) { return hidden <= 1024 ? 1024 : hidden <= 2048 ? 2048 : 0; }
const char* launch_lm_head_quantize(const uint16_t* W, int N, int K, int8_t* Q, float* qs, hipStream_t s);
int lm_head_prune_blocks(const GemvArgs& g);
int lm_head_rescore_groups(const GemvArgs& g, int n_cu);
const char* lm_head_prune_check(const LmHeadPruneArgs& a);
const char* launch_lm_head_approx(const LmHeadPruneArgs& a, hipStream_t s);
const char* launch_lm_head_rescore(const LmHeadPruneArgs& a, int groups, hipStream_t s);

struct SkinnyArgs {
  const float* x; int ldx; int S;
  const uint16_t* x16;
  int x16_frag;
  int out16_frag;
  const float* rms_w; float eps;
  const uint16_t* W; int N; int K;
  const float* bias;
  int mode;
  float* out; int ldo;
  uint16_t* out16;
  const float* resid;
  const uint16_t* xw16f; const float* ss_parts; int ss_nparts;
  const float* next_w; uint16_t* next_xw16f; float* next_ss;
  int qsplit;
  int qs_halves;
  int glu_hp3;
  int n_cu;
  int fast_math;
  Q3A_STAMP_FIELD
};
struct NextNormOut {
  const float* next_w;
  uint16_t* next_xw16f;
  float* next_ss;
  int nparts;
  long group_stride_x, group_stride_ss;
  int group_size;
};
const char* launch_skinny(const SkinnyArgs& a, bool split, hipStream_t s);
const char* skinny_init();
__host__ __device__ inline size_t skinny_frag_index(int s, int k) {
  return ((((size_t)(k >> 5) * 2 + (s >> 4)) * 4 + ((k >> 3) & 3)) * 16 + (s & 15)) * 8 + (k & 7);
}

struct DecodeAttnArgs {
  const float* qkv;
  const int* pos;
  const float* q_norm; const float* k_norm; float eps;
  const float* rope_cur;
  void* kcache; void* vcache;
  float* pm; float* pl;
  float* po;
  int nsplit;
  int n_q, n_kv, max_ctx;
  float scale_div;
  float* out;
  uint16_t* out16;
  int out_frag;
  int trim_prologue;
  Q3A_STAMP_FIELD
};
#ifndef Q3A_DATTN_SPLIT_KEYS
#define Q3A_DATTN_SPLIT_KEYS 128
#endif
constexpr int DATTN_KEYS_PER_SPLIT_BF16 = Q3A_DATTN_SPLIT_KEYS, DATTN_KEYS_PER_SPLIT_F32 = 128;
inline int dattn_keys_per_split(bool kv_f32) { return kv_f32 ? DATTN_KEYS_PER_SPLIT_F32 : DATTN_KEYS_PER_SPLIT_BF16; }
const char* launch_decode_attn(const DecodeAttnArgs& a, int S, bool kv_f32, hipStream_t s);
const char* launch_decode_attn_batched(const DecodeAttnArgs& a, int S, bool kv_f32, hipStream_t s);
const char* launch_attn_combine(const float* pm, const float* pl, const float* po, int nsplit, int S, int n_q, float* out,
                                hipStream_t s, uint16_t* out16 = nullptr, bool frag = false);

struct StepCommit {
  int* next_tok;
  int* out_ids;
  int out_stride;
  float* out_lp;
  int* step_count;
  int* pos;
  uint8_t* done;
  int* n_done;
  int n_seq;
  int* host_progress;
  const uint16_t* embed; int H;
  float* x_next;
  int eos0, eos1;
  const float* cos_t; const float* sin_t;
  float* rope_cur;
  NextNormOut nn;
};
struct StepCommitMsgs { const char *null_arg, *shape, *rope, *groups; };
#define Q3A_STEP_COMMIT_MSGS(who) \
  q3a::StepCommitMsgs { who ": null argument", who ": bad shape", who ": rope_cur needs the tables", who ": more than 32 sequences need group strides" }
inline const char* step_commit_check(const StepCommit& c, int S, const StepCommitMsgs& m, bool fed_only = false) {
  if (!c.next_tok || !c.embed || !c.x_next) return m.null_arg;
  if (c.H < 4 || c.H % 4 != 0) return m.shape;
  if (c.nn.next_w && S > 32 && (c.nn.group_stride_x <= 0 || c.nn.group_stride_ss <= 0)) return m.groups;
  if (fed_only) return nullptr;
  if (!c.out_ids || !c.step_count || !c.pos || !c.done) return m.null_arg;
  if (c.out_stride < 1) return m.shape;
  if (c.rope_cur && (!c.cos_t || !c.sin_t)) return m.rope;
  return nullptr;
}
struct FinalizeArgs {
  ArgmaxPartials part;
  int n_part;
  int V;
  int advance;
  StepCommit c;
};
const char* launch_argmax_partials(const float* logits, int V, int S, const ArgmaxPartials& p, int nblk, hipStream_t s);
const char* launch_argmax_finalize(const FinalizeArgs& a, int S, hipStream_t s);
const char* launch_set_tokens(const int* tok, int S, const StepCommit& c, hipStream_t s);

struct DraftAcceptArgs {
  int n_seq;
  const int* draft; const int* draft_off;
  const int* prompt_len;
  const int* top_id; const float* top_lp;
  int* accepted;
  StepCommit c;
};
const char* launch_draft_accept(const DraftAcceptArgs& a, hipStream_t s);

constexpr int BEAM_MAX_W = 8;
constexpr int BEAM_CHUNK = 2048;
constexpr int KV_REORDER_SLICES = 8;
inline int beam_topk_chunks(int V) { return (V + BEAM_CHUNK - 1) / BEAM_CHUNK; }
struct BeamTopkArgs {
  const float* logits; int S; int V; int W;
  float* cand_val; int* cand_idx;
  float* part_max; float* part_sum;
  int* out_ids; float* out_lp;
};
const char* launch_beam_topk(const BeamTopkArgs& a, hipStream_t s);
enum { BEAM_ST_ROUNDS = 0, BEAM_ST_COPIES = 1, BEAM_ST_KV_ROWS = 2, BEAM_ST_FINISHED = 3, BEAM_ST_ALL_DONE = 4, BEAM_ST_LAUNCHES = 5, BEAM_ST_COUNT = 8 };
struct BeamAdvanceArgs {
  int U, W;
  const int* topk_ids; const float* topk_lp;
  float* score; uint8_t* finished;
  int* parent;
  int* token;
  int* feed;
  int* hist_parent; int* hist_token; float* hist_lp; int hist_cap;
  int* state;
  const int* pos; const int* lo; int hi_bias;
  int* host_progress;
  int eos0, eos1;
};
const char* launch_beam_advance(const BeamAdvanceArgs& a, hipStream_t s);
// ... 40 lines not shown
```

### qwen3_asr_rs_amd/csrc/selftest.cpp

```cpp
#include <cmath>
#include <cstring>

#include "engine_internal.h"
#include "sample_rng.h"

using namespace q3a;

namespace {

void use_device(int device) {
  if (int n_dev = 0; hipGetDeviceCount(&n_dev) != hipSuccess || n_dev == 0) fail("no HIP device available");
  HIPCHK(hipSetDevice(device));
}
DevBuf room(size_t bytes) { DevBuf b; b.ensure(bytes); return b; }
template <class T> DevBuf to_device(const T* src, size_t n) {
  DevBuf b = room(n * sizeof(T));
  HIPCHK(hipMemcpy(b.p, src, n * sizeof(T), hipMemcpyHostToDevice));
  return b;
}
template <class T> DevBuf to_device(const std::vector<T>& v) { return to_device(v.data(), v.size()); }
template <class T> void to_host(T* dst, const DevBuf& b, size_t n) { HIPCHK(hipMemcpy(dst, b.p, n * sizeof(T), hipMemcpyDeviceToHost)); }
template <class T> std::vector<T> to_host(const DevBuf& b, size_t n) { std::vector<T> v(n); to_host(v.data(), b, n); return v; }
void finish() { HIPCHK(hipDeviceSynchronize()); HIPCHK(hipGetLastError()); }

// ... 296 lines not shown
  }
  Q3A_CATCH(nullptr)
}

int32_t q3a_selftest_gemv_launch(int32_t device, int32_t pruned, const uint16_t* w, int32_t N, int32_t K, const float* x, const float* rms_w, float eps,
                                 const float* bias, int32_t mode, const float* resid, const float* attn_pm, const float* attn_pl, const float* attn_po,
                                 int32_t attn_nsplit, int32_t attn_heads, float* out, int32_t* out_state) {
  Q3A_TRY(nullptr)
  const char* what = "q3a_selftest_gemv_launch";
  if (!w || N < 1 || K < 8 || K % 8 != 0 || K > 6144 || mode < 0 || mode > 3 || (pruned != 0 && pruned != 1)) fail(std::string(what) + ": bad argument");
  const bool attn = attn_po != nullptr;
  if (attn ? (x || rms_w || !attn_pm || !attn_pl || attn_nsplit < 1 || attn_heads < 1 || K != attn_heads * 128 ||
              (long)attn_heads * attn_nsplit > GEMV_ATTN_MAX_TABLE) : (!x || attn_pm || attn_pl))
    fail(std::string(what) + ": x alone, or the three partial arrays with K = heads * 128 alone");
  if (mode == 2 && N % 32 != 0) fail(std::string(what) + ": GLU needs N % 32 == 0");
  if ((mode == 1) != (resid != nullptr)) fail(std::string(what) + ": the residual goes with mode 1");
  if (mode == 3 ? (!rms_w || !out_state) : (!out || pruned)) fail(std::string(what) + ": mode 3 needs the norm weight and out_state, the other modes out");
  if (pruned && out) fail(std::string(what) + ": the pruned argmax stores no logits");
  use_device(device);
  const size_t n_out = mode == 2 ? (size_t)N / 2 : (size_t)N;
  const DevBuf dW = to_device(w, (size_t)N * K);
  DevBuf dX, dG, dB, dR, dPm, dPl, dPo;
  auto padded = [&](const float* src) {
    std::vector<float> v(6144 + 8, NAN);
    memcpy(v.data(), src, (size_t)K * 4);
    return to_device(v);
  };
  if (x) dX = padded(x);
  if (rms_w) dG = padded(rms_w);
  if (bias) dB = to_device(bias, (size_t)N);
  if (resid) dR = to_device(resid, (size_t)N);
  if (attn) {
    const size_t ns = (size_t)attn_heads * attn_nsplit;
    std::vector<float> pm(ns + 8, NAN), pl(ns + 8, NAN);
    memcpy(pm.data(), attn_pm, ns * 4); memcpy(pl.data(), attn_pl, ns * 4);
    dPm = to_device(pm); dPl = to_device(pl); dPo = to_device(attn_po, ns * 128);
  }
  Guarded dO;
  if (out) dO = Guarded(out, n_out * 4);
  GemvArgs g{};
  g.x = dX.as<float>(); g.ldx = K; g.rms_w = dG.as<float>(); g.eps = eps; g.W = dW.as<uint16_t>(); g.N = N; g.K = K; g.bias = dB.as<float>();
  g.mode = mode; g.out = dO.as<float>(); g.ldo = (int)n_out; g.resid = dR.as<float>();
  g.attn_pm = dPm.as<float>(); g.attn_pl = dPl.as<float>(); g.attn_po = dPo.as<float>(); g.attn_nsplit = attn_nsplit; g.attn_heads = attn_heads;
  g.attn_fast_exp = 0; g.fast_math = 0;
  if (mode != 3) {
    KCHK(launch_gemv(g, 1, nullptr));
    finish();
    dO.fetch(out, "output");
  } else {
    int n_part = gemv_blocks(g);
    const DevBuf dPv = room((size_t)n_part * 4), dPi = room((size_t)n_part * 4);
    g.part = ArgmaxPartials{dPv.as<float>(), dPi.as<int>(), nullptr, n_part};
    DevBuf dQ, dQs, dLo, dHi;
    if (pruned) {
      LmHeadPruneArgs pa{};
      pa.g = g; pa.qcols = lm_head_q_cols(K); pa.logit_bias = bias ? 1 : 0;
      if (pa.qcols == 0) fail(std::string(what) + ": hidden size beyond the pruned argmax");
      const size_t nb4 = ((size_t)lm_head_prune_blocks(g) + 3) / 4 * 4;
      dQ = room((size_t)N * pa.qcols); dQs = room((size_t)N * 16); dLo = room(nb4 * 4); dHi = room(nb4 * 4);
      pa.Wq = dQ.as<int8_t>(); pa.qs = dQs.as<float>(); pa.blk_lo = dLo.as<float>(); pa.blk_hi = dHi.as<float>();
      KCHK(lm_head_prune_check(pa));
      KCHK(launch_lm_head_quantize(g.W, N, K, dQ.as<int8_t>(), dQs.as<float>(), nullptr));
      n_part = lm_head_rescore_groups(g, 0);
      KCHK(launch_lm_head_approx(pa, nullptr));
      KCHK(launch_lm_head_rescore(pa, n_part, nullptr));
    } else {
      KCHK(launch_gemv(g, 1, nullptr));
    }
    constexpr int STRIDE = 4, STEP = 2, POS = 5;
    const DevBuf dTok = to_device(std::vector<int>(1, -1)), dIds = to_device(std::vector<int>(STRIDE, -1)), dSc = to_device(std::vector<int>(1, STEP));
    const DevBuf dPos = to_device(std::vector<int>(1, POS)), dDone = to_device(std::vector<uint8_t>(1, 0)), dXn = room((size_t)K * 4);
    FinalizeArgs f{};
    f.part = g.part; f.n_part = n_part; f.V = N; f.advance = 1;
    f.c = bare_commit(1, dTok, dIds.as<int>(), STRIDE, nullptr, dSc, dPos, dDone, g.W, K, dXn.as<float>(), -1, -1);
    KCHK(launch_argmax_finalize(f, 1, nullptr));
    finish();
    if (out) dO.fetch(out, "output");
    const std::vector<int> ids = to_host<int>(dIds, STRIDE);
    out_state[0] = to_host<int>(dTok, 1)[0]; out_state[1] = ids[STEP]; out_state[2] = to_host<int>(dSc, 1)[0]; out_state[3] = to_host<int>(dPos, 1)[0];
  }
  Q3A_CATCH(nullptr)
}

int32_t q3a_selftest_decode_attn_launch(int32_t device, int32_t kv_f32, const float* qkv, int32_t pos, const float* q_norm, const float* k_norm, float eps,
                                        const float* rope_cur, void* kcache, void* vcache, int32_t n_q, int32_t n_kv, int32_t max_ctx, int32_t nsplit,
                                        float scale_div, float* pm, float* pl, float* po) {
  Q3A_TRY(nullptr)
  const char* what = "q3a_selftest_decode_attn_launch";
  if (!qkv || !q_norm || !k_norm || !rope_cur || !kcache || !vcache || !pm || !pl || !po || n_q < 1 || n_kv < 1 || n_q % n_kv != 0 || max_ctx < 1 ||
      nsplit < 1 || !(scale_div > 0.f))
    fail(std::string(what) + ": bad argument");
  const int keys = dattn_keys_per_split(kv_f32 != 0);
  if (pos < 0 || pos >= max_ctx || pos >= nsplit * keys) fail(std::string(what) + ": pos outside the cache or beyond the last split");
  use_device(device);
  const size_t eb = kv_f32 ? 4 : 2, n_cache = (size_t)n_kv * max_ctx * 128, ns = (size_t)n_q * nsplit;
  const DevBuf dQkv = to_device(qkv, (size_t)(n_q + 2 * n_kv) * 128), dQn = to_device(q_norm, 128), dKn = to_device(k_norm, 128);
  const DevBuf dRope = to_device(rope_cur, 128), dPos = to_device(std::vector<int>(1, pos));
  const Guarded dK(kcache, n_cache * eb), dV(vcache, n_cache * eb), dPm(pm, ns * 4), dPl(pl, ns * 4), dPo(po, ns * 128 * 4);
  DecodeAttnArgs a{};
  a.qkv = dQkv.as<float>(); a.pos = dPos.as<int>(); a.q_norm = dQn.as<float>(); a.k_norm = dKn.as<float>(); a.eps = eps; a.rope_cur = dRope.as<float>();
  a.kcache = dK.as<void>(); a.vcache = dV.as<void>(); a.pm = dPm.as<float>(); a.pl = dPl.as<float>(); a.po = dPo.as<float>();
  a.nsplit = nsplit; a.n_q = n_q; a.n_kv = n_kv; a.max_ctx = max_ctx; a.scale_div = scale_div;
  KCHK(launch_decode_attn(a, 1, kv_f32 != 0, nullptr));
  finish();
  dK.fetch(kcache, "key cache"); dV.fetch(vcache, "value cache"); dPm.fetch(pm, "split maxima"); dPl.fetch(pl, "split sums"); dPo.fetch(po, "split outputs");
  Q3A_CATCH(nullptr)
}

int32_t q3a_selftest_draft_accept(int32_t device, int32_t S, const int32_t* draft_ids, const int32_t* draft_off, const int32_t* prompt_lens,
                                  const int32_t* top_ids, const float* top_lp, int32_t out_stride, const uint16_t* embed, int32_t V, int32_t H,
                                  const float* norm_w, int32_t group_size, const float* cos_t, const float* sin_t, int32_t max_pos,
                                  int32_t* accepted, int32_t* out_ids, float* out_lp, int32_t* state, float* x_next, float* rope_cur,
                                  uint16_t* nn_x, float* nn_ss) {
  Q3A_TRY(nullptr)
  const char* what = "q3a_selftest_draft_accept";
  if (S < 1 || !draft_off || !prompt_lens || !top_ids || !embed || !cos_t || !sin_t || !accepted || !out_ids || !state || !x_next || !rope_cur)
    fail(std::string(what) + ": bad argument");
  if (out_stride < 1 || V < 1 || H < 64 || H % 64 != 0 || max_pos < 1) fail(std::string(what) + ": bad shape");
  if (group_size < 1 || group_size > 32) fail(std::string(what) + ": group_size must lie in [1, 32]");
  if (norm_w && (!nn_x || !nn_ss)) fail(std::string(what) + ": norm_w needs nn_x and nn_ss");
  if (draft_off[0] != 0) fail(std::string(what) + ": draft_off[0] must be 0");
  const size_t Sz = S;
  for (size_t s = 0; s < Sz; ++s) {
    const int n = draft_off[s + 1] - draft_off[s];
    if (n < 0 || (n > 0 && !draft_ids)) fail(std::string(what) + ": bad draft offsets");
    if (prompt_lens[s] < 1 || prompt_lens[s] + n >= max_pos) fail(std::string(what) + ": a position outside the RoPE tables");
  }
  const size_t nd = draft_off[S], M = nd + Sz;
  for (size_t r = 0; r < M; ++r)
    if (top_ids[r] < 0 || top_ids[r] >= V) fail(std::string(what) + ": a head id outside the embedding table");
  use_device(device);
  const int groups = (S + group_size - 1) / group_size, nparts = H / 16;
  const size_t nnx = (size_t)groups * 32 * H, nns = (size_t)groups * nparts * 32;
  std::vector<int> dr(draft_ids, draft_ids + nd);
  dr.resize(nd + 4, 0);
  const DevBuf dDr = to_device(dr), dOff = to_device(draft_off, Sz + 1), dPl = to_device(prompt_lens, Sz), dTop = to_device(top_ids, M);
  DevBuf dTlp;
  if (top_lp) dTlp = to_device(top_lp, M);
  const DevBuf dAcc = room(Sz * 8), dTok = room(Sz * 4), dSc = to_device(std::vector<int>(Sz, -7)), dPos = to_device(std::vector<int>(Sz, -7));
  const Guarded gIds(out_ids, Sz * out_stride * 4);
  Guarded gLp;
  if (top_lp && out_lp) gLp = Guarded(out_lp, Sz * out_stride * 4);
  const DevBuf dDone = to_device(std::vector<uint8_t>(Sz, 0)), dNd = to_device(std::vector<int>(16, 0)), dProg = to_device(std::vector<int>(16, 0));
  const DevBuf dEmb = to_device(embed, (size_t)V * H), dCos = to_device(cos_t, (size_t)max_pos * 64), dSin = to_device(sin_t, (size_t)max_pos * 64);
  const Guarded gX(x_next, Sz * H * 4), gRope(rope_cur, Sz * 128 * 4);
  DevBuf dW;
  Guarded gNx, gNs;
  if (norm_w) { dW = to_device(norm_w, (size_t)H); gNx = Guarded(nn_x, nnx * 2); gNs = Guarded(nn_ss, nns * 4); }
  DraftAcceptArgs a{};
  a.n_seq = S; a.draft = dDr.as<int>(); a.draft_off = dOff.as<int>(); a.prompt_len = dPl.as<int>();
  a.top_id = dTop.as<int>(); a.top_lp = top_lp ? dTlp.as<float>() : nullptr; a.accepted = dAcc.as<int>();
  StepCommit& c = a.c;
  c = bare_commit(S, dTok, gIds.as<int>(), out_stride, gLp.b.p ? gLp.as<float>() : nullptr, dSc, dPos, dDone, dEmb.as<uint16_t>(), H, gX.as<float>(), kEos0, kEos1);
  c.n_done = dNd.as<int>(); c.host_progress = dProg.as<int>();
  c.cos_t = dCos.as<float>(); c.sin_t = dSin.as<float>(); c.rope_cur = gRope.as<float>();
  if (norm_w) {
    c.nn.next_w = dW.as<float>(); c.nn.next_xw16f = gNx.as<uint16_t>(); c.nn.next_ss = gNs.as<float>(); c.nn.nparts = nparts;
    c.nn.group_stride_x = (long)32 * H; c.nn.group_stride_ss = (long)nparts * 32; c.nn.group_size = group_size;
  }
  KCHK(launch_draft_accept(a, nullptr));
  finish();
  to_host(accepted, dAcc, Sz * 2);
  gIds.fetch(out_ids, "out_ids");
  if (gLp.b.p) gLp.fetch(out_lp, "out_lp");
  gX.fetch(x_next, "x_next");
  gRope.fetch(rope_cur, "rope_cur");
  if (norm_w) { gNx.fetch(nn_x, "nn_x"); gNs.fetch(nn_ss, "nn_ss"); }
  to_host(state, dTok, Sz);
  to_host(state + Sz, dSc, Sz);
  to_host(state + 2 * Sz, dPos, Sz);
  const std::vector<uint8_t> dn = to_host<uint8_t>(dDone, Sz);
  for (size_t s = 0; s < Sz; ++s) state[3 * Sz + s] = dn[s];
  to_host(state + 4 * Sz, dNd, 1);
  to_host(state + 4 * Sz + 1, dProg, 2);
  Q3A_CATCH(nullptr)
}

int32_t q3a_selftest_gemm(int32_t device, int32_t M, int32_t N, int32_t K, int32_t split, float* max_abs_err,
                          float* ref_abs_max) {
  Q3A_TRY(nullptr)
  use_device(device);
  Lcg rnd{12345u};
  GemmCase c(rnd, M, N, K, false);
  GemmEpilogue ep; ep.out = c.dY.as<float>(); ep.ldo = N;
  KCHK(launch_gemm(c.dX.as<float>(), K, c.dW.as<uint16_t>(), M, N, K, ep, false, split != 0, nullptr));
// ... 97 lines not shown
```

Baseline: 495.9 audio-seconds/sec.

## Split o-proj by kv-head pairs and fold partials into norm-fused GLU gemv

For batch-1 decode, attention now uses finer key splits (32/64 keys with 4 waves) so that short contexts spread across more workgroups. A new o-proj kernel combines the split partials per head group and writes partial projection vectors. The gate/up gemv then sums those vectors with the residual while applying RMSNorm, so the separate o-proj residual pass is dropped. This adds a kernel variant and partial buffers and raises the minimum split count, and it changes the order of floating-point summation.

```diff
diff --git a/include/q3asr.h b/include/q3asr.h
--- a/include/q3asr.h
+++ b/include/q3asr.h
@@ -235,6 +235,13 @@
 int32_t q3a_selftest_decode_attn_launch(int32_t device, int32_t kv_f32, const float* qkv, int32_t pos, const float* q_norm, const float* k_norm, float eps,
                                         const float* rope_cur, void* kcache, void* vcache, int32_t n_q, int32_t n_kv, int32_t max_ctx, int32_t nsplit,
                                         float scale_div, float* pm, float* pl, float* po);
+int32_t q3a_selftest_decode_attn_split_launch(int32_t device, int32_t kv_f32, int32_t keys_per_split, const float* qkv, int32_t pos, const float* q_norm,
+                                              const float* k_norm, float eps, const float* rope_cur, void* kcache, void* vcache, int32_t n_q, int32_t n_kv,
+                                              int32_t max_ctx, int32_t nsplit, float scale_div, float* pm, float* pl, float* po);
+int32_t q3a_selftest_oproj_head_launch(int32_t device, const uint16_t* w, int32_t N, int32_t K, const float* bias, const float* attn_pm, const float* attn_pl,
+                                       const float* attn_po, int32_t attn_nsplit, int32_t attn_heads, int32_t n_parts, float* y_part);
+int32_t q3a_selftest_gemv_parts_launch(int32_t device, const uint16_t* w, int32_t N, int32_t K, const float* x, const float* rms_w, float eps,
+                                       const float* bias, const float* x_parts, int32_t n_parts, float* out, float* x_out);
 int32_t q3a_gemm256_split_rows(int32_t M, int32_t N);
 
 #ifdef __cplusplus
diff --git a/qwen3_asr_rs_amd/_lib.py b/qwen3_asr_rs_amd/_lib.py
--- a/qwen3_asr_rs_amd/_lib.py
+++ b/qwen3_asr_rs_amd/_lib.py
@@ -24,6 +24,7 @@
     "q3a_set_repetition", "q3a_selftest_repeat",
     "q3a_selftest_gemm_launch", "q3a_selftest_qkrope_launch", "q3a_gemm256_split_rows",
     "q3a_selftest_gemv_launch", "q3a_selftest_decode_attn_launch",
+    "q3a_selftest_decode_attn_split_launch", "q3a_selftest_oproj_head_launch", "q3a_selftest_gemv_parts_launch",
     "q3a_prefill_draft", "q3a_transcribe_draft_batch_ptrs", "q3a_draft_next_round", "q3a_selftest_draft_accept",
 ]
 
@@ -160,6 +161,9 @@
         "q3a_selftest_qkrope_launch": (i32, [i32, i32, i32, P, i32, P, i32, i32, P, P, P, P, P, P, C.c_float, P, P, i32, i32, i32, i32, i32, P, P, P]),
         "q3a_selftest_gemv_launch": (i32, [i32, i32, P, i32, i32, P, P, C.c_float, P, i32, P, P, P, P, i32, i32, P, P]),
         "q3a_selftest_decode_attn_launch": (i32, [i32, i32, P, i32, P, P, C.c_float, P, P, P, i32, i32, i32, i32, C.c_float, P, P, P]),
+        "q3a_selftest_decode_attn_split_launch": (i32, [i32, i32, i32, P, i32, P, P, C.c_float, P, P, P, i32, i32, i32, i32, C.c_float, P, P, P]),
+        "q3a_selftest_oproj_head_launch": (i32, [i32, P, i32, i32, P, P, P, P, i32, i32, i32, P]),
+        "q3a_selftest_gemv_parts_launch": (i32, [i32, P, i32, i32, P, P, C.c_float, P, P, i32, P, P]),
         "q3a_gemm256_split_rows": (i32, [i32, i32]),
         "q3a_prefill_draft": (i32, [P, i32p, i32p, i32p, i32p, i32, i32p, i32p, f32p]),
         "q3a_transcribe_draft_batch_ptrs": (i32, [P, C.POINTER(P), i64p, i32, i32p, i32, i32p, i32p, i32, i32, i32, i32p, i32, i32p, i32p]),
@@ -168,6 +172,8 @@
                                             i32p, i32p, f32p, i32p, f32p, f32p, P, f32p]),
     }
     for name, (res, args) in sig.items():
+        if os.environ.get("Q3A_LIB") and not hasattr(lib, name):
+            continue
         fn = getattr(lib, name)
         fn.restype = res
         fn.argtypes = args
diff --git a/qwen3_asr_rs_amd/csrc/engine.cpp b/qwen3_asr_rs_amd/csrc/engine.cpp
--- a/qwen3_asr_rs_amd/csrc/engine.cpp
+++ b/qwen3_asr_rs_amd/csrc/engine.cpp
@@ -66,6 +66,7 @@
     {"eos_run_ahead", "Q3A_EOS_RUN_AHEAD", &Knobs::eos_run_ahead},
     {"skinny_glu_hp3", "Q3A_SKINNY_GLU_HP3", &Knobs::skinny_glu_hp3},
     {"lm_head_prune", "Q3A_LM_HEAD_PRUNE", &Knobs::lm_head_prune},
+    {"oproj_by_head", "Q3A_OPROJ_BY_HEAD", &Knobs::oproj_by_head},
     {"layer_taps", "Q3A_DEBUG_LAYER_TAPS", &Knobs::layer_taps},
     {"poison_attn_partials", nullptr, &Knobs::poison_attn_partials},
 };
@@ -99,9 +100,9 @@
   const std::vector<hipEvent_t>& join_ev; const hipEvent_t& fork_ev; const int& n_cu; int* const& host_prog_dev;
   std::vector<ProfEvent>* const& prof; Taps& taps;
   const int8_t* const& lm_q; const float* const& lm_qs; const int& lm_q_cols;
-  const int &B, &max_ctx, &max_new, &gsize, &live_nsplit_, &attn_nsplit, &min_P_, &part_stride, &beam_w_;
+  const int &B, &max_ctx, &max_new, &gsize, &live_nsplit_, &live_kps_, &attn_nsplit, &min_P_, &part_stride, &beam_w_;
   const size_t& kv_layer_elems; const bool& head_logits_;
-  const int &k_parallel_groups, &k_skinny_q, &k_dattn_batched_min_wgs, &k_skinny_glu_hp3, &k_lm_head_prune;
+  const int &k_parallel_groups, &k_skinny_q, &k_dattn_batched_min_wgs, &k_skinny_glu_hp3, &k_lm_head_prune, &k_oproj_by_head;
   const bool& logit_bias_on_;
   const bool& sampling_on_;
   const bool& repetition_on_;
@@ -121,6 +122,7 @@
   DevBuf part_sum, out_lp;
   DevBuf blk_lo, blk_hi;
   DevBuf prune_stats;
+  DevBuf o_part, x_mid;
   DevBuf attn_pm, attn_pl, attn_po, nn_x, nn_ss;
   DevBuf rope_cur, rope_cos, rope_sin;
   DevBuf n_done, forced_tok;
@@ -132,7 +134,7 @@
   DevBuf draft_accepted;
   template <class Self, class F> static void each_buf(Self& s, F&& f) {
     for (auto* b : {&s.kcache, &s.vcache, &s.x_dec, &s.d_pos, &s.next_tok, &s.out_ids, &s.step_count, &s.done, &s.s_ln, &s.s_qkv, &s.s_ctx, &s.s_act, &s.logits,
-                    &s.part_val, &s.part_idx, &s.part_sum, &s.out_lp, &s.blk_lo, &s.blk_hi, &s.prune_stats, &s.attn_pm, &s.attn_pl, &s.attn_po, &s.nn_x, &s.nn_ss,
+                    &s.part_val, &s.part_idx, &s.part_sum, &s.out_lp, &s.blk_lo, &s.blk_hi, &s.prune_stats, &s.o_part, &s.x_mid, &s.attn_pm, &s.attn_pl, &s.attn_po, &s.nn_x, &s.nn_ss,
                     &s.rope_cur, &s.rope_cos, &s.rope_sin, &s.n_done, &s.forced_tok,
                     &s.beam_cand_val, &s.beam_cand_idx, &s.beam_part_max, &s.beam_part_sum, &s.beam_topk_ids, &s.beam_topk_lp, &s.beam_score, &s.beam_finished,
                     &s.beam_parent, &s.beam_token, &s.beam_feed, &s.beam_hist_parent, &s.beam_hist_token, &s.beam_hist_lp, &s.beam_state, &s.beam_lo,
@@ -341,6 +343,7 @@
     da.rope_cur = rope_cur.as<float>() + (size_t)s0 * 128;
     da.pm = attn_pm.as<float>() + (size_t)s0 * d.n_q * attn_nsplit; da.pl = attn_pl.as<float>() + (size_t)s0 * d.n_q * attn_nsplit;
     da.po = attn_po.as<float>() + (size_t)s0 * d.n_q * attn_nsplit * 128; da.nsplit = live_nsplit_;
+    da.keys_per_split = live_kps_;
     da.n_q = d.n_q; da.n_kv = d.n_kv; da.max_ctx = max_ctx; da.scale_div = sqrtf((float)d.head_dim);
     da.q_norm = wf(l.q_norm); da.k_norm = wf(l.k_norm);
     da.kcache = (uint8_t*)kc_layer(li) + (size_t)s0 * kv_seq; da.vcache = (uint8_t*)vc_layer(li) + (size_t)s0 * kv_seq;
@@ -350,6 +353,20 @@
       g.x = x; g.rms_w = wf(l.in_ln); g.out = qkv;
       run(pj.qkv, g);
       timed(Q3A_KC_DECODE_ATTN, 0, [&] { KCHK(launch_decode_attn(da, S, kv_f32(), ks)); });
+      if (live_kps_ > 0) {
+        OprojHeadArgs oh{};
+        oh.pm = da.pm; oh.pl = da.pl; oh.po = da.po; oh.nsplit = live_nsplit_;
+        oh.W = pj.o.W; oh.N = pj.o.N; oh.K = pj.o.K; oh.bias = pj.o.bias; oh.n_parts = d.n_kv / 2; oh.y_part = o_part.as<float>();
+        timed(pj.o.kclass, pj.o.bytes, [&] { KCHK(launch_oproj_head(oh, ks)); });
+        GemvArgs u = gemv_args(pj.gu);
+        u.x = x; u.rms_w = wf(l.post_ln); u.out = s_act_g(grp);
+        u.x_parts = oh.y_part; u.x_nparts = oh.n_parts; u.x_out = x_mid.as<float>();
+        run(pj.gu, u);
+        GemvArgs dn = gemv_args(pj.down);
+        dn.x = s_act_g(grp); dn.out = x; dn.resid = u.x_out;
+        run(pj.down, dn);
+        return;
+      }
       GemvArgs o = gemv_args(pj.o);
       if (std::min(S, 4) * d.n_q * live_nsplit_ <= GEMV_ATTN_MAX_TABLE) {
         o.attn_pm = da.pm; o.attn_pl = da.pl; o.attn_po = da.po;
@@ -429,6 +446,10 @@
     run_head(1);
   }
 
+  bool oproj_by_head() const {
+    return k_oproj_by_head != 0 && B == 1 && !precise() && d.n_q == 2 * d.n_kv && d.n_kv % 2 == 0 && d.n_kv / 2 <= GEMV_X_PARTS_MAX && d.hidden <= 1024;
+  }
+  int fine_keys_per_split(int keys) const { return oproj_by_head() ? dattn_fine_keys_per_split(keys) : 0; }
   bool uses_key_splits() const {
     if (B <= kGemvMaxSeq) return true;
     const int ng = n_groups(B);
@@ -534,7 +555,7 @@
   size_t kv_layer_elems = 0;
 
   int gsize = 32;
-  int k_parallel_groups = 1, k_skinny_q = 1, k_dattn_batched_min_wgs = 128, k_skinny_glu_hp3 = 1, k_lm_head_prune = 1;
+  int k_parallel_groups = 1, k_skinny_q = 1, k_dattn_batched_min_wgs = 128, k_skinny_glu_hp3 = 1, k_lm_head_prune = 1, k_oproj_by_head = 1;
   std::vector<hipStream_t> chain_streams;
   std::vector<hipEvent_t> join_ev;
   hipEvent_t fork_ev = nullptr;
@@ -542,6 +563,7 @@
   static constexpr size_t kGraphCacheMax = 16;
   std::vector<std::pair<std::string, hipGraphExec_t>> graph_cache;
   int pos_hi_ = 0, live_nsplit_ = 0;
+  int live_kps_ = 0;
   int min_P_ = 0;
 
   hipStream_t up_stream = nullptr;
@@ -567,8 +589,8 @@
   int rep_ngram_ = 0;
 
   DecodeStep step{StepView{d, L, opts, arena, arena_flags, stream, chain_streams, join_ev, fork_ev, n_cu, host_prog_dev, prof, taps, lm_q, lm_qs, lm_q_cols,
-                           B, max_ctx, max_new, gsize, live_nsplit_, attn_nsplit, min_P_, part_stride, beam_w(), kv_layer_elems, head_logits(),
-                           k_parallel_groups, k_skinny_q, k_dattn_batched_min_wgs, k_skinny_glu_hp3, k_lm_head_prune, logit_bias_on_, sampling_on_, repetition_on_}};
+                           B, max_ctx, max_new, gsize, live_nsplit_, live_kps_, attn_nsplit, min_P_, part_stride, beam_w(), kv_layer_elems, head_logits(),
+                           k_parallel_groups, k_skinny_q, k_dattn_batched_min_wgs, k_skinny_glu_hp3, k_lm_head_prune, k_oproj_by_head, logit_bias_on_, sampling_on_, repetition_on_}};
 
   bool precise() const { return step.precise(); }
   bool token_lp() const { return step.token_lp(); }
@@ -1039,6 +1061,7 @@
       k_dattn_batched_min_wgs = kn.dattn_batched_min_wgs.load();
       k_skinny_glu_hp3 = kn.skinny_glu_hp3.load();
       k_lm_head_prune = kn.lm_head_prune.load();
+      k_oproj_by_head = kn.oproj_by_head.load();
     }
     const size_t ng = (size_t)step.n_groups(b);
     step.nn_x.ensure(ng * 32 * H * 2); step.nn_ss.ensure((size_t)ng * (H / 8) * 32 * 4);
@@ -1055,6 +1078,10 @@
       step.blk_lo.ensure(nblk4 * 4); step.blk_hi.ensure(nblk4 * 4);
     }
     attn_nsplit = (max_ctx + dattn_keys_per_split(kv_f32()) - 1) / dattn_keys_per_split(kv_f32());
+    if (step.oproj_by_head()) {
+      attn_nsplit = std::max(attn_nsplit, OPROJ_HEAD_MAX_SPLITS);
+      step.o_part.ensure((size_t)(d.n_kv / 2) * H * 4); step.x_mid.ensure(H * 4);
+    }
     {
       const size_t n_stat = (size_t)b * d.n_q * attn_nsplit;
       step.attn_pm.ensure((n_stat + 8) * 4); step.attn_pl.ensure((n_stat + 8) * 4);
@@ -1392,8 +1419,8 @@
       for (int i = 0; i < 8; ++i) { h ^= (v >> (8 * i)) & 0xff; h *= 1099511628211ull; }
     });
     char buf[256];
-    snprintf(buf, sizeof(buf), "%d.%d.%d.%d.%d.%d.%d.%d.%d.%d.b%d.lb%d.sm%d.rp%d/%d/%d/%d/%p/%016llx", B, gsize, k_parallel_groups, k_skinny_q,
-             k_dattn_batched_min_wgs, k_skinny_glu_hp3, k_lm_head_prune, (int)(min_P_ < 256), (int)head_logits(), (int)token_lp(), beam_w(), (int)logit_bias_on_, (int)sampling_on_, (int)repetition_on_, live_nsplit_,
+    snprintf(buf, sizeof(buf), "%d.%d.%d.%d.%d.%d.%d.%d.%d.%d.%d.b%d.lb%d.sm%d.rp%d/%d.%d/%d/%d/%p/%016llx", B, gsize, k_parallel_groups, k_skinny_q,
+             k_dattn_batched_min_wgs, k_skinny_glu_hp3, k_lm_head_prune, k_oproj_by_head, (int)(min_P_ < 256), (int)head_logits(), (int)token_lp(), beam_w(), (int)logit_bias_on_, (int)sampling_on_, (int)repetition_on_, live_nsplit_, live_kps_,
              max_ctx, max_new, (const void*)arena, (unsigned long long)h);
     return buf;
   }
@@ -1450,7 +1477,9 @@
     const bool eager = !opts.use_graph || prof;
     const int kps = dattn_keys_per_split(kv_f32());
     for (int i = 0; i < n; ++i) {
-      live_nsplit_ = step.uses_key_splits() ? std::min(attn_nsplit, pos_hi_ / kps + 1) : attn_nsplit;
+      live_kps_ = step.fine_keys_per_split(pos_hi_ + 1);
+      live_nsplit_ = live_kps_ > 0 ? pos_hi_ / live_kps_ + 1
+                     : step.uses_key_splits() ? std::min(attn_nsplit, pos_hi_ / kps + 1) : attn_nsplit;
       if (eager) enqueue_step();
       else HIPCHK(hipGraphLaunch(graph_for_step(), stream));
       ++pos_hi_;
diff --git a/qwen3_asr_rs_amd/csrc/k_dattn.hip b/qwen3_asr_rs_amd/csrc/k_dattn.hip
--- a/qwen3_asr_rs_amd/csrc/k_dattn.hip
+++ b/qwen3_asr_rs_amd/csrc/k_dattn.hip
@@ -31,21 +31,21 @@
 #endif
 constexpr int DA_WAVES = Q3A_DA_WAVES;
 
-template <int GROUP, typename KVT>
+template <int GROUP, typename KVT, int SPLIT_KEYS, int WAVES>
 __device__ __forceinline__ void decode_attn_body(const DecodeAttnArgs& a, const int kvh, const int s, const int sp) {
+  static_assert(WAVES >= GROUP + 2, "one wave per q head, one for k, one for v");
   constexpr int DPL = Frag16<KVT>::DPL;
   constexpr int LPK = 128 / DPL;
   constexpr int KPI = 64 / LPK;
-  constexpr int SPLIT_KEYS = sizeof(KVT) == 2 ? DATTN_KEYS_PER_SPLIT_BF16 : DATTN_KEYS_PER_SPLIT_F32;
-  constexpr int NI = (SPLIT_KEYS / DA_WAVES) / KPI;
+  constexpr int NI = (SPLIT_KEYS / WAVES) / KPI;
   constexpr int KEYS_PER_WAVE = KPI * NI;
-  constexpr int KEYS_PER_SPLIT = KEYS_PER_WAVE * DA_WAVES;
-  static_assert(KEYS_PER_SPLIT == (sizeof(KVT) == 2 ? DATTN_KEYS_PER_SPLIT_BF16 : DATTN_KEYS_PER_SPLIT_F32), "split size");
+  constexpr int KEYS_PER_SPLIT = KEYS_PER_WAVE * WAVES;
+  static_assert(NI >= 1 && KEYS_PER_SPLIT == SPLIT_KEYS, "split size");
   __shared__ float q_s[GROUP][128];
   __shared__ __attribute__((aligned(16))) KVT k_s[128];
   __shared__ __attribute__((aligned(16))) KVT v_s[128];
-  __shared__ float cm[DA_WAVES][GROUP], cl[DA_WAVES][GROUP];
-  __shared__ float co[DA_WAVES][GROUP][128];
+  __shared__ float cm[WAVES][GROUP], cl[WAVES][GROUP];
+  __shared__ float co[WAVES][GROUP][128];
   const int pos = a.pos[s];
   Q3A_ARG(a.q_norm); Q3A_ARG(a.k_norm); Q3A_ARG(a.eps); Q3A_ARG(a.pm); Q3A_ARG(a.pl); Q3A_ARG(a.po); Q3A_ARG(a.scale_div); Q3A_ARG(pos);
   const int tid = threadIdx.x, lane = tid & 63, wave = tid >> 6;
@@ -199,10 +199,10 @@
     const int g = wave;
     float M = -INFINITY;
 #pragma unroll
-    for (int w = 0; w < DA_WAVES; ++w) M = fmaxf(M, cm[w][g]);
+    for (int w = 0; w < WAVES; ++w) M = fmaxf(M, cm[w][g]);
     float L = 0.f, o0 = 0.f, o1 = 0.f;
 #pragma unroll
-    for (int w = 0; w < DA_WAVES; ++w) {
+    for (int w = 0; w < WAVES; ++w) {
       const float f = (cm[w][g] == -INFINITY) ? 0.f : expw(cm[w][g] - M);
       L += cl[w][g] * f;
       o0 += co[w][g][lane] * f;
@@ -233,7 +233,21 @@
 #ifdef Q3A_STAMP
   a.stamp = t.stamp;
 #endif
-  decode_attn_body<GROUP, KVT>(a, blockIdx.x, blockIdx.y, blockIdx.z);
+  decode_attn_body<GROUP, KVT, sizeof(KVT) == 2 ? DATTN_KEYS_PER_SPLIT_BF16 : DATTN_KEYS_PER_SPLIT_F32, DA_WAVES>(a, blockIdx.x, blockIdx.y, blockIdx.z);
+}
+template <int GROUP, typename KVT>
+__global__ __launch_bounds__(4 * 64) void decode_attn_fine_kernel(void* kcache, void* vcache, const int* pos, const float* qkv,
+                                                                  const float* rope_cur, int nsplit, int n_kv, int max_ctx, int keys_per_split,
+                                                                  DecodeAttnTail t) {
+  DecodeAttnArgs a{};
+  a.kcache = kcache; a.vcache = vcache; a.pos = pos; a.qkv = qkv; a.rope_cur = rope_cur; a.nsplit = nsplit; a.n_q = GROUP * n_kv; a.n_kv = n_kv;
+  a.max_ctx = max_ctx;
+  a.q_norm = t.q_norm; a.k_norm = t.k_norm; a.eps = t.eps; a.pm = t.pm; a.pl = t.pl; a.po = t.po; a.scale_div = t.scale_div;
+#ifdef Q3A_STAMP
+  a.stamp = t.stamp;
+#endif
+  if (keys_per_split == 32) decode_attn_body<GROUP, KVT, 32, 4>(a, blockIdx.x, blockIdx.y, blockIdx.z);
+  else decode_attn_body<GROUP, KVT, 64, 4>(a, blockIdx.x, blockIdx.y, blockIdx.z);
 }
 
 
@@ -548,9 +562,12 @@
 
 const char* launch_decode_attn(const DecodeAttnArgs& a, int S, bool kv_f32, hipStream_t s) {
   if (S <= 0) return nullptr;
-  if (a.nsplit <= 0 || (a.nsplit - 1) * dattn_keys_per_split(kv_f32) >= a.max_ctx) return "decode_attn: 1 .. ceil(max_ctx / keys per split) key splits";
+  const int kps = a.keys_per_split ? a.keys_per_split : dattn_keys_per_split(kv_f32);
+  if (kps != 128 && (kv_f32 || (kps != 32 && kps != 64))) return "decode_attn: 32- and 64-key splits run on the bf16 cache only; otherwise 128 keys per split";
+  if (a.nsplit <= 0 || (a.nsplit - 1) * kps >= a.max_ctx) return "decode_attn: 1 .. ceil(max_ctx / keys per split) key splits";
   const int group = a.n_q / a.n_kv;
-  dim3 grid(a.n_kv, S, a.nsplit), block(DA_WAVES * 64);
+  if (kps != 128 && group != 2) return "decode_attn: 32- and 64-key splits run for kv heads of two q heads";
+  dim3 grid(a.n_kv, S, a.nsplit), block((kps == 128 ? DA_WAVES : 4) * 64);
   DecodeAttnTail t{};
   t.q_norm = a.q_norm; t.k_norm = a.k_norm; t.eps = a.eps; t.pm = a.pm; t.pl = a.pl; t.po = a.po; t.scale_div = a.scale_div;
 #ifdef Q3A_STAMP
@@ -562,7 +579,9 @@
     if (kv_f32) hipLaunchKernelGGL((decode_attn_kernel<G, float>), grid, block, 0, s, Q3A_DA_ARGS); \
     else hipLaunchKernelGGL((decode_attn_kernel<G, uint16_t>), grid, block, 0, s, Q3A_DA_ARGS);     \
   } while (0)
-  if (group == 1) Q3A_DA(1);
+  if (kps != 128)
+    hipLaunchKernelGGL((decode_attn_fine_kernel<2, uint16_t>), grid, block, 0, s, a.kcache, a.vcache, a.pos, a.qkv, a.rope_cur, a.nsplit, a.n_kv, a.max_ctx, kps, t);
+  else if (group == 1) Q3A_DA(1);
   else if (group == 2) Q3A_DA(2);
   else if (group == 4) Q3A_DA(4);
   else return "decode_attn: GQA group must be 1, 2 or 4";
diff --git a/qwen3_asr_rs_amd/csrc/k_gemv.hip b/qwen3_asr_rs_amd/csrc/k_gemv.hip
--- a/qwen3_asr_rs_amd/csrc/k_gemv.hip
+++ b/qwen3_asr_rs_amd/csrc/k_gemv.hip
@@ -266,9 +266,10 @@
   }
 }
 
-template <int PR, int KI, bool RMS, bool ATTN, int MF, bool XL>
+template <int PR, int KI, bool RMS, bool ATTN, int MF, bool XL, bool XP = false>
 __device__ __forceinline__ void gemv1_body(const GemvArgs& a) {
   static_assert(!XL || !ATTN, "the merged attention vector already goes through LDS");
+  static_assert(!XP || (XL && RMS), "the partial vectors are added in the hand-over of the norm-fused XL form");
   constexpr bool XH = !RMS && !ATTN && KI > 4;
   constexpr bool XLDS = XL || XH;
   static_assert(!XH || KI % 2 == 0, "the hand-over stores unguarded: its rounds of 1024 columns must end at KI * 512");
@@ -291,6 +292,8 @@
   uint4 wq[KI][PR];
   constexpr int XLN = (KI + 1) / 2;
   float4 xl_rx[XLDS ? XLN : 1], xl_rw[(XL && RMS) ? XLN : 1];
+  constexpr int XPN = XP ? GEMV_X_PARTS_MAX : 1;
+  float4 xp_r[XP ? XLN : 1][XPN];
   auto request_x = [&]() {
     if (ATTN) return;
     if constexpr (XLDS) {
@@ -298,6 +301,11 @@
       for (int j = 0; j < XLN; ++j) {
         const int k = (tid + j * 256) * 4, kc = k < K ? k : 0;
         xl_rx[j] = *reinterpret_cast<const float4*>(a.x + kc);
+        if constexpr (XP) {
+#pragma unroll
+          for (int h = 0; h < XPN; ++h)
+            xp_r[j][h] = *reinterpret_cast<const float4*>(a.x_parts + (size_t)(h < a.x_nparts ? h : a.x_nparts - 1) * K + kc);
+        }
         if (RMS) xl_rw[j] = *reinterpret_cast<const float4*>(a.rms_w + kc);
       }
       return;
@@ -406,7 +414,13 @@
     for (int j = 0; j < XLN; ++j) {
       const int k = (tid + j * 256) * 4;
       if (XH || k < KI * 512) {
-        const float4 v = xl_rx[j];
+        float4 v = xl_rx[j];
+        if constexpr (XP) {
+#pragma unroll
+          for (int h = 0; h < XPN; ++h)
+            if (h < a.x_nparts) { v.x += xp_r[j][h].x; v.y += xp_r[j][h].y; v.z += xp_r[j][h].z; v.w += xp_r[j][h].w; }
+          if (blockIdx.x == 0 && k < K) *reinterpret_cast<float4*>(a.x_out + k) = v;
+        }
         *reinterpret_cast<float4*>(x_lds + k) = make_float4(v.x, v.y, v.z, v.w);
         if (RMS) *reinterpret_cast<float4*>(xl_w + k) = xl_rw[j];
       }
@@ -500,6 +514,120 @@
   gemv1_body<PR, KI, RMS, ATTN, MF, XL>(a);
 }
 
+struct GemvXpTail {
+  float* out; float* x_out; int fast_math;
+  Q3A_STAMP_FIELD
+};
+template <int PR, int KI>
+__global__ __launch_bounds__(256) void gemv1_xp_kernel(const uint16_t* W, const float* x, const float* rms_w, const float* x_parts,
+                                                       const float* bias, int N, int K, int x_nparts, float eps, GemvXpTail t) {
+  GemvArgs a{};
+  a.W = W; a.x = x; a.rms_w = rms_w; a.x_parts = x_parts; a.bias = bias; a.N = N; a.K = K; a.x_nparts = x_nparts; a.eps = eps; a.mode = 2;
+  a.out = t.out; a.x_out = t.x_out; a.fast_math = t.fast_math;
+  Q3A_STAMP_COPY(a, t);
+  gemv1_body<PR, KI, true, false, 0, true, true>(a);
+}
+
+struct OprojHeadTail {
+  const float* bias;
+  Q3A_STAMP_FIELD
+};
+template <int CW, int RB>
+__global__ __launch_bounds__(256) void oproj_head_kernel(const float* pm, const float* pl, const float* po, const uint16_t* W, float* y_part,
+                                                         int N, int K, int nsplit, int n_parts, OprojHeadTail t) {
+  constexpr int NS = OPROJ_HEAD_MAX_SPLITS;
+  constexpr int HEADS = CW / 128;
+  constexpr int LPR = CW / 8;
+  constexpr int RPI = 64 / LPR;
+  constexpr int NI = RB / 4 / RPI;
+  constexpr int E4 = CW / 4;
+  constexpr int TG = 256 / E4;
+  constexpr int SPT = NS / TG;
+  static_assert(CW == 128 || CW == 256 || CW == 512, "a slice is 1, 2 or 4 q heads");
+  static_assert(NI >= 1 && NI * RPI * 4 == RB && SPT * TG == NS && HEADS * NS <= 256, "row block / split plan");
+  __shared__ float m_s[HEADS * NS], l_s[HEADS * NS], inv_s[HEADS];
+  __shared__ __attribute__((aligned(16))) float red[TG][CW];
+  const int tid = threadIdx.x, lane = tid & 63, wave = tid >> 6;
+  Q3A_STAMP_ENTRY(t_entry);
+  const int part = blockIdx.x % n_parts, rb = blockIdx.x / n_parts;
+  const int q0 = part * HEADS;
+  const int e4 = tid % E4, tg = tid / E4, hh = e4 >> 5, d = (e4 & 31) * 4;
+  const int st = tid < HEADS * NS ? tid : HEADS * NS - 1, st_j = st % NS, st_jc = st_j < nsplit ? st_j : nsplit - 1;
+  float st_m = pm[(size_t)(q0 + st / NS) * nsplit + st_jc], st_l = pl[(size_t)(q0 + st / NS) * nsplit + st_jc];
+  float4 o[SPT];
+#pragma unroll
+  for (int i = 0; i < SPT; ++i) {
+    const int j = tg + i * TG, jc = j < nsplit ? j : nsplit - 1;
+    o[i] = *reinterpret_cast<const float4*>(po + ((size_t)(q0 + hh) * nsplit + jc) * 128 + d);
+  }
+  __builtin_amdgcn_sched_barrier(0);
+  const int row0 = rb * RB + wave * (RB / 4) + lane / LPR;
+  uint4 wq[NI];
+#pragma unroll
+  for (int i = 0; i < NI; ++i) {
+    const int row = row0 + i * RPI, rc = row < N ? row : N - 1;
+    wq[i] = ld_stream16(W + (size_t)rc * K + part * CW + (lane % LPR) * 8);
+  }
+  __builtin_amdgcn_sched_barrier(0);
+  float bv[NI];
+#pragma unroll
+  for (int i = 0; i < NI; ++i) {
+    const int row = row0 + i * RPI;
+    bv[i] = (t.bias && part == 0) ? t.bias[row < N ? row : N - 1] : 0.f;
+  }
+  __builtin_amdgcn_sched_barrier(0);
+  Q3A_STAMP_AT(t.stamp, blockIdx.x, 1);
+  Q3A_STAMP_PUT(t.stamp, blockIdx.x, 0, t_entry);
+  if (st_j >= nsplit) { st_m = -INFINITY; st_l = 0.f; }
+  if (tid < HEADS * NS) { m_s[tid] = st_m; l_s[tid] = st_l; }
+  __syncthreads();
+  float M = -INFINITY, L = 0.f;
+#pragma unroll
+  for (int j = 0; j < NS; ++j) M = fmaxf(M, m_s[hh * NS + j]);
+#pragma unroll
+  for (int j = 0; j < NS; ++j) L += l_s[hh * NS + j] * __expf(m_s[hh * NS + j] - M);
+  float4 acc = make_float4(0.f, 0.f, 0.f, 0.f);
+#pragma unroll
+  for (int i = 0; i < SPT; ++i) {
+    const float f = __expf(m_s[hh * NS + tg + i * TG] - M);
+    acc.x += o[i].x * f; acc.y += o[i].y * f; acc.z += o[i].z * f; acc.w += o[i].w * f;
+  }
+  *reinterpret_cast<float4*>(&red[tg][e4 * 4]) = acc;
+  if (tg == 0 && (e4 & 31) == 0) inv_s[hh] = 1.0f / L;
+  __syncthreads();
+  const int c0 = (lane % LPR) * 8;
+  float x[8];
+#pragma unroll
+  for (int e = 0; e < 8; ++e) x[e] = 0.f;
+#pragma unroll
+  for (int g = 0; g < TG; ++g) {
+    const float4 a0 = *reinterpret_cast<const float4*>(&red[g][c0]), a1 = *reinterpret_cast<const float4*>(&red[g][c0 + 4]);
+    x[0] += a0.x; x[1] += a0.y; x[2] += a0.z; x[3] += a0.w; x[4] += a1.x; x[5] += a1.y; x[6] += a1.z; x[7] += a1.w;
+  }
+  const float inv = inv_s[c0 >> 7];
+#pragma unroll
+  for (int e = 0; e < 8; ++e) x[e] *= inv;
+  Q3A_STAMP_AT(t.stamp, blockIdx.x, 2);
+  float y[NI];
+#pragma unroll
+  for (int i = 0; i < NI; ++i) {
+    float v = row16_sum(dot8(wq[i], x, 0.f));
+    if (LPR >= 32) v = xor16_sum(v);
+    if (LPR >= 64) v = xor32_sum(v);
+    y[i] = v + bv[i];
+  }
+  if (wave == 0) asm volatile("" ::"v"(y[0]));
+  Q3A_STAMP_AT(t.stamp, blockIdx.x, 3);
+  if (lane % LPR == 0) {
+#pragma unroll
+    for (int i = 0; i < NI; ++i) {
+      const int row = row0 + i * RPI;
+      if (row < N) y_part[(size_t)part * N + row] = y[i];
+    }
+  }
+  Q3A_STAMP_AT(t.stamp, blockIdx.x, 4);
+}
+
 template <int PR, int KI, bool LP = false>
 __device__ __forceinline__ void gemv1_head_block(const GemvArgs& a, int blk, float (&am_v)[4][1], int (&am_i)[4][1], float (*am_s)[1],
                                                  ArgmaxAcc<LP>& out) {
@@ -882,8 +1010,20 @@
       else hipLaunchKernelGGL((gemv1_head_kernel<PR, KI>), grid, block, 0, s, GEMV_HEAD_ARGS(a));
       return;
     }
-    if constexpr (KI == 2) { hipLaunchKernelGGL((gemv1_kernel<PR, KI, true, false, 0, true>), grid, block, 0, s, GEMV_PLAIN_ARGS(a)); return; }
-    hipLaunchKernelGGL((gemv1_kernel<PR, KI, true, false>), grid, block, 0, s, GEMV_PLAIN_ARGS(a));
+    if constexpr (KI == 2) {
+      if constexpr (PR == 2) {
+        if (a.x_parts) {
+          GemvXpTail t{};
+          t.out = a.out; t.x_out = a.x_out; t.fast_math = a.fast_math;
+          Q3A_STAMP_COPY(t, a);
+          hipLaunchKernelGGL((gemv1_xp_kernel<PR, KI>), grid, block, 0, s, a.W, a.x, a.rms_w, a.x_parts, a.bias, a.N, a.K, a.x_nparts, a.eps, t);
+          return;
+        }
+      }
+      hipLaunchKernelGGL((gemv1_kernel<PR, KI, true, false, 0, true>), grid, block, 0, s, GEMV_PLAIN_ARGS(a));
+    } else {
+      hipLaunchKernelGGL((gemv1_kernel<PR, KI, true, false>), grid, block, 0, s, GEMV_PLAIN_ARGS(a));
+    }
   } else {
     hipLaunchKernelGGL((gemv1_kernel<PR, KI, false, false>), grid, block, 0, s, GEMV_PLAIN_ARGS(a));
   }
@@ -958,6 +1098,26 @@
   return nullptr;
 }
 
+const char* oproj_head_check(const OprojHeadArgs& a) {
+  if (!a.pm || !a.pl || !a.po || !a.W || !a.y_part || a.N < 1) return "oproj_head: missing buffer";
+  if (a.N > 1024) return "oproj_head: N <= 1024 (the gate / up form that adds the partial vectors exists at K <= 1024)";
+  if (a.nsplit < 1 || a.nsplit > OPROJ_HEAD_MAX_SPLITS) return "oproj_head: 1 .. 16 key splits (more: the merging o_proj of launch_gemv)";
+  if (a.n_parts < 1 || a.K != a.n_parts * 512) return "oproj_head: a slice is 512 columns (two kv heads of two q heads)";
+  return nullptr;
+}
+const char* launch_oproj_head(const OprojHeadArgs& a, hipStream_t s) {
+  if (const char* e = oproj_head_check(a)) return e;
+  OprojHeadTail t{};
+  t.bias = a.bias;
+  Q3A_STAMP_COPY(t, a);
+  constexpr int rb = 16;
+  const dim3 grid(a.n_parts * ((a.N + rb - 1) / rb)), block(256);
+#define OPROJ_HEAD_ARGS a.pm, a.pl, a.po, a.W, a.y_part, a.N, a.K, a.nsplit, a.n_parts, t
+  hipLaunchKernelGGL((oproj_head_kernel<512, rb>), grid, block, 0, s, OPROJ_HEAD_ARGS);
+#undef OPROJ_HEAD_ARGS
+  return nullptr;
+}
+
 const char* launch_gemv(const GemvArgs& a0, int NB, hipStream_t s) {
   if (a0.K % 8 != 0) return "gemv: K must be a multiple of 8";
   if (a0.K > 6144) return "gemv: K > 6144 unsupported";
@@ -969,6 +1129,8 @@
   if (a0.attn_po && (a0.K % 128 != 0 || a0.K != a0.attn_heads * 128)) return "gemv: attention-partial input needs K = heads*128";
   if (a0.attn_po && a0.rms_w) return "gemv: attention-partial input cannot be combined with a fused RMSNorm";
   if (a0.attn_po && (NB < 4 ? NB : 4) * a0.attn_heads * a0.attn_nsplit > ATTN_F_MAX) return "gemv: too many attention splits for the LDS scale table";
+  if (a0.x_parts && (NB != 1 || !a0.x || !a0.rms_w || a0.mode != 2 || a0.K > 1024 || a0.x_nparts < 1 || a0.x_nparts > GEMV_X_PARTS_MAX || !a0.x_out))
+    return "gemv: partial vectors are added in the one-sequence norm-fused GLU form at K <= 1024 only (1 .. 4 vectors, x_out set)";
   const int pr = gemv_rows_per_wave(a0);
   const int nb_cap = (int)((64 * 1024) / ((size_t)a0.K * 4));
   int done = 0;
diff --git a/qwen3_asr_rs_amd/csrc/kernels.h b/qwen3_asr_rs_amd/csrc/kernels.h
--- a/qwen3_asr_rs_amd/csrc/kernels.h
+++ b/qwen3_asr_rs_amd/csrc/kernels.h
@@ -94,6 +94,7 @@
   std::atomic<int> eos_run_ahead{1};
   std::atomic<int> skinny_glu_hp3{1};
   std::atomic<int> lm_head_prune{1};
+  std::atomic<int> oproj_by_head{1};
   std::atomic<int> layer_taps{0};
   std::atomic<int> poison_attn_partials{0};
 };
@@ -181,9 +182,23 @@
   const float* attn_pm; const float* attn_pl; const float* attn_po; int attn_nsplit; int attn_heads;
   int attn_fast_exp;
   int fast_math;
+  const float* x_parts; int x_nparts; float* x_out;
   Q3A_STAMP_FIELD
 };
+constexpr int GEMV_X_PARTS_MAX = 4;
 const char* launch_gemv(const GemvArgs& a, int NB, hipStream_t s);
+
+struct OprojHeadArgs {
+  const float* pm; const float* pl; const float* po; int nsplit;
+  const uint16_t* W; int N; int K;
+  const float* bias;
+  int n_parts;
+  float* y_part;
+  Q3A_STAMP_FIELD
+};
+constexpr int OPROJ_HEAD_MAX_SPLITS = 16;
+const char* oproj_head_check(const OprojHeadArgs& a);
+const char* launch_oproj_head(const OprojHeadArgs& a, hipStream_t s);
 constexpr int GEMV_ATTN_MAX_TABLE = 1024;
 int gemv_blocks(const GemvArgs& a);
 int gemv_rows_per_wave(const GemvArgs& a);
@@ -249,6 +264,7 @@
   float* pm; float* pl;
   float* po;
   int nsplit;
+  int keys_per_split;
   int n_q, n_kv, max_ctx;
   float scale_div;
   float* out;
@@ -257,11 +273,9 @@
   int trim_prologue;
   Q3A_STAMP_FIELD
 };
-#ifndef Q3A_DATTN_SPLIT_KEYS
-#define Q3A_DATTN_SPLIT_KEYS 128
-#endif
-constexpr int DATTN_KEYS_PER_SPLIT_BF16 = Q3A_DATTN_SPLIT_KEYS, DATTN_KEYS_PER_SPLIT_F32 = 128;
+constexpr int DATTN_KEYS_PER_SPLIT_BF16 = 128, DATTN_KEYS_PER_SPLIT_F32 = 128;
 inline int dattn_keys_per_split(bool kv_f32) { return kv_f32 ? DATTN_KEYS_PER_SPLIT_F32 : DATTN_KEYS_PER_SPLIT_BF16; }
+inline int dattn_fine_keys_per_split(int keys) { return keys <= 512 ? 32 : keys <= 1024 ? 64 : keys <= 2048 ? 128 : 0; }
 const char* launch_decode_attn(const DecodeAttnArgs& a, int S, bool kv_f32, hipStream_t s);
 const char* launch_decode_attn_batched(const DecodeAttnArgs& a, int S, bool kv_f32, hipStream_t s);
 const char* launch_attn_combine(const float* pm, const float* pl, const float* po, int nsplit, int S, int n_q, float* out,
diff --git a/qwen3_asr_rs_amd/csrc/selftest.cpp b/qwen3_asr_rs_amd/csrc/selftest.cpp
--- a/qwen3_asr_rs_amd/csrc/selftest.cpp
+++ b/qwen3_asr_rs_amd/csrc/selftest.cpp
@@ -402,15 +402,73 @@
   Q3A_CATCH(nullptr)
 }
 
+int32_t q3a_selftest_oproj_head_launch(int32_t device, const uint16_t* w, int32_t N, int32_t K, const float* bias, const float* attn_pm, const float* attn_pl,
+                                       const float* attn_po, int32_t attn_nsplit, int32_t attn_heads, int32_t n_parts, float* y_part) {
+  Q3A_TRY(nullptr)
+  const char* what = "q3a_selftest_oproj_head_launch";
+  if (!w || !attn_pm || !attn_pl || !attn_po || !y_part || N < 1 || attn_heads < 1 || attn_nsplit < 1 || n_parts < 1 || K != attn_heads * 128)
+    fail(std::string(what) + ": bad argument");
+  OprojHeadArgs a{};
+  a.pm = attn_pm; a.pl = attn_pl; a.po = attn_po;
+  a.nsplit = attn_nsplit; a.W = w; a.N = N; a.K = K; a.n_parts = n_parts; a.y_part = y_part;
+  KCHK(oproj_head_check(a));
+  use_device(device);
+  const size_t ns = (size_t)attn_heads * attn_nsplit;
+  const DevBuf dW = to_device(w, (size_t)N * K), dPm = to_device(attn_pm, ns), dPl = to_device(attn_pl, ns), dPo = to_device(attn_po, ns * 128);
+  DevBuf dB;
+  if (bias) dB = to_device(bias, (size_t)N);
+  const Guarded dY(y_part, (size_t)n_parts * N * 4);
+  a.pm = dPm.as<float>(); a.pl = dPl.as<float>(); a.po = dPo.as<float>(); a.W = dW.as<uint16_t>(); a.bias = dB.as<float>(); a.y_part = dY.as<float>();
+  KCHK(launch_oproj_head(a, nullptr));
+  finish();
+  dY.fetch(y_part, "partial vectors");
+  Q3A_CATCH(nullptr)
+}
+
+int32_t q3a_selftest_gemv_parts_launch(int32_t device, const uint16_t* w, int32_t N, int32_t K, const float* x, const float* rms_w, float eps,
+                                       const float* bias, const float* x_parts, int32_t n_parts, float* out, float* x_out) {
+  Q3A_TRY(nullptr)
+  const char* what = "q3a_selftest_gemv_parts_launch";
+  if (!w || !x || !rms_w || !x_parts || !out || !x_out || N < 32 || N % 32 != 0 || K < 8 || K % 8 != 0 || K > 1024 || n_parts < 1 || n_parts > GEMV_X_PARTS_MAX)
+    fail(std::string(what) + ": bad argument");
+  use_device(device);
+  const DevBuf dW = to_device(w, (size_t)N * K), dP = to_device(x_parts, (size_t)n_parts * K);
+  auto padded = [&](const float* src) {
+    std::vector<float> v(1024 + 8, NAN);
+    memcpy(v.data(), src, (size_t)K * 4);
+    return to_device(v);
+  };
+  const DevBuf dX = padded(x), dG = padded(rms_w);
+  DevBuf dB;
+  if (bias) dB = to_device(bias, (size_t)N);
+  const Guarded dO(out, (size_t)N / 2 * 4), dXo(x_out, (size_t)K * 4);
+  GemvArgs g{};
+  g.x = dX.as<float>(); g.ldx = K; g.rms_w = dG.as<float>(); g.eps = eps; g.W = dW.as<uint16_t>(); g.N = N; g.K = K; g.bias = dB.as<float>();
+  g.mode = 2; g.out = dO.as<float>(); g.ldo = N / 2; g.fast_math = 0;
+  g.x_parts = dP.as<float>(); g.x_nparts = n_parts; g.x_out = dXo.as<float>();
+  KCHK(launch_gemv(g, 1, nullptr));
+  finish();
+  dO.fetch(out, "output"); dXo.fetch(x_out, "summed x");
+  Q3A_CATCH(nullptr)
+}
+
 int32_t q3a_selftest_decode_attn_launch(int32_t device, int32_t kv_f32, const float* qkv, int32_t pos, const float* q_norm, const float* k_norm, float eps,
                                         const float* rope_cur, void* kcache, void* vcache, int32_t n_q, int32_t n_kv, int32_t max_ctx, int32_t nsplit,
                                         float scale_div, float* pm, float* pl, float* po) {
+  return q3a_selftest_decode_attn_split_launch(device, kv_f32, 0, qkv, pos, q_norm, k_norm, eps, rope_cur, kcache, vcache, n_q, n_kv, max_ctx, nsplit,
+                                               scale_div, pm, pl, po);
+}
+
+int32_t q3a_selftest_decode_attn_split_launch(int32_t device, int32_t kv_f32, int32_t keys_per_split, const float* qkv, int32_t pos, const float* q_norm,
+                                              const float* k_norm, float eps, const float* rope_cur, void* kcache, void* vcache, int32_t n_q, int32_t n_kv,
+                                              int32_t max_ctx, int32_t nsplit, float scale_div, float* pm, float* pl, float* po) {
   Q3A_TRY(nullptr)
   const char* what = "q3a_selftest_decode_attn_launch";
   if (!qkv || !q_norm || !k_norm || !rope_cur || !kcache || !vcache || !pm || !pl || !po || n_q < 1 || n_kv < 1 || n_q % n_kv != 0 || max_ctx < 1 ||
       nsplit < 1 || !(scale_div > 0.f))
     fail(std::string(what) + ": bad argument");
-  const int keys = dattn_keys_per_split(kv_f32 != 0);
+  if (keys_per_split != 0 && keys_per_split != 32 && keys_per_split != 64 && keys_per_split != 128) fail(std::string(what) + ": 32, 64 or 128 keys per split (0: the default)");
+  const int keys = keys_per_split ? keys_per_split : dattn_keys_per_split(kv_f32 != 0);
   if (pos < 0 || pos >= max_ctx || pos >= nsplit * keys) fail(std::string(what) + ": pos outside the cache or beyond the last split");
   use_device(device);
   const size_t eb = kv_f32 ? 4 : 2, n_cache = (size_t)n_kv * max_ctx * 128, ns = (size_t)n_q * nsplit;
@@ -420,7 +478,7 @@
   DecodeAttnArgs a{};
   a.qkv = dQkv.as<float>(); a.pos = dPos.as<int>(); a.q_norm = dQn.as<float>(); a.k_norm = dKn.as<float>(); a.eps = eps; a.rope_cur = dRope.as<float>();
   a.kcache = dK.as<void>(); a.vcache = dV.as<void>(); a.pm = dPm.as<float>(); a.pl = dPl.as<float>(); a.po = dPo.as<float>();
-  a.nsplit = nsplit; a.n_q = n_q; a.n_kv = n_kv; a.max_ctx = max_ctx; a.scale_div = scale_div;
+  a.nsplit = nsplit; a.keys_per_split = keys_per_split; a.n_q = n_q; a.n_kv = n_kv; a.max_ctx = max_ctx; a.scale_div = scale_div;
   KCHK(launch_decode_attn(a, 1, kv_f32 != 0, nullptr));
   finish();
   dK.fetch(kcache, "key cache"); dV.fetch(vcache, "value cache"); dPm.fetch(pm, "split maxima"); dPl.fetch(pl, "split sums"); dPo.fetch(po, "split outputs");
```

New measurement: 524.7 audio-seconds/sec, median of 6. 1.06x the previous value.
